# abb128/april-asr

Measured on AMD Instinct MI355X. Metric: audio_seconds_per_second (concurrent 16 kHz sessions x 1/RTF), aprilv0_en-us-sized streaming RNN-T, higher is better.
Workload: dtype f32

## Files before the change

april_asr_amd/__init__.py:

```python
import ctypes as C
import math
import struct
import weakref
from enum import IntEnum
from typing import Callable, List, Sequence

import numpy as np

from . import _ffi

__all__ = ["Result", "Token", "Model", "Session", "SessionGroup", "Bias", "resampler_taps"]


class Result(IntEnum):
    PARTIAL_RECOGNITION = 1
    FINAL_RECOGNITION = 2
    ERROR_CANT_KEEP_UP = 3
    SILENCE = 4


class Token:
    __slots__ = ("token", "logprob", "word_boundary", "sentence_end", "time", "log_softmax", "confidence", "blank_log_softmax",
                 "alternatives")

# ... 90 lines not shown
        if device_ptr:
            h = L.aprilx_model_from_blob(C.c_void_p(device_ptr), size, 1)
        else:
            blob = np.ascontiguousarray(blob, np.uint8)
            h = L.aprilx_model_from_blob(blob.ctypes.data, blob.size, 0)
        if not h:
            raise Exception("Failed to build model from blob")
        m = cls.__new__(cls)
        m._L = L; m._handle = h
        m.dims = _ffi.AprilxDims()
        L.aprilx_model_dims(h, C.byref(m.dims))
        return m

    @staticmethod
    def broadcast_id() -> bytes:
        L = _ffi.init()
        buf = C.create_string_buffer(128)
        n = L.aprilx_broadcast_get_id(buf, 128)
        if n <= 0:
            raise RuntimeError("aprilx_broadcast_get_id failed")
        return buf.raw[:n]

    @classmethod
    def broadcast(cls, root_model, rank: int, world: int, id_bytes: bytes):
        L = _ffi.init()
        idb = C.create_string_buffer(bytes(id_bytes), 128)
        h = L.aprilx_model_broadcast(root_model._handle if root_model is not None else None, rank, world, idb)
        if not h:
            raise Exception("model broadcast failed")
        if root_model is not None:
            return root_model
        m = cls.__new__(cls)
        m._L = L; m._handle = h
        m.dims = _ffi.AprilxDims()
        L.aprilx_model_dims(h, C.byref(m.dims))
        return m

    def load_info(self):
        info = _ffi.AprilxLoadInfo()
        self._L.aprilx_model_load_info(self._handle, C.byref(info))
        return info

    def save_blob(self, path: str, f16: bool = False):
        fn = self._L.aprilx_model_save_blob_f16 if f16 else self._L.aprilx_model_save_blob
        if fn(self._handle, path.encode("utf-8")) != 0:
            raise RuntimeError("blob save failed")

    @classmethod
    def load_blob(cls, path: str, init_gpu: bool = True):
        L = _ffi.init() if init_gpu else _ffi.lib()
        h = L.aprilx_model_load_blob(path.encode("utf-8"))
        if not h:
            raise Exception("Failed to load model blob")
        m = cls.__new__(cls)
        m._L = L; m._handle = h
        m.dims = _ffi.AprilxDims()
        L.aprilx_model_dims(h, C.byref(m.dims))
        return m

    def run_encoder(self, x, h, c):
        d = self.dims
        x = np.ascontiguousarray(x, np.float32); n = x.shape[0]
        h = np.ascontiguousarray(h, np.float32).reshape(n, d.n_layers, d.d_model)
        c = np.ascontiguousarray(c, np.float32).reshape(n, d.n_layers, d.hidden)
        eout = np.empty((n, d.joiner), np.float32); h2 = np.empty_like(h); c2 = np.empty_like(c)
        rc = self._L.aprilx_run_encoder(self._handle, n, x.ctypes.data, h.ctypes.data, c.ctypes.data,
                                        eout.ctypes.data, h2.ctypes.data, c2.ctypes.data)
        assert rc == 0
        return eout, h2, c2

    def run_decoder(self, ctx):
        ctx = np.ascontiguousarray(ctx, np.int64).reshape(-1, self.dims.context)
        out = np.empty((ctx.shape[0], self.dims.joiner), np.float32)
        assert self._L.aprilx_run_decoder(self._handle, ctx.shape[0], ctx.ctypes.data, out.ctypes.data) == 0
        return out

    def run_joiner(self, eout, dout):
        e = np.ascontiguousarray(eout, np.float32).reshape(-1, self.dims.joiner)
        dd = np.ascontiguousarray(dout, np.float32).reshape(-1, self.dims.joiner)
        out = np.empty((e.shape[0], self.dims.vocab), np.float32)
        assert self._L.aprilx_run_joiner(self._handle, e.shape[0], e.ctypes.data, dd.ctypes.data, out.ctypes.data) == 0
        return out

    def run_fbank(self, pcm_frames):
        p = np.ascontiguousarray(pcm_frames, np.int16).reshape(-1, self.dims.fft_size)
        out = np.empty((p.shape[0], self.dims.mel), np.float32)
        assert self._L.aprilx_run_fbank(self._handle, p.shape[0], p.ctypes.data, out.ctypes.data) == 0
        return out

    def resample(self, pcm, in_rate: int) -> np.ndarray:
        a = np.ascontiguousarray(pcm, np.int16).ravel()
        lmk = np.zeros(3, np.int32)
        if self._L.aprilx_resampler_taps(int(in_rate), int(self.dims.sample_rate), lmk.ctypes.data, None, 0) != 0:
            raise ValueError("input rate %d is not accepted" % in_rate)
        cap = (a.size * int(lmk[0]) + int(lmk[1]) - 1) // int(lmk[1])
        out = np.zeros(max(cap, 1), np.int16)
        n = int(self._L.aprilx_resample(self._handle, int(in_rate), a.ctypes.data, a.size, out.ctypes.data, out.size))
        if n < 0:
            raise ValueError("aprilx_resample refused %d samples at %d Hz" % (a.size, in_rate))
        return out[:n]

    def run_confidence(self, logits, k: int):
        a = np.ascontiguousarray(logits, np.float32).reshape(-1, self.dims.vocab)
        out = (_ffi.AprilxTokenInfo * a.shape[0])()
        if self._L.aprilx_run_confidence(self._handle, a.shape[0], a.ctypes.data, int(k), out) != 0:
            raise ValueError("aprilx_run_confidence refused n=%d k=%d" % (a.shape[0], k))
        return out

    def bias(self, phrases, boost: float = 2.0, strict: bool = False):
        return Bias(self, phrases, boost, flags=BIAS_STRICT if strict else 0)

    def run_confidence_biased(self, logits, k: int, bias, bias_state):
        a = np.ascontiguousarray(logits, np.float32).reshape(-1, self.dims.vocab)
        bs = np.ascontiguousarray(bias_state, np.int32).reshape(a.shape[0])
        out = (_ffi.AprilxTokenInfo * a.shape[0])()
        if self._L.aprilx_run_confidence_biased(self._handle, a.shape[0], a.ctypes.data, int(k), bias._handle, bs.ctypes.data, out) != 0:
            raise ValueError("aprilx_run_confidence_biased refused n=%d k=%d" % (a.shape[0], k))
        return out

    def run_decide_biased(self, logits, early_emit, now_ms, rnd, state, bias, bias_state, op: int = 0):
        st = np.ascontiguousarray(state, np.int32).reshape(-1, 4).copy()
        n = st.shape[0]
        lg = np.ascontiguousarray(logits, np.float32).reshape(n, self.dims.vocab)
        now = np.ascontiguousarray(now_ms, np.int32).reshape(n)
        bs = np.ascontiguousarray(bias_state, np.int32).reshape(n).copy()
        rec = np.zeros(n, np.dtype([("idx", np.int32), ("max", np.float32), ("blank", np.float32), ("flags", np.uint32)]))
        rc = self._L.aprilx_run_decide_biased(self._handle, n, int(op), lg.ctypes.data, float(early_emit), now.ctypes.data, int(rnd),
                                              st.ctypes.data, rec.ctypes.data, bias._handle, bs.ctypes.data)
        if rc != 0:
            raise ValueError("aprilx_run_decide_biased refused the call")
        return rec, st, bs

    def run_decide_opts(self, logits, early_emit, now_ms, rnd, state, opts, bias=None, bias_state=None, op: int = 0):
        st = np.ascontiguousarray(state, np.int32).reshape(-1, 4).copy()
        n = st.shape[0]
        lg = np.ascontiguousarray(logits, np.float32).reshape(n, self.dims.vocab)
        now = np.ascontiguousarray(now_ms, np.int32).reshape(n)
        bs = np.ascontiguousarray(bias_state, np.int32).reshape(n).copy() if bias is not None else None
        arr = (_ffi.AprilxSearchOptions * n)()
        for i, o in enumerate(opts):
            if o is not None:
                arr[i].size = C.sizeof(_ffi.AprilxSearchOptions); arr[i].endpoint_silence_ms = int(o[0]); arr[i].blank_penalty = float(o[1])
        rec = np.zeros(n, np.dtype([("idx", np.int32), ("max", np.float32), ("blank", np.float32), ("flags", np.uint32)]))
        rc = self._L.aprilx_run_decide_opts(self._handle, n, int(op), lg.ctypes.data, float(early_emit), now.ctypes.data, int(rnd), st.ctypes.data,
                                            rec.ctypes.data, bias._handle if bias is not None else None, bs.ctypes.data if bs is not None else None, arr)
        if rc != 0:
            raise ValueError("aprilx_run_decide_opts refused the call")
        return rec, st, bs

    def stats(self, device_index: int = 0):
        s = _ffi.AprilxStats()
        self._L.aprilx_model_stats(self._handle, device_index, C.byref(s))
        return s

    def feed_latencies(self, device_index: int = 0, reset: bool = False) -> np.ndarray:
        n = int(self._L.aprilx_model_feed_latency(self._handle, device_index, None, 0, 0))
        out = np.zeros(n, np.float64)
        if n:
            n = int(self._L.aprilx_model_feed_latency(self._handle, device_index, out.ctypes.data, n, 1 if reset else 0))
        elif reset:
            self._L.aprilx_model_feed_latency(self._handle, device_index, None, 0, 1)
        return out[:n]

    def profile(self, enable):
        self._L.aprilx_model_profile(self._handle, int(enable))


BIAS_STRICT = 1


class Bias:

    def __init__(self, model: Model, phrases, boost: float = 2.0, flags: int = 0):
        self._L = model._L
        items = [(p, boost) if isinstance(p, (str, bytes)) else (p[0], p[1]) for p in phrases]
        raw = [p.encode("utf-8") if isinstance(p, str) else bytes(p) for p, _ in items]
        arr = (C.c_char_p * max(len(raw), 1))(*raw)
        boosts = (C.c_float * max(len(raw), 1))(*[float(b) for _, b in items])
        err = C.create_string_buffer(256)
        self._handle = self._L.aprilx_bias_create_ex(model._handle, len(raw), arr, boosts, int(flags), err, 256)
        self.message = err.value.decode("utf-8", "replace")
        if not self._handle:
            raise ValueError("bias set refused: " + self.message)
        st, ed = C.c_int32(0), C.c_int64(0)
        self.dropped = int(self._L.aprilx_bias_info(self._handle, C.byref(st), C.byref(ed)))
        self.states, self.n_edges = int(st.value), int(ed.value)
        self.flags = int(self._L.aprilx_bias_flags(self._handle))
        self.strict = bool(self.flags & BIAS_STRICT)

    def edges(self, state: int):
        n = int(self._L.aprilx_bias_edges(self._handle, int(state), None, None, None, 0))
        if n < 0:
            raise ValueError("no state %d" % state)
        tok = np.zeros(n, np.int32); nxt = np.zeros(n, np.int32); bonus = np.zeros(n, np.float32)
        if n:
            assert self._L.aprilx_bias_edges(self._handle, int(state), tok.ctypes.data, nxt.ctypes.data, bonus.ctypes.data, n) == n
        return tok, nxt, bonus

    def csr(self):
        parts = [self.edges(s) for s in range(self.states)]
        off = np.zeros(self.states + 1, np.int32)
        off[1:] = np.cumsum([p[0].size for p in parts])
        return (off,) + tuple(np.concatenate([p[i] for p in parts]) if parts else np.zeros(0) for i in range(3))

    def close(self):
        if getattr(self, "_handle", None):
            self._L.aprilx_bias_free(self._handle)
            self._handle = None

    def __del__(self):
        try:
            self.close()
        except Exception:
            pass


def _dispatch(userdata, result_type, count, tokens):
    sess = C.cast(userdata, C.py_object).value
    sess._on_result(result_type, count, tokens)


_HANDLER = _ffi.HANDLER(_dispatch)


class Session:
    def __init__(self, model: Model, callback: Callable[[Result, List[Token]], None], asynchronous: bool = False,
                 no_rt: bool = False, speaker_name: str = "", raw_events: bool = False, counters=None, input_sample_rate=None,
                 alternatives=None, bias=None, endpoint_silence_ms=None, blank_penalty=None, max_utterance_ms=None):
        self._L = model._L
        self.info_log = None
        self.model = model
        self.callback = callback
        self._raw = raw_events
        cfg = _ffi.AprilConfig()
        cfg.flags = (2 if no_rt else 1) if asynchronous else 0
        if speaker_name:
            cfg.speaker = _ffi.AprilSpeakerID.from_buffer_copy(struct.pack("@q", hash(speaker_name)) * 2)
        if counters is not None:
            self._counters = counters
            cfg.handler = C.cast(self._L.aprilx_counting_handler, _ffi.HANDLER)
            cfg.userdata = counters.ctypes.data
        else:
            cfg.handler = _HANDLER
            cfg.userdata = id(self)
        self._handle = self._L.aas_create_session(model._handle, cfg)
        if not self._handle:
            raise Exception("Failed to create session")
        if not hasattr(model, "_sessions"):
            model._sessions = weakref.WeakSet()
        model._sessions.add(self)
        if input_sample_rate is not None:
            self.set_input_rate(input_sample_rate)
        if alternatives:
            self.set_confidence(alternatives)
        if bias is not None:
            self.set_bias(bias)
        if endpoint_silence_ms is not None or blank_penalty is not None or max_utterance_ms is not None:
            self.set_search_options(endpoint_silence_ms, blank_penalty, max_utterance_ms)

    def _on_result(self, result_type, count, tokens):
        if self.info_log is not None:
            self.info_log.append((int(result_type), [C.string_at(tokens[i].reserved, C.sizeof(_ffi.AprilxTokenInfo)) if tokens[i].reserved
                                                     else None for i in range(count)]))
        if self._raw:
            self.callback(int(result_type), [(tokens[i].token, float(tokens[i].logprob), int(tokens[i].flags),
                                              int(tokens[i].time_ms)) for i in range(count)])
        else:
            self.callback(Result(result_type), [Token(tokens[i], self.model) for i in range(count)])

    def get_rt_speedup(self) -> float:
        return float(self._L.aas_realtime_get_speedup(self._handle))

    def feed_pcm16(self, data) -> None:
        if isinstance(data, (bytes, bytearray, memoryview)):
            buf = (C.c_char * len(data)).from_buffer_copy(bytes(data))
            self._L.aas_feed_pcm16(self._handle, C.addressof(buf), len(data) // 2)
        else:
            a = np.ascontiguousarray(data, np.int16)
            self._L.aas_feed_pcm16(self._handle, a.ctypes.data, a.size)

    def flush(self) -> None:
        self._L.aas_flush(self._handle)

    def set_input_rate(self, rate_hz: int) -> None:
        if self._L.aprilx_session_set_input_rate(self._handle, int(rate_hz)) != 0:
            raise ValueError("input rate %d refused (outside 4000..384000 Hz / L > 4096, or audio fed since the last flush)" % rate_hz)

    def set_confidence(self, n_alternatives: int) -> None:
        if self._L.aprilx_session_set_confidence(self._handle, int(n_alternatives)) != 0:
            raise ValueError("confidence with %d alternatives refused (0..8, and no audio fed since the last flush)" % n_alternatives)

    def set_bias(self, bias) -> None:
        if self._L.aprilx_session_set_bias(self._handle, bias._handle if bias is not None else None) != 0:
            raise ValueError("bias set refused (built for another token list, 64 sets in use on the engine already, or audio fed since the last flush)")

    def set_search_options(self, endpoint_silence_ms=None, blank_penalty=None, max_utterance_ms=None) -> None:
        if endpoint_silence_ms is None and blank_penalty is None and max_utterance_ms is None:
            rc = self._L.aprilx_session_set_search_options(self._handle, None)
        else:
            o = _ffi.AprilxSearchOptions(C.sizeof(_ffi.AprilxSearchOptions), 2200 if endpoint_silence_ms is None else int(endpoint_silence_ms),
                                         0 if max_utterance_ms is None else int(max_utterance_ms), 0.0 if blank_penalty is None else float(blank_penalty))
            rc = self._L.aprilx_session_set_search_options(self._handle, C.byref(o))
        if rc != 0:
            raise ValueError("search options refused (a value out of range, or audio fed since the last flush)")

    @property
# ... 124 lines not shown
```

april_asr_amd/_ffi.py:

```python
import ctypes as C
import os

_HERE = os.path.dirname(os.path.abspath(__file__))
LIB_PATH = os.environ.get("APRIL_ASR_LIB") or os.path.join(_HERE, "libaprilasr.so")


class AprilSpeakerID(C.Structure):
    _fields_ = [("data", C.c_uint8 * 16)]


class AprilToken(C.Structure):
    _fields_ = [("token", C.c_char_p), ("logprob", C.c_float), ("flags", C.c_int),
                ("time_ms", C.c_size_t), ("reserved", C.c_void_p)]


HANDLER = C.CFUNCTYPE(None, C.c_void_p, C.c_int, C.c_size_t, C.POINTER(AprilToken))


class AprilConfig(C.Structure):
    _fields_ = [("speaker", AprilSpeakerID), ("handler", HANDLER), ("userdata", C.c_void_p), ("flags", C.c_int)]


class AprilxDims(C.Structure):
    _fields_ = [(n, C.c_int32) for n in ("n_layers", "d_model", "hidden", "ffn", "joiner", "vocab", "mel", "seg",
                                         "seg_step", "context", "fft_size", "frame_shift", "sample_rate", "blank_id",
                                         "n_devices", "precision", "d_model_file")] + [("param_count", C.c_int64)]


class AprilxStats(C.Structure):
    _fields_ = [(n, C.c_uint64) for n in ("ticks", "steps", "chunks", "rounds", "frames", "max_batch_seen")] + \
               [("kernel_ms", C.c_double * 6), ("kernel_launches", C.c_uint64 * 6), ("host_ms", C.c_double * 8),
                ("flights", C.c_uint64), ("replay_mismatch", C.c_uint64), ("kernels_per_step", C.c_uint64),
                ("lm_steps", C.c_uint64), ("lm_chunks", C.c_uint64),
                ("wave_steps", C.c_uint64), ("wave_chunks", C.c_uint64),
                ("gates_clock_ms", C.c_double), ("gates_clock_launches", C.c_uint64), ("gates_clock_rows", C.c_uint64),
                ("gates_clock_ms_by_n", C.c_double * 4), ("gates_clock_launches_by_n", C.c_uint64 * 4),
                ("resample_ms", C.c_double), ("resample_launches", C.c_uint64), ("confidence_records", C.c_uint64)]


class AprilxTokenInfo(C.Structure):
    _fields_ = [("size", C.c_uint32), ("n_alt", C.c_uint32), ("eval_index", C.c_uint64), ("lse", C.c_float),
                ("token_logprob", C.c_float), ("blank_logprob", C.c_float), ("reserved0", C.c_float),
                ("alt_id", C.c_int32 * 8), ("alt_logit", C.c_float * 8)]


class AprilxSearchOptions(C.Structure):
    _fields_ = [("size", C.c_uint32), ("endpoint_silence_ms", C.c_uint32), ("max_utterance_ms", C.c_uint32), ("blank_penalty", C.c_float)]


class AprilxLoadInfo(C.Structure):
    _fields_ = [("broadcast_ms", C.c_double), ("comm_init_ms", C.c_double), ("broadcast_bytes", C.c_uint64),
                ("ranks", C.c_int32), ("used_rccl", C.c_int32)]


EXPORTED_REFERENCE_SYMBOLS = [
    "aam_api_init", "aam_create_model", "aam_get_name", "aam_get_description", "aam_get_language",
    "aam_get_sample_rate", "aam_free", "aas_create_session", "aas_feed_pcm16", "aas_flush",
    "aas_realtime_get_speedup", "aas_free",
]
EXPORTED_ENGINE_SYMBOLS = [
    "aprilx_model_dims", "aprilx_model_token", "aprilx_model_blob_size", "aprilx_model_export_blob",
    "aprilx_model_from_blob", "aprilx_model_save_blob", "aprilx_model_save_blob_f16", "aprilx_model_load_blob",
    "aprilx_broadcast_get_id", "aprilx_model_broadcast", "aprilx_model_load_info", "aprilx_feed_many", "aprilx_flush_many", "aprilx_session_drain", "aprilx_feed_many_pipelined", "aprilx_drain_many",
    "aprilx_run_encoder", "aprilx_run_decoder", "aprilx_run_joiner", "aprilx_run_fbank", "aprilx_run_decide", "aprilx_plan_gemm", "aprilx_stream_form",
    "aprilx_session_trace_logits", "aprilx_session_chunks", "aprilx_session_read_frames", "aprilx_session_context", "aprilx_model_stats", "aprilx_model_profile", "aprilx_model_feed_latency",
    "aprilx_greedy_create", "aprilx_greedy_step", "aprilx_greedy_finish", "aprilx_greedy_free", "aprilx_probe_file", "aprilx_model_load_host", "aprilx_model_fbank_tables", "aprilx_counting_handler",
    "aprilx_session_set_input_rate", "aprilx_session_input_rate", "aprilx_resampler_taps", "aprilx_resample",
    "aprilx_session_set_confidence", "aprilx_session_confidence", "aprilx_run_confidence",
    "aprilx_bias_create", "aprilx_bias_free", "aprilx_bias_info", "aprilx_bias_edges", "aprilx_session_set_bias", "aprilx_session_bias_state",
    "aprilx_run_decide_biased", "aprilx_greedy_set_bias", "aprilx_greedy_bias_state",
    "aprilx_bias_create_ex", "aprilx_bias_flags", "aprilx_run_confidence_biased",
    "aprilx_session_set_search_options", "aprilx_session_search_options", "aprilx_run_decide_opts", "aprilx_greedy_set_search_options",
]

_lib = None
_inited = False


def lib():
    global _lib
    if _lib is not None:
        return _lib
    if not os.path.exists(LIB_PATH):
        raise ImportError("libaprilasr.so is not built: run `python -c 'import __graft_entry__ as g; g.build()'` "
                          "or `make -C april_asr_amd/csrc` (hipcc, gfx950). There is no CPU fallback.")
    L = C.CDLL(LIB_PATH)
    vp, sz = C.c_void_p, C.c_size_t
    L.aam_api_init.argtypes = [C.c_int]; L.aam_api_init.restype = None
    L.aam_create_model.argtypes = [C.c_char_p]; L.aam_create_model.restype = vp
    for f in ("aam_get_name", "aam_get_description", "aam_get_language"):
        getattr(L, f).argtypes = [vp]; getattr(L, f).restype = C.c_char_p
    L.aam_get_sample_rate.argtypes = [vp]; L.aam_get_sample_rate.restype = sz
    L.aam_free.argtypes = [vp]; L.aam_free.restype = None
    L.aas_create_session.argtypes = [vp, AprilConfig]; L.aas_create_session.restype = vp
    L.aas_feed_pcm16.argtypes = [vp, vp, sz]; L.aas_feed_pcm16.restype = None
    L.aas_flush.argtypes = [vp]; L.aas_flush.restype = None
    L.aas_realtime_get_speedup.argtypes = [vp]; L.aas_realtime_get_speedup.restype = C.c_float
    L.aas_free.argtypes = [vp]; L.aas_free.restype = None
    L.aprilx_model_dims.argtypes = [vp, C.POINTER(AprilxDims)]; L.aprilx_model_dims.restype = C.c_int
    L.aprilx_model_token.argtypes = [vp, C.c_int32]; L.aprilx_model_token.restype = C.c_char_p
    L.aprilx_model_blob_size.argtypes = [vp]; L.aprilx_model_blob_size.restype = sz
    L.aprilx_model_export_blob.argtypes = [vp, vp, sz]; L.aprilx_model_export_blob.restype = C.c_int
    L.aprilx_model_from_blob.argtypes = [vp, sz, C.c_int]; L.aprilx_model_from_blob.restype = vp
    L.aprilx_model_save_blob.argtypes = [vp, C.c_char_p]; L.aprilx_model_save_blob.restype = C.c_int
    L.aprilx_model_save_blob_f16.argtypes = [vp, C.c_char_p]; L.aprilx_model_save_blob_f16.restype = C.c_int
    L.aprilx_model_load_blob.argtypes = [C.c_char_p]; L.aprilx_model_load_blob.restype = vp
    L.aprilx_broadcast_get_id.argtypes = [vp, sz]; L.aprilx_broadcast_get_id.restype = C.c_int
    L.aprilx_model_broadcast.argtypes = [vp, C.c_int, C.c_int, vp]; L.aprilx_model_broadcast.restype = vp
    L.aprilx_model_load_info.argtypes = [vp, C.POINTER(AprilxLoadInfo)]; L.aprilx_model_load_info.restype = C.c_int
    L.aprilx_feed_many.argtypes = [sz, C.POINTER(vp), C.POINTER(vp), C.POINTER(sz)]; L.aprilx_feed_many.restype = None
    L.aprilx_flush_many.argtypes = [sz, C.POINTER(vp)]; L.aprilx_flush_many.restype = None
    L.aprilx_session_drain.argtypes = [vp]; L.aprilx_session_drain.restype = None
    L.aprilx_feed_many_pipelined.argtypes = [sz, C.POINTER(vp), C.POINTER(vp), C.POINTER(sz), C.c_int]; L.aprilx_feed_many_pipelined.restype = None
    L.aprilx_drain_many.argtypes = [sz, C.POINTER(vp)]; L.aprilx_drain_many.restype = None
    L.aprilx_run_encoder.argtypes = [vp, C.c_int] + [vp] * 6; L.aprilx_run_encoder.restype = C.c_int
    L.aprilx_run_decoder.argtypes = [vp, C.c_int, vp, vp]; L.aprilx_run_decoder.restype = C.c_int
    L.aprilx_run_joiner.argtypes = [vp, C.c_int, vp, vp, vp]; L.aprilx_run_joiner.restype = C.c_int
    L.aprilx_run_fbank.argtypes = [vp, C.c_int, vp, vp]; L.aprilx_run_fbank.restype = C.c_int
    L.aprilx_plan_gemm.argtypes = [C.c_int] * 6 + [vp]; L.aprilx_plan_gemm.restype = C.c_int
    L.aprilx_stream_form.argtypes = [C.c_int] * 6; L.aprilx_stream_form.restype = C.c_int
    L.aprilx_run_decide.argtypes = [vp, C.c_int, C.c_int, vp, C.c_float, vp, C.c_int, vp, vp]; L.aprilx_run_decide.restype = C.c_int
    L.aprilx_session_trace_logits.argtypes = [vp, vp, sz, C.POINTER(sz)]; L.aprilx_session_trace_logits.restype = None
    L.aprilx_session_chunks.argtypes = [vp]; L.aprilx_session_chunks.restype = C.c_uint64
    L.aprilx_session_read_frames.argtypes = [vp, C.c_uint64, C.c_int, C.c_void_p]; L.aprilx_session_read_frames.restype = C.c_uint64
    L.aprilx_session_context.argtypes = [vp, vp, vp]; L.aprilx_session_context.restype = None
    L.aprilx_model_stats.argtypes = [vp, C.c_int, C.POINTER(AprilxStats)]; L.aprilx_model_stats.restype = None
    L.aprilx_model_feed_latency.argtypes = [vp, C.c_int, vp, C.c_int, C.c_int]; L.aprilx_model_feed_latency.restype = C.c_int
    L.aprilx_model_profile.argtypes = [vp, C.c_int]; L.aprilx_model_profile.restype = None
    L.aprilx_greedy_create.argtypes = [vp, HANDLER, vp]; L.aprilx_greedy_create.restype = vp
    L.aprilx_greedy_step.argtypes = [vp, C.c_int32, C.c_float, C.c_float, C.c_float, sz, C.POINTER(C.c_int32)]
    L.aprilx_greedy_step.restype = C.c_int
    L.aprilx_greedy_finish.argtypes = [vp]; L.aprilx_greedy_finish.restype = None
    L.aprilx_greedy_free.argtypes = [vp]; L.aprilx_greedy_free.restype = None
    L.aprilx_model_load_host.argtypes = [C.c_char_p]; L.aprilx_model_load_host.restype = vp
    L.aprilx_model_fbank_tables.argtypes = [vp, vp, vp]; L.aprilx_model_fbank_tables.restype = C.c_int
    L.aprilx_probe_file.argtypes = [C.c_char_p, C.c_char_p, sz]; L.aprilx_probe_file.restype = C.c_int
    L.aprilx_session_set_input_rate.argtypes = [vp, C.c_uint32]; L.aprilx_session_set_input_rate.restype = C.c_int
    L.aprilx_session_input_rate.argtypes = [vp]; L.aprilx_session_input_rate.restype = C.c_uint32
    L.aprilx_resampler_taps.argtypes = [C.c_uint32, C.c_uint32, vp, vp, sz]; L.aprilx_resampler_taps.restype = C.c_int
    L.aprilx_resample.argtypes = [vp, C.c_uint32, vp, sz, vp, sz]; L.aprilx_resample.restype = C.c_int64
    L.aprilx_session_set_confidence.argtypes = [vp, C.c_int]; L.aprilx_session_set_confidence.restype = C.c_int
    L.aprilx_session_confidence.argtypes = [vp]; L.aprilx_session_confidence.restype = C.c_int
    L.aprilx_run_confidence.argtypes = [vp, C.c_int, vp, C.c_int, vp]; L.aprilx_run_confidence.restype = C.c_int
    L.aprilx_bias_create.argtypes = [vp, sz, C.POINTER(C.c_char_p), C.POINTER(C.c_float), C.c_char_p, sz]; L.aprilx_bias_create.restype = vp
    L.aprilx_bias_create_ex.argtypes = [vp, sz, C.POINTER(C.c_char_p), C.POINTER(C.c_float), C.c_uint32, C.c_char_p, sz]; L.aprilx_bias_create_ex.restype = vp
    L.aprilx_bias_flags.argtypes = [vp]; L.aprilx_bias_flags.restype = C.c_int
    L.aprilx_run_confidence_biased.argtypes = [vp, C.c_int, vp, C.c_int, vp, vp, vp]; L.aprilx_run_confidence_biased.restype = C.c_int
    L.aprilx_bias_free.argtypes = [vp]; L.aprilx_bias_free.restype = None
    L.aprilx_bias_info.argtypes = [vp, C.POINTER(C.c_int32), C.POINTER(C.c_int64)]; L.aprilx_bias_info.restype = C.c_int
    L.aprilx_bias_edges.argtypes = [vp, C.c_int32, vp, vp, vp, sz]; L.aprilx_bias_edges.restype = C.c_int
    L.aprilx_session_set_bias.argtypes = [vp, vp]; L.aprilx_session_set_bias.restype = C.c_int
    L.aprilx_session_bias_state.argtypes = [vp, C.POINTER(C.c_int32), C.POINTER(C.c_int32)]; L.aprilx_session_bias_state.restype = C.c_int
    L.aprilx_run_decide_biased.argtypes = [vp, C.c_int, C.c_int, vp, C.c_float, vp, C.c_int, vp, vp, vp, vp]; L.aprilx_run_decide_biased.restype = C.c_int
    L.aprilx_greedy_set_bias.argtypes = [vp, vp]; L.aprilx_greedy_set_bias.restype = C.c_int
    L.aprilx_greedy_bias_state.argtypes = [vp]; L.aprilx_greedy_bias_state.restype = C.c_int
    L.aprilx_session_set_search_options.argtypes = [vp, C.POINTER(AprilxSearchOptions)]; L.aprilx_session_set_search_options.restype = C.c_int
    L.aprilx_session_search_options.argtypes = [vp, C.POINTER(AprilxSearchOptions)]; L.aprilx_session_search_options.restype = C.c_int
    L.aprilx_run_decide_opts.argtypes = [vp, C.c_int, C.c_int, vp, C.c_float, vp, C.c_int, vp, vp, vp, vp, vp]; L.aprilx_run_decide_opts.restype = C.c_int
    L.aprilx_greedy_set_search_options.argtypes = [vp, C.POINTER(AprilxSearchOptions)]; L.aprilx_greedy_set_search_options.restype = C.c_int
    _lib = L
    return L


def init():
    global _inited
    L = lib()
    if not _inited:
        L.aam_api_init(1)
        _inited = True
    return L
```

april_asr_amd/csrc/engine.cc:

```cpp
#include "engine.h"
#include <array>
#include <algorithm>
#include <cmath>
#include <chrono>
#include <cstdlib>
#include <cstring>
#include "common.h"
#include "env.h"

namespace aprilx {

static size_t align64(size_t x) { return (x + 63) & ~(size_t)63; }

void plan_layout(const NetDims &d, bool has_dec_conv_b, PackedLayout &L)
{
    L.dims = d;
    L.has_dec_conv_b = has_dec_conv_b;
    L.vocab_pad = (d.vocab + 31) & ~31;
    size_t off = 0;
    auto take = [&](size_t n) { size_t o = off; off = align64(off + n); return o; };
    L.k3 = (d.conv_ch[1] * 9 + 63) & ~63;
    L.conv_w[0] = take((size_t)d.conv_ch[0] * 9); L.conv_b[0] = take((size_t)d.conv_ch[0]);
    L.conv_w[1] = take((size_t)d.conv_ch[1] * d.conv_ch[0] * 9); L.conv_b[1] = take((size_t)d.conv_ch[1]);
    L.conv_w[2] = take((size_t)L.k3 * d.conv_ch[2]); L.conv_b[2] = take((size_t)d.conv_ch[2]);
// ... 27 lines not shown
    v.emplace_back(L.w_out, (size_t)d.joiner * L.vocab_pad);
    return v;
}

static void pack_mfma(const float *W, int K, int N, int Npad, const std::vector<int> *colmap, float *dst)
{
    const int KB = K / 16, NTt = Npad / 16;
    for (int t = 0; t < NTt; ++t)
        for (int kb = 0; kb < KB; ++kb)
            for (int lane = 0; lane < 64; ++lane) {
                const int np = t * 16 + (lane & 15);
                const int src = np < N ? (colmap ? (*colmap)[(size_t)np] : np) : -1;
                float *o = dst + (((size_t)t * KB + kb) * 64 + lane) * 4;
                for (int j = 0; j < 4; ++j) {
                    const int k = kb * 16 + (lane >> 4) * 4 + j;
                    o[j] = src >= 0 ? W[(size_t)k * N + src] : 0.0f;
                }
            }
}

void pack_weights(const HostModel &m, PackedLayout &L, std::vector<float> &blob)
{
    const NetDims &d = L.dims;
    blob.assign(L.total, 0.0f);
    float *B = blob.data();
    for (int i = 0; i < 3; ++i) {
        if (i < 2) memcpy(B + L.conv_w[i], m.conv_w[i].data(), m.conv_w[i].size() * 4);
        memcpy(B + L.conv_b[i], m.conv_b[i].data(), m.conv_b[i].size() * 4);
    }
    {
        const int kreal = d.conv_ch[1] * 9, c2 = d.conv_ch[2];
        std::vector<float> w3((size_t)L.k3 * c2, 0.0f);
        for (int o = 0; o < c2; ++o) for (int k = 0; k < kreal; ++k) w3[(size_t)k * c2 + o] = m.conv_w[2][(size_t)o * kreal + k];
        pack_mfma(w3.data(), L.k3, c2, c2, nullptr, B + L.conv_w[2]);
    }
    {
        const int c2 = d.conv_ch[2], F = d.f_out;
        std::vector<float> we((size_t)d.embed_in * d.d_model);
        for (int c = 0; c < c2; ++c) for (int f = 0; f < F; ++f)
            memcpy(&we[((size_t)f * c2 + c) * d.d_model], &m.w_embed[((size_t)c * F + f) * d.d_model], (size_t)d.d_model * 4);
        pack_mfma(we.data(), d.embed_in, d.d_model, d.d_model, nullptr, B + L.w_embed);
    }
    memcpy(B + L.b_embed, m.b_embed.data(), (size_t)d.d_model * 4);
    L.embed_eps = m.embed_norm_eps;
    L.norm_eps.resize((size_t)d.n_layers);
    std::vector<int> gmap((size_t)4 * d.hidden);
    for (int u = 0; u < d.hidden; ++u) for (int g = 0; g < 4; ++g) gmap[(size_t)u * 4 + g] = g * d.hidden + u;
    for (int l = 0; l < d.n_layers; ++l) {
        const LayerWeights &lw = m.layers[(size_t)l];
        const PackedLayout::Layer &o = L.layers[(size_t)l];
        pack_mfma(lw.w_gates.data(), 2 * d.d_model, 4 * d.hidden, 4 * d.hidden, &gmap, B + o.wg);
        for (int n = 0; n < 4 * d.hidden; ++n) B[o.bg + n] = lw.b_gates[(size_t)gmap[(size_t)n]];
        pack_mfma(lw.w_hr.data(), d.hidden, d.d_model, d.d_model, nullptr, B + o.whr);
        pack_mfma(lw.w_ff1.data(), d.d_model, d.ffn, d.ffn, nullptr, B + o.wff1);
        memcpy(B + o.bff1, lw.b_ff1.data(), (size_t)d.ffn * 4);
        pack_mfma(lw.w_ff2.data(), d.ffn, d.d_model, d.d_model, nullptr, B + o.wff2);
        memcpy(B + o.bff2, lw.b_ff2.data(), (size_t)d.d_model * 4);
        L.norm_eps[(size_t)l] = lw.norm_eps;
    }
    pack_mfma(m.w_encproj.data(), d.d_model, d.joiner, d.joiner, nullptr, B + L.w_encproj);
    memcpy(B + L.b_encproj, m.b_encproj.data(), (size_t)d.joiner * 4);
    memcpy(B + L.emb, m.emb.data(), m.emb.size() * 4);
    memcpy(B + L.dec_conv, m.dec_conv.data(), m.dec_conv.size() * 4);
    if (!m.dec_conv_b.empty()) memcpy(B + L.dec_conv_b, m.dec_conv_b.data(), m.dec_conv_b.size() * 4);
    pack_mfma(m.w_decproj.data(), d.d_model, d.joiner, d.joiner, nullptr, B + L.w_decproj);
    memcpy(B + L.b_decproj, m.b_decproj.data(), (size_t)d.joiner * 4);
    pack_mfma(m.w_out.data(), d.joiner, d.vocab, L.vocab_pad, nullptr, B + L.w_out);
    memcpy(B + L.b_out, m.b_out.data(), (size_t)d.vocab * 4);
}

template <typename T> static T *dmalloc(size_t n) { HipLegacyLock legacy; T *p = nullptr; HIP_CHECK(hipMalloc((void **)&p, std::max<size_t>(n, 1) * sizeof(T))); return p; }
template <typename T> static T *hmalloc(size_t n) { HipLegacyLock legacy; T *p = nullptr; HIP_CHECK(hipHostMalloc((void **)&p, std::max<size_t>(n, 1) * sizeof(T), hipHostMallocDefault)); return p; }

std::recursive_mutex &hip_legacy_mutex() { static std::recursive_mutex m; return m; }

static int pick_kz(int K, int N, int kblk = 16)
{
    int kz = 256 / std::max(1, N / 16);
    kz = std::max(1, std::min(kz, 8));
    while (kz > 1 && ((K / kblk) / kz < 4 || (K / kblk) % (4 * kz) != 0)) kz >>= 1;
    return kz;
}

Engine::Engine(const EngineConfig &cfg, const PackedLayout &layout, const float *blob_host, const float *blob_device,
               const ModelParams &params, const FbankHostTables &ft, const std::vector<uint8_t> &tok_class)
    : cfg_(cfg), L_(layout), P_(params)
{
    HipLegacyLock legacy;
    HIP_CHECK(hipSetDevice(cfg_.device));
    HIP_CHECK(hipStreamCreateWithFlags(&stream_, hipStreamNonBlocking));
    HIP_CHECK(hipStreamCreateWithFlags(&f_stream_, hipStreamNonBlocking));
    HIP_CHECK(hipStreamCreateWithFlags(&s_stream_, hipStreamNonBlocking));
    search_stream_ = stream_;
    for (int i = 0; i < 32; ++i) { hipEvent_t e; HIP_CHECK(hipEventCreateWithFlags(&e, hipEventDisableTiming)); join_ev_.push_back(e); }
    split_streams_ = std::max(0, std::min(2, env_int("APRIL_SPLIT_STREAMS", 2)));
    const NetDims &d = L_.dims;
    w_ = dmalloc<float>(L_.total);
    if (blob_device) HIP_CHECK(hipMemcpy(w_, blob_device, L_.total * 4, hipMemcpyDeviceToDevice));
    else if (blob_host) HIP_CHECK(hipMemcpy(w_, blob_host, L_.total * 4, hipMemcpyHostToDevice));

    const size_t S = (size_t)cfg_.max_slots, MB = (size_t)cfg_.max_batch;
    ring_frames_ = std::max(P_.segment_size * 32, env_int("APRIL_RING_FRAMES", 8192));
    h_ = dmalloc<float>((size_t)d.n_layers * S * d.d_model);
    c_ = dmalloc<float>((size_t)d.n_layers * S * d.hidden);
    if (!env_str("APRIL_RING_FRAMES")) {
        size_t free_b = 0, total_b = 0;
        if (hipMemGetInfo(&free_b, &total_b) == hipSuccess && free_b > 0) {
            const size_t per_frame = S * (size_t)d.mel * sizeof(float);
            const size_t fit = (free_b / 4) / per_frame;
            if (fit < (size_t)ring_frames_) {
                const int shrunk = std::max(P_.segment_size * 32, (int)std::min<size_t>(fit, 8192) / 64 * 64);
                LOGW("engine: %zu MB of feature rings (%d frames x %zu slots) exceed a quarter of the %zu MB free on device %d: %d frames per session",
                     per_frame * (size_t)ring_frames_ >> 20, ring_frames_, S, free_b >> 20, cfg_.device, shrunk);
                ring_frames_ = shrunk;
            }
        } else (void)hipGetLastError();
        float *p = nullptr;
        if (hipMalloc((void **)&p, S * ring_frames_ * d.mel * sizeof(float)) == hipSuccess) ring_ = p;
        else {
            (void)hipGetLastError();
            const size_t asked = S * (size_t)ring_frames_ * d.mel * sizeof(float);
            ring_frames_ = std::max(P_.segment_size * 32, 2048);
            LOGW("engine: no room for %zu MB of feature rings, falling back to %d frames per session", asked >> 20, ring_frames_);
        }
    }
    if (!ring_) ring_ = dmalloc<float>(S * ring_frames_ * d.mel);
    eout_ = dmalloc<float>(S * d.joiner);
    dout_ = dmalloc<float>(S * d.joiner);
    gstate_ = dmalloc<GreedyState>(S);
    HIP_CHECK(hipMemset(h_, 0, (size_t)d.n_layers * S * d.d_model * 4));
    HIP_CHECK(hipMemset(c_, 0, (size_t)d.n_layers * S * d.hidden * 4));
    HIP_CHECK(hipMemset(ring_, 0, S * ring_frames_ * d.mel * 4));
    HIP_CHECK(hipMemset(eout_, 0, S * d.joiner * 4));
    HIP_CHECK(hipMemset(dout_, 0, S * d.joiner * 4));
    {
        std::vector<GreedyState> init(S);
        for (auto &g : init) { g.ctx0 = P_.blank_id; g.ctx1 = P_.blank_id; g.last_tok = -1; g.last_emit_ms = 0; }
        HIP_CHECK(hipMemcpy(gstate_, init.data(), S * sizeof(GreedyState), hipMemcpyHostToDevice));
    }
    cls_ = dmalloc<uint8_t>((size_t)d.vocab);
    HIP_CHECK(hipMemcpy(cls_, tok_class.data(), (size_t)d.vocab, hipMemcpyHostToDevice));

    kz_embed_ = pick_kz(d.embed_in, d.d_model);
    kz_hr_ = pick_kz(d.hidden, d.d_model);
    kz_ff2_ = pick_kz(d.ffn, d.d_model);
    kz_proj_ = pick_kz(d.d_model, d.joiner);
    kz_out_ = pick_kz(d.joiner, L_.vocab_pad);
    {
        const bool want = cfg_.precision == 1 && env_int("APRIL_F16_TILE", 1) != 0;
        f16_tile_ = want && d.d_model % 128 == 0 && d.hidden % 128 == 0 && d.ffn % 128 == 0 && d.hidden % 16 == 0;
        if (f16_tile_) {
            kzx_hr_ = pick_kz(d.hidden, d.d_model, 32); kzx_ff2_ = pick_kz(d.ffn, d.d_model, 32);
            for (int p = 0; p < 2; ++p) y16_buf_[p] = dmalloc<uint16_t>(MB * d.d_model);
            y16_ = y16_buf_[0]; xb16_ = dmalloc<uint16_t>(MB * d.d_model);
            u16_ = dmalloc<uint16_t>(MB * d.hidden); ff16_ = dmalloc<uint16_t>(MB * d.ffn);
            h16_ = dmalloc<uint16_t>((size_t)d.n_layers * S * d.d_model);
            HIP_CHECK(hipMemset(h16_, 0, (size_t)d.n_layers * S * d.d_model * 2));
        }
    }
    ws_mstride_ = cfg_.max_batch;
    const size_t ws_n = (size_t)std::max({kz_embed_ * d.d_model, kz_hr_ * d.d_model, kz_ff2_ * d.d_model, kz_proj_ * d.joiner, kz_out_ * L_.vocab_pad});
    ws_ = dmalloc<float>(ws_n * MB);
    ws_g_ = dmalloc<float>((size_t)std::max(kz_proj_ * d.joiner, kz_out_ * L_.vocab_pad) * MB);
    xin_ = dmalloc<float>(MB * d.embed_in);
    a3_ = dmalloc<float>(MB * d.f_out * L_.k3);
    HIP_CHECK(hipMemset(a3_, 0, MB * d.f_out * L_.k3 * 4));
    for (int p = 0; p < 2; ++p) { y_buf_[p] = dmalloc<float>(MB * d.d_model); ssq_buf_[p] = dmalloc<float>(MB * (d.d_model / SSQ_COLS)); }
    y_ = y_buf_[0]; ssq_ = ssq_buf_[0];
    ws_fe_ = dmalloc<float>((size_t)kz_embed_ * d.d_model * MB);
    ws_sr_ = dmalloc<float>((size_t)std::max(kz_proj_ * d.joiner, d.d_model) * MB);
    xb_ = dmalloc<float>(MB * d.d_model);
    u_ = dmalloc<float>(MB * d.hidden);
    ff_ = dmalloc<float>(MB * d.ffn);
    de_ = dmalloc<float>(MB * d.d_model);
    HIP_CHECK(hipMemset(de_, 0, MB * d.d_model * 4));
    logits_ = dmalloc<float>(3 * MB * d.vocab);
    logits_h_ = hmalloc<float>(3 * MB * d.vocab);
    ring_cap_ = std::max<size_t>((size_t)1 << 20, 3 * MB * 8 + 2 * S); ring_h_ = hmalloc<int>(2 * ring_cap_);
    step_cap_ = 1 << 14; step_off_h_ = hmalloc<int>((size_t)2 * step_cap_); rec_off_h_ = hmalloc<int>((size_t)2 * step_cap_);
    rec_cap_ = std::max<size_t>((size_t)1 << 20, 3 * MB * 8); rec_d_ = dmalloc<StepRecord>(2 * rec_cap_); rec_h_ = hmalloc<StepRecord>(2 * rec_cap_);
    for (int i = 0; i < 2; ++i) HIP_CHECK(hipEventCreateWithFlags(&flight_done_[i], hipEventDisableTiming));
    counter_d_ = dmalloc<int>(1);
    for (int p = 0; p < 2; ++p) {
        rec_off_buf_[p] = dmalloc<int>(1); flags_buf_[p] = dmalloc<int>(8); step_buf_[p] = dmalloc<int>(4 * MB);
        HIP_CHECK(hipMemset(rec_off_buf_[p], 0, 4)); HIP_CHECK(hipMemset(flags_buf_[p], 0, 32));
    }
    rec_off_d_ = rec_off_buf_[0]; flags_d_ = flags_buf_[0]; step_d_ = step_buf_[0];
    active_d_ = dmalloc<int>(MB); dirty_d_ = dmalloc<int>(MB);
    dec_slots_d_ = dmalloc<int>(std::max(S, MB));
    HIP_CHECK(hipMemset(counter_d_, 0, 4));

    upload_tables(ft);
    use_graphs_ = env_int("APRIL_NO_GRAPHS", 0) == 0;
    if (const int n = env_int("APRIL_GRAPH_CACHE_CAP", 0))
        step_graphs_.cap = lm_graphs_.cap = lm_search_graphs_.cap = sw_plan_cap_ = (size_t)std::max(n, 2), sw_graphs_.cap = 4 * sw_plan_cap_;
    free_.reserve(S);
    for (int i = cfg_.max_slots - 1; i >= 0; --i) free_.push_back(i);
    LOGI("engine: device %d, %d slots, max batch %d, weights %.1f MB, kz(embed,hr,ff2,proj,out)=%d,%d,%d,%d,%d",
         cfg_.device, cfg_.max_slots, cfg_.max_batch, L_.total * 4.0 / 1e6, kz_embed_, kz_hr_, kz_ff2_, kz_proj_, kz_out_);
}

void Engine::finish_weights()
{
    HipLegacyLock legacy;
    HIP_CHECK(hipSetDevice(cfg_.device));
    if (cfg_.precision == 1 && !wh_) {
        wh_ = dmalloc<uint16_t>(L_.total);
        for (const auto &sec : gemm_sections(L_)) launch_cvt_f16(w_ + sec.first, wh_ + sec.first, sec.second, nullptr);
        if (f16_tile_) {
            const NetDims &d = L_.dims;
            wx_ = dmalloc<uint16_t>(L_.total);
            for (const PackedLayout::Layer &o : L_.layers) {
                launch_repack_x32(w_ + o.wg, wx_ + o.wg, 2 * d.d_model, 4 * d.hidden, nullptr);
                launch_repack_x32(w_ + o.whr, wx_ + o.whr, d.hidden, d.d_model, nullptr);
                launch_repack_x32(w_ + o.wff1, wx_ + o.wff1, d.d_model, d.ffn, nullptr);
                launch_repack_x32(w_ + o.wff2, wx_ + o.wff2, d.ffn, d.d_model, nullptr);
            }
        }
        HIP_CHECK(hipDeviceSynchronize());
    }
    if (!conv_wt_) {
        const NetDims &d = L_.dims;
        conv_wt_ = dmalloc<float>((size_t)9 * d.conv_ch[0] + (size_t)9 * d.conv_ch[0] * d.conv_ch[1]);
        launch_conv_weight_transpose(w_ + L_.conv_w[0], w_ + L_.conv_w[1], d.conv_ch[0], d.conv_ch[1], conv_wt_, conv_wt_ + (size_t)9 * d.conv_ch[0], nullptr);
        HIP_CHECK(hipDeviceSynchronize());
    }
    build_dec_table();
}

void Engine::build_dec_table()
{
    if (dec_table_) return;
    const NetDims &d = L_.dims;
    const size_t limit_mb = (size_t)std::max(0, env_int("APRIL_DEC_TABLE_MB", 2048));
    const size_t rows = (size_t)d.vocab * (size_t)d.vocab;
    if (d.context != 2 || rows * (size_t)d.joiner * 4 > limit_mb * 1024 * 1024 || rows * (size_t)d.joiner * 4 >= ((size_t)1 << 32)) return;
    const int MB = cfg_.max_batch;
    float *table = dmalloc<float>(rows * (size_t)d.joiner);
    std::vector<int> iota((size_t)MB), ctx((size_t)MB * 2);
    for (int i = 0; i < MB; ++i) iota[(size_t)i] = i;
    int *ctx_d = dmalloc<int>((size_t)MB * 2);
    HIP_CHECK(hipMemcpy(dec_slots_d_, iota.data(), (size_t)MB * 4, hipMemcpyHostToDevice));
    for (size_t base = 0; base < rows; base += (size_t)MB) {
        const int n = (int)std::min<size_t>((size_t)MB, rows - base);
        for (int i = 0; i < n; ++i) { const size_t r = base + (size_t)i; ctx[(size_t)2 * i] = (int)(r / (size_t)d.vocab); ctx[(size_t)2 * i + 1] = (int)(r % (size_t)d.vocab); }
        HIP_CHECK(hipMemcpy(ctx_d, ctx.data(), (size_t)n * 8, hipMemcpyHostToDevice));
        DecEmbedArgs a; a.dec = dec_params(); a.ctx = ctx_d; a.M = n; a.out = de_; a.ldo = d.d_model;
        launch_dec_embed(a, stream_);
        run_decproj(n, dec_slots_d_, nullptr, nullptr, 1, table + base * (size_t)d.joiner);
        HIP_CHECK(hipStreamSynchronize(stream_));
    }
    (void)hipFree(ctx_d);
    dec_table_ = table;
    LOGI("engine: decoder table %zu rows x %d (%.0f MB)", rows, d.joiner, rows * (double)d.joiner * 4 / 1e6);
}

Engine::~Engine()
{
    HipLegacyLock legacy;
    (void)hipSetDevice(cfg_.device);
    (void)hipStreamSynchronize(f_stream_); (void)hipStreamSynchronize(stream_); (void)hipStreamSynchronize(s_stream_);
    dump_stream_trace();
    for (StreamTrace &t : trace_) for (hipEvent_t e : t.ev) if (e) (void)hipEventDestroy(e);
    if (trace_base_) (void)hipEventDestroy(trace_base_);
    for (hipEvent_t e : join_ev_) (void)hipEventDestroy(e);
    for (auto &e : ev_pool_) { (void)hipEventDestroy(e.a); (void)hipEventDestroy(e.b); }
    drop_graphs(); free_sw_plans(); if (gclk_slots_) (void)hipFree(gclk_slots_);
    if (lm_stream_) { (void)hipStreamSynchronize(lm_stream_); (void)hipStreamDestroy(lm_stream_); }
    for (hipEvent_t e : lm_events_) (void)hipEventDestroy(e);
    if (zargs_h_) { (void)hipHostFree(zargs_h_); (void)hipFree(zargs_d_); }
    for (int i = 0; i < 3; ++i) if (zargs_done_[i]) (void)hipEventDestroy(zargs_done_[i]);
    for (void *p : {(void *)lm_now_d_, (void *)lm_rows_d_, (void *)lm_rec_off_d_}) if (p) (void)hipFree(p);
    if (conf_k_d_) (void)hipFree(conf_k_d_);
    if (conf_d_) (void)hipFree(conf_d_);
    if (conf_k_h_) (void)hipHostFree(conf_k_h_);
    if (conf_h_) (void)hipHostFree(conf_h_);
    for (auto &b : bias_sets_) if (b.dev) (void)hipFree(b.dev);
    for (void *p : {(void *)bias_set_d_, (void *)bias_state_d_, (void *)bias_desc_d_}) if (p) (void)hipFree(p);
    for (void *p : {(void *)bias_set_h_, (void *)bias_desc_h_}) if (p) (void)hipHostFree(p);
    if (opt_d_) (void)hipFree(opt_d_);
    if (opt_h_) (void)hipHostFree(opt_h_);
    if (ws_g_) (void)hipFree(ws_g_);
    if (conv_wt_) (void)hipFree(conv_wt_);
    if (dec_table_) (void)hipFree(dec_table_);
    if (p_lm_) (void)hipFree(p_lm_);
    for (int p = 0; p < 2; ++p)
        for (void *q : {(void *)eout_lm_buf_[p], (void *)y16_buf_[p], (void *)y_buf_[p], (void *)ssq_buf_[p], (void *)rec_off_buf_[p], (void *)flags_buf_[p], (void *)step_buf_[p]}) if (q) (void)hipFree(q);
    if (ws_fe_) (void)hipFree(ws_fe_);
    if (ws_sr_) (void)hipFree(ws_sr_);
    for (void *p : {(void *)wx_, (void *)xb16_, (void *)u16_, (void *)ff16_, (void *)h16_}) if (p) (void)hipFree(p);
    for (void *p : {(void *)w_, (void *)wh_, (void *)h_, (void *)c_, (void *)ring_, (void *)eout_, (void *)dout_, (void *)gstate_, (void *)cls_, (void *)ws_, (void *)xin_,
                    (void *)a3_, (void *)xb_, (void *)u_, (void *)ff_, (void *)de_, (void *)logits_, (void *)rec_d_, (void *)counter_d_,
                    (void *)active_d_, (void *)dirty_d_, (void *)dec_slots_d_,
                    (void *)ds_desc_[0], (void *)ds_desc_[1], (void *)ds_pcm_[0], (void *)ds_pcm_[1]})
        if (p) (void)hipFree(p);
    for (void *p : {(void *)ring_h_, (void *)step_off_h_, (void *)rec_off_h_, (void *)rec_h_, (void *)logits_h_, (void *)hs_desc_[0], (void *)hs_desc_[1], (void *)hs_pcm_[0], (void *)hs_pcm_[1]})
        if (p) (void)hipHostFree(p);
    for (int b = 0; b < 2; ++b) if (fb_done_[b]) (void)hipEventDestroy(fb_done_[b]);
    for (int b = 0; b < 2; ++b) if (flight_done_[b]) (void)hipEventDestroy(flight_done_[b]);
    for (void *p : table_allocs_) (void)hipFree(p);
    (void)hipStreamDestroy(stream_); (void)hipStreamDestroy(f_stream_); (void)hipStreamDestroy(s_stream_);
}

void Engine::upload_tables(const FbankHostTables &ft)
{
    auto up = [&](const void *src, size_t bytes) {
        void *p = nullptr;
        HIP_CHECK(hipMalloc(&p, std::max<size_t>(bytes, 16)));
        if (bytes) HIP_CHECK(hipMemcpy(p, src, bytes, hipMemcpyHostToDevice));
        table_allocs_.push_back(p);
        return p;
    };
    ft_.window = (const float *)up(ft.window.data(), ft.window.size() * 4);
    ft_.mel = (const float *)up(ft.mel.data(), ft.mel.size() * 4);
    ft_.mel_lo = (const int *)up(ft.mel_lo.data(), ft.mel_lo.size() * 4);
    ft_.mel_hi = (const int *)up(ft.mel_hi.data(), ft.mel_hi.size() * 4);
    ft_.nfct = (int)ft.factors.size();
    for (int k = 0; k < ft_.nfct; ++k) {
        ft_.fct[k] = ft.factors[(size_t)k];
        ft_.tw[k] = (const double *)up(ft.tw[(size_t)k].data(), ft.tw[(size_t)k].size() * 8);
        ft_.tws[k] = ft.tws[(size_t)k].empty() ? nullptr : (const double *)up(ft.tws[(size_t)k].data(), ft.tws[(size_t)k].size() * 8);
    }
    ft_.padded = ft.padded; ft_.nbins = ft.nbins;
    pad_value_ = ft.pad_value;
}

int Engine::alloc_slot()
{
    std::lock_guard<std::mutex> g(slot_mu_);
    if (free_.empty() && !zero_pending_.empty()) zero_pending_slots();
    if (free_.empty()) return -1;
    const int s = free_.back();
    free_.pop_back();
    ++live_;
    return s;
}

void Engine::zero_pending_slots()
{
    if (zero_pending_.empty()) return;
    if (hipSetDevice(cfg_.device) == hipSuccess) {
        std::lock_guard<std::mutex> cg(capture_mu_);
        const NetDims &d = L_.dims;
        for (size_t o = 0; o < zero_pending_.size(); o += 64) {
            ZeroSlotArgs z;
            z.h = h_; z.c = c_; z.n_layers = d.n_layers; z.slots = (size_t)cfg_.max_slots; z.d_model = d.d_model; z.hidden = d.hidden;
            z.eout = eout_; z.dout = dout_; z.joiner = d.joiner; z.state = gstate_; z.blank = P_.blank_id; z.h16 = h16_;
            z.n_list = (int)std::min<size_t>(64, zero_pending_.size() - o);
            for (int i = 0; i < z.n_list; ++i) z.list[i] = zero_pending_[o + (size_t)i];
            launch_zero_slot(z, stream_);
        }
    }
    for (int s : zero_pending_) free_.push_back(s);
    zero_pending_.clear();
}

void Engine::free_slot(int slot)
{
    if (conf_ever_.load(std::memory_order_relaxed)) set_slot_confidence(slot, 0);
    if (bias_ever_.load(std::memory_order_relaxed)) set_slot_bias(slot, nullptr);
    if (opt_ever_.load(std::memory_order_relaxed)) set_slot_search_options(slot, SearchOpt{0u, 0.0f});
    std::lock_guard<std::mutex> g(slot_mu_);
    zero_pending_.push_back(slot);
    --live_;
    if (zero_pending_.size() >= 256) zero_pending_slots();
}

void Engine::sync_streams()
{
    HIP_CHECK(hipStreamSynchronize(f_stream_)); HIP_CHECK(hipStreamSynchronize(stream_)); HIP_CHECK(hipStreamSynchronize(s_stream_));
}

void Engine::sync()
{
    sync_streams();
    f_unseen_by_m_ = s_unseen_by_m_ = m_unseen_by_f_ = m_unseen_by_s_ = false;
    if (profiling_) collect_timing();
}

template <typename Chain> static hipGraphExec_t capture_graph(hipStream_t st, Chain &&chain)
{
    hipGraph_t graph = nullptr;
    hipGraphExec_t exec = nullptr;
    HipLegacyLock capture_guard;
    HIP_CHECK(hipStreamBeginCapture(st, hipStreamCaptureModeRelaxed));
    chain();
    HIP_CHECK(hipStreamEndCapture(st, &graph));
    HIP_CHECK(hipGraphInstantiate(&exec, graph, nullptr, nullptr, 0));
    HIP_CHECK(hipGraphDestroy(graph));
    return exec;
}

void GraphCache::clear()
{
    if (!map_.empty()) LOGI("engine: %s graphs emptied (%zu entries)", name, map_.size());
    for (auto &g : map_) (void)hipGraphExecDestroy(g.second);
    map_.clear(); uses_.clear();
}

template <typename Chain> hipGraphExec_t Engine::cached_graph(GraphCache &cache, const GraphCache::Key &key, hipStream_t st, Chain &&chain)
{
    if (!cache.find(key)) cache.insert(key, capture_graph(st, chain));
    return cache.find(key);
}

template <typename Capture> void Engine::capture_both_parities(Capture &&capture)
{
    const int par = flight_parity_;
    for (int q : {1 - par, par}) { select_parity(q); capture(); }
}

Engine::StreamTrace *Engine::trace_slot()
{
    static const char *path = env_str("APRIL_STREAM_TRACE");
    if (!path) return nullptr;
    if (!trace_base_) { HIP_CHECK(hipEventCreate(&trace_base_)); HIP_CHECK(hipEventRecord(trace_base_, stream_)); }
    if (trace_.size() >= 4096) return nullptr;
    trace_.emplace_back();
    StreamTrace &t = trace_.back();
    for (hipEvent_t &e : t.ev) HIP_CHECK(hipEventCreate(&e));
    return &t;
}

void Engine::dump_stream_trace()
{
    const char *path = env_str("APRIL_STREAM_TRACE");
    if (!path || trace_.empty()) return;
    FILE *f = fopen(path, "w");
    if (!f) return;
    fprintf(f, "# one line per split feed; times in us since the first split feed; FE = index fetch + conv + embed on stream F, LY = layer wavefront on M, SR = encoder_proj + search on S\n");
    fprintf(f, "# feed sessions chunks  FE_start FE_end  LY_start LY_end  SR_start SR_end   overlap: FE inside the previous feed's LY window? SR inside the next feed's LY window?\n");
    std::vector<std::array<float, 6>> ts;
    for (StreamTrace &t : trace_) {
        std::array<float, 6> a{};
        bool ok = t.used;
        for (int i = 0; i < 6 && ok; ++i) ok = hipEventElapsedTime(&a[(size_t)i], trace_base_, t.ev[i]) == hipSuccess;
        if (ok) ts.push_back(a); else (void)hipGetLastError();
    }
    for (size_t i = 0; i < ts.size(); ++i) {
        const auto &a = ts[i];
        const bool fe_in_prev = i > 0 && a[0] * 1e3f < ts[i - 1][3] * 1e3f && a[1] * 1e3f > ts[i - 1][2] * 1e3f;
        const bool sr_in_next = i + 1 < ts.size() && a[5] > ts[i + 1][2] && a[4] < ts[i + 1][3];
        fprintf(f, "%4zu %5d %2d  %10.1f %10.1f  %10.1f %10.1f  %10.1f %10.1f   %s %s\n", i, trace_[i].m, trace_[i].T, a[0] * 1e3, a[1] * 1e3, a[2] * 1e3, a[3] * 1e3, a[4] * 1e3, a[5] * 1e3,
                fe_in_prev ? "FE<prevLY" : "-", sr_in_next ? "SR<nextLY" : "-");
    }
    fclose(f);
}

void Engine::join(hipStream_t waiter, hipStream_t src)
{
    hipEvent_t e = join_ev_[join_pos_++ % join_ev_.size()];
    HIP_CHECK(hipEventRecord(e, src));
    HIP_CHECK(hipStreamWaitEvent(waiter, e, 0));
}

void Engine::general_prologue()
{
    if (f_unseen_by_m_) { join(stream_, f_stream_); f_unseen_by_m_ = false; }
    if (s_unseen_by_m_) { join(stream_, s_stream_); s_unseen_by_m_ = false; }
    m_unseen_by_f_ = m_unseen_by_s_ = true;
    flight_tail_s_ = false;
}

void Engine::set_profiling(bool on) { std::lock_guard<std::mutex> cg(capture_mu_); sync(); profiling_ = on; }
void Engine::reset_timing() { for (auto &t : timing_) t = KernelTiming(); }
void Engine::set_gates_clock(bool on)
{
    std::lock_guard<std::mutex> cg(capture_mu_);
    HIP_CHECK(hipSetDevice(cfg_.device));
    sync();
    if (on) {
        if (!gclk_slots_) gclk_slots_ = dmalloc<unsigned long long>((size_t)GCLK_SLOTS * STAMP_WORDS);
        HIP_CHECK(hipMemsetAsync(gclk_slots_, 0, (size_t)GCLK_SLOTS * STAMP_WORDS * 8, stream_));
        HIP_CHECK(hipStreamSynchronize(stream_));
        gclk_ms_ = 0; gclk_launches_ = 0; gclk_rows_ = 0;
        for (int i = 0; i < 4; ++i) { gclk_ms_n_[i] = 0; gclk_launches_n_[i] = 0; }
        gclk_ = true;
        return;
    }
    collect_gates_clock(); gclk_ = false;
}
void Engine::collect_gates_clock()
{
    if (!gclk_ || !gclk_slots_) return;
    std::vector<unsigned long long> h((size_t)GCLK_SLOTS * STAMP_WORDS);
    HIP_CHECK(hipMemcpyAsync(h.data(), gclk_slots_, h.size() * 8, hipMemcpyDeviceToHost, stream_)); HIP_CHECK(hipStreamSynchronize(stream_));
    for (auto &kv : sw_plans_)
        for (size_t i = 0; i < kv.second.stamp_slots.size(); ++i) {
            const auto &sl = kv.second.stamp_slots[i];
            const unsigned long long ticks = h[(size_t)sl.first * STAMP_WORDS + 2], n = h[(size_t)sl.first * STAMP_WORDS + 3];
            gclk_ms_ += (double)ticks * 1e-5; gclk_launches_ += (long)n; gclk_rows_ += (long)n * sl.second;
            const int bn = std::min(std::max(kv.second.stamp_n[i], 1), 4) - 1;
            gclk_ms_n_[bn] += (double)ticks * 1e-5; gclk_launches_n_[bn] += (long)n;
        }
}
void Engine::timed_begin(int cls)
{
    ++launch_count_;
    if (!profiling_) return;
    if (ev_used_ == ev_pool_.size()) { Ev e; HIP_CHECK(hipEventCreate(&e.a)); HIP_CHECK(hipEventCreate(&e.b)); e.cls = cls; ev_pool_.push_back(e); }
    ev_pool_[ev_used_].cls = cls;
    if (cls == T_GATES) gemm_profile_next_launch(ev_pool_[ev_used_].a, ev_pool_[ev_used_].b);
    else HIP_CHECK(hipEventRecord(ev_pool_[ev_used_].a, stream_));
}
void Engine::timed_end(int cls)
{
    if (!profiling_) return;
    if (cls == T_GATES) {
        if (gemm_profile_pending()) { gemm_profile_next_launch(nullptr, nullptr); return; }
    } else HIP_CHECK(hipEventRecord(ev_pool_[ev_used_].b, stream_));
    ++ev_used_;
}
void Engine::collect_timing()
{
    for (size_t i = 0; i < ev_used_; ++i) {
        float ms = 0;
        if (hipEventElapsedTime(&ms, ev_pool_[i].a, ev_pool_[i].b) == hipSuccess) { timing_[ev_pool_[i].cls].ms += ms; timing_[ev_pool_[i].cls].launches++; }
    }
    ev_used_ = 0;
}

void Engine::fbank(int n_frames, const FbankFrameDesc *desc, const std::pair<const int16_t *, size_t> *parts, size_t n_parts, size_t n_pcm, HostPool *pool)
{
    const int n_rs = n_frames > 0 ? std::max(rs_n_, 0) : 0;
    ResampleDesc *rs = rs_desc_;
    const std::pair<const int16_t *, size_t> *in_parts = rs_in_parts_;
    const size_t n_in_parts = n_rs ? rs_n_in_parts_ : 0, n_in = n_rs ? rs_n_in_ : 0;
    rs_n_ = 0;
    if (n_frames <= 0) return;
    HIP_CHECK(hipSetDevice(cfg_.device));
    for (int i = 0; i < n_rs; ++i) rs[i].taps = resample_table(rs_specs_[i]);
    if (n_frames > desc_cap_ || n_pcm + n_in > pcm_cap_ || (size_t)n_rs > rs_cap_) {
        sync();
        HipLegacyLock regrow_guard;
        for (int b = 0; b < 2; ++b) {
            if (hs_desc_[b]) { (void)hipHostFree(hs_desc_[b]); (void)hipFree(ds_desc_[b]); }
            if (hs_pcm_[b]) { (void)hipHostFree(hs_pcm_[b]); (void)hipFree(ds_pcm_[b]); }
        }
        desc_cap_ = std::max({n_frames * 2, desc_cap_, 1024});
        pcm_cap_ = std::max({(n_pcm + n_in) * 2, pcm_cap_, (size_t)1 << 16});
        rs_cap_ = std::max({(size_t)n_rs * 2, rs_cap_, n_rs ? (size_t)256 : (size_t)0});
        const size_t units = pcm_cap_ + 8 + ((size_t)desc_cap_ * sizeof(FbankFrameDesc) + 1) / 2 + 8 + rs_cap_ * sizeof(ResampleDesc) / 2;
        for (int b = 0; b < 2; ++b) {
            hs_pcm_[b] = hmalloc<int16_t>(units); ds_pcm_[b] = dmalloc<int16_t>(units);
            hs_desc_[b] = nullptr; ds_desc_[b] = nullptr;
            if (!fb_done_[b]) HIP_CHECK(hipEventCreateWithFlags(&fb_done_[b], hipEventDisableTiming));
        }
    }
    const int b = fb_flip_;
    fb_flip_ ^= 1;
    HIP_CHECK(hipEventSynchronize(fb_done_[b]));
    const size_t doff = ((n_pcm + n_in) * sizeof(int16_t) + 15) / 16 * 16;
    const size_t roff = (doff + (size_t)n_frames * sizeof(FbankFrameDesc) + 15) / 16 * 16;
    const size_t bytes = n_rs ? roff + (size_t)n_rs * sizeof(ResampleDesc) : doff + (size_t)n_frames * sizeof(FbankFrameDesc);
    char *hs = reinterpret_cast<char *>(hs_pcm_[b]);
    memcpy(hs + doff, desc, (size_t)n_frames * sizeof(FbankFrameDesc));
    ResampleArgs ra;
    if (n_rs) {
        ResampleDesc *hr = reinterpret_cast<ResampleDesc *>(hs + roff);
        int64_t blocks = 0, lds = 0;
        for (int i = 0; i < n_rs; ++i) {
            hr[i] = rs[i];
            hr[i].in_off += (int32_t)n_pcm;
            blocks = std::max<int64_t>(blocks, (rs[i].out_cnt + kResampleBlock - 1) / kResampleBlock);
            lds = std::max<int64_t>(lds, resample_lds_floats(rs[i].L, rs[i].M, rs[i].K));
        }
        ra.n_desc = n_rs; ra.max_blocks = (int)blocks; ra.lds_floats = (int)lds;
    }
    auto stage = [&](const std::pair<const int16_t *, size_t> *pp, size_t np, size_t base) {
        if (pool && np >= 256) {
            part_off_.resize(np);
            size_t off = base;
            for (size_t i = 0; i < np; ++i) { part_off_[i] = off; off += pp[i].second; }
            int16_t *dst = hs_pcm_[b];
            pool->run(np, 64, [&](size_t i) { if (pp[i].first) memcpy(dst + part_off_[i], pp[i].first, pp[i].second * sizeof(int16_t)); });
        } else {
            size_t off = base;
            for (size_t i = 0; i < np; ++i) { if (pp[i].first) memcpy(hs_pcm_[b] + off, pp[i].first, pp[i].second * sizeof(int16_t)); off += pp[i].second; }
        }
    };
    stage(parts, n_parts, 0);
    if (n_in_parts) stage(in_parts, n_in_parts, n_pcm);
    std::lock_guard<std::mutex> cg(capture_mu_);
    if (m_unseen_by_f_) { join(f_stream_, stream_); m_unseen_by_f_ = false; }
    HIP_CHECK(hipMemcpyAsync(ds_pcm_[b], hs_pcm_[b], bytes, hipMemcpyHostToDevice, f_stream_));
    FbankArgs a;
    a.t = ft_; a.pcm = ds_pcm_[b]; a.desc = reinterpret_cast<const FbankFrameDesc *>(reinterpret_cast<const char *>(ds_pcm_[b]) + doff); a.n_frames = n_frames; a.ring = ring_; a.ring_frames = ring_frames_; a.pad_value = pad_value_;
    if (n_rs) { ra.in = ds_pcm_[b]; ra.out = ds_pcm_[b]; ra.desc = reinterpret_cast<const ResampleDesc *>(reinterpret_cast<const char *>(ds_pcm_[b]) + roff); }
    if (profiling_) {
        join(stream_, f_stream_);
        if (n_rs) { timed_begin(T_RESAMPLE); launch_resample(ra, stream_); timed_end(T_RESAMPLE); }
        timed_begin(T_FBANK); launch_fbank(a, stream_); timed_end(T_FBANK);
        join(f_stream_, stream_);
    } else {
        if (n_rs) launch_resample(ra, f_stream_);
        launch_fbank(a, f_stream_);
    }
    HIP_CHECK(hipEventRecord(fb_done_[b], f_stream_));
    f_unseen_by_m_ = true;
}

const float *Engine::resample_table(const ResampleSpec *spec)
{
    std::lock_guard<std::mutex> g(rs_mu_);
    auto it = rs_tables_.find(spec);
    if (it != rs_tables_.end()) return it->second;
    HIP_CHECK(hipSetDevice(cfg_.device));
    float *d = dmalloc<float>(spec->taps.size());
    {
        HipLegacyLock legacy;
        if (!spec->taps.empty()) HIP_CHECK(hipMemcpy(d, spec->taps.data(), spec->taps.size() * sizeof(float), hipMemcpyHostToDevice));
        table_allocs_.push_back(d);
    }
    rs_tables_[spec] = d;
    return d;
}


RowScale Engine::in_scale(int l, size_t r0) const
{
    const NetDims &d = L_.dims;
    const int G = d.d_model / SSQ_COLS;
    RowScale r; r.ssq = ssq_ + r0 * G; r.groups = G; r.inv_n = 1.0f / (float)(d.d_norm ? d.d_norm : d.d_model); r.eps = l == 0 ? L_.embed_eps : L_.norm_eps[(size_t)l - 1];
    return r;
}

GemmArgs Engine::args_gates(int l, size_t r0, int rows, int waves) const
{
    const NetDims &d = L_.dims;
    const size_t S = (size_t)cfg_.max_slots;
    const PackedLayout::Layer &o = L_.layers[(size_t)l];
    GemmArgs g; g.a0 = y_ + r0 * d.d_model; g.lda0 = d.d_model; g.K0 = d.d_model; g.lda1 = d.d_model; g.K1 = d.d_model;
    lin(g, o.wg); g.M = rows; g.N = 4 * d.hidden; g.K = 2 * d.d_model; g.kz = 1; g.wave_mask = waves;
    if (f16_tile_) { g.a0 = reinterpret_cast<const float *>(y16_ + r0 * d.d_model); lin16(g, o.wg); }
    if (waves != GATES_H) g.x_scale = in_scale(l, r0);
    if (waves == GATES_X) {
        g.a1 = g.a0; g.epi = EPI_XPART; g.out = p_lm_ + r0 * 4 * d.hidden; g.ldo = 4 * d.hidden;
        return g;
    }
    g.a1 = h_ + (size_t)l * S * d.d_model; g.aidx1 = step_d_; g.epi = EPI_LSTM;
    g.out = u_ + r0 * d.hidden; g.ldo = d.hidden; g.bias = w_ + o.bg; g.c_state = c_ + (size_t)l * S * d.hidden; g.slot_idx = step_d_; g.hidden = d.hidden;
    if (waves == GATES_H) { g.p_add = p_lm_ + r0 * 4 * d.hidden; g.ldp = 4 * d.hidden; }
    else if (cfg_.precision == 0 && gates_tile_rows(rows)) g.tile_ok = 2;
    if (f16_tile_) {
        g.a1 = reinterpret_cast<const float *>(h16_ + (size_t)l * S * d.d_model); g.out = nullptr; g.out16 = u16_ + r0 * d.hidden;
    }
    return g;
}

constexpr long GATES_TILE_MIN_ROWS = 2048;
bool Engine::gates_tile_rows(long rows) const
{
    static const int mode = env_int("APRIL_GATES_TILE", 2);
    return mode == 1 || (mode == 2 && rows >= GATES_TILE_MIN_ROWS);
}

GemmArgs Engine::args_whr(int l, size_t r0, int rows) const
{
    const NetDims &d = L_.dims;
    const size_t S = (size_t)cfg_.max_slots;
    const PackedLayout::Layer &o = L_.layers[(size_t)l];
    GemmArgs g; g.a0 = u_ + r0 * d.hidden; g.lda0 = d.hidden; g.K0 = d.hidden; lin(g, o.whr);
    g.M = rows; g.N = d.d_model; g.K = d.hidden; g.kz = kz_hr_; g.tile_ok = tile_ok(); g.force_fullk = 1;
    g.epi = EPI_HR; g.state = h_ + (size_t)l * S * d.d_model; g.ld_state = d.d_model; g.slot_idx = step_d_; g.resid = y_ + r0 * d.d_model; g.ldr = d.d_model;
    g.r_scale = in_scale(l, r0);
    g.out = xb_ + r0 * d.d_model; g.ldo = d.d_model;
    if (f16_tile_) {
        g.a0 = reinterpret_cast<const float *>(u16_ + r0 * d.hidden); lin16(g, o.whr); g.kz = kzx_hr_;
        g.state16 = h16_ + (size_t)l * S * d.d_model; g.out16 = xb16_ + r0 * d.d_model;
    }
    return g;
}

GemmArgs Engine::args_ff1(int l, size_t r0, int rows) const
{
    const NetDims &d = L_.dims;
    const PackedLayout::Layer &o = L_.layers[(size_t)l];
    GemmArgs g; g.a0 = xb_ + r0 * d.d_model; g.lda0 = d.d_model; g.K0 = d.d_model; lin(g, o.wff1);
    g.M = rows; g.N = d.ffn; g.K = d.d_model; g.kz = 1; g.epi = EPI_BIAS_DSWISH; g.out = ff_ + r0 * d.ffn; g.ldo = d.ffn; g.bias = w_ + o.bff1;
    if (f16_tile_) { g.a0 = reinterpret_cast<const float *>(xb16_ + r0 * d.d_model); lin16(g, o.wff1); g.out = nullptr; g.out16 = ff16_ + r0 * d.ffn; }
    return g;
}

GemmArgs Engine::args_ff2(int l, size_t r0, int rows) const
{
    const NetDims &d = L_.dims;
    const PackedLayout::Layer &o = L_.layers[(size_t)l];
    GemmArgs g; g.a0 = ff_ + r0 * d.ffn; g.lda0 = d.ffn; g.K0 = d.ffn; lin(g, o.wff2);
    g.M = rows; g.N = d.d_model; g.K = d.ffn; g.kz = kz_ff2_; g.tile_ok = tile_ok(); g.force_fullk = 1;
    g.epi = EPI_RESID_SSQ; g.bias = w_ + o.bff2; g.resid = xb_ + r0 * d.d_model; g.ldr = d.d_model; g.out = y_ + r0 * d.d_model; g.ldo = d.d_model; g.ssq_out = ssq_ + r0 * (d.d_model / SSQ_COLS);
    if (f16_tile_) { g.a0 = reinterpret_cast<const float *>(ff16_ + r0 * d.ffn); lin16(g, o.wff2); g.kz = kzx_ff2_; g.out16 = y16_ + r0 * d.d_model; }
    return g;
}

GemmArgs Engine::args_encproj(size_t r0, int rows, const int *slot_idx, float *out) const
{
    const NetDims &d = L_.dims;
    GemmArgs g; g.a0 = y_ + r0 * d.d_model; g.lda0 = d.d_model; g.K0 = d.d_model; lin(g, L_.w_encproj);
    g.M = rows; g.N = d.joiner; g.K = d.d_model; g.kz = kz_proj_; g.tile_ok = tile_ok();
    g.epi = EPI_SLOT_STORE; g.bias = w_ + L_.b_encproj; g.out = out; g.ldo = d.joiner; g.slot_idx = slot_idx; g.x_scale = in_scale(d.n_layers, r0);
    return g;
}

static GemmArgs partial_form(const GemmArgs &f, float *ws, int m_stride)
{
    GemmArgs g = f;
    g.epi = EPI_PARTIAL; g.force_fullk = 0; g.out = ws; g.m_stride = m_stride;
    g.bias = nullptr; g.resid = nullptr; g.state = nullptr; g.slot_idx = nullptr; g.ssq_out = nullptr; g.r_scale = RowScale(); g.out16 = nullptr; g.state16 = nullptr;
    g.x_scale = RowScale(); g.row_mask = nullptr;
    return g;
}
static RowArgs row_form(const GemmArgs &f, const float *ws, int m_stride, int parts)
{
    RowArgs r; r.ws = ws; r.parts = parts; r.m_stride = m_stride; r.N = f.N; r.M = f.M;
    r.resid = f.resid; r.ldr = f.ldr; r.out = f.out; r.ldo = f.ldo; r.out16 = f.out16; r.run_flag = f.run_flag; r.run_gen = f.run_gen;
    if (f.epi == EPI_HR) { r.mode = ROW_HR; r.r_scale = f.r_scale; r.slot_idx = f.slot_idx; r.state = f.state; r.ld_state = f.ld_state; r.state16 = f.state16; }
    else if (f.epi == EPI_RESID_SSQ) { r.mode = ROW_RESID_SSQ; r.bias = f.bias; r.ssq_out = f.ssq_out; }
    else { r.mode = ROW_SLOT_STORE; r.bias = f.bias; r.slot_idx = f.slot_idx; r.r_scale = f.x_scale; r.row_mask = f.row_mask; }
    return r;
}

void Engine::launch_rowepi(GemmArgs f, float *ws, hipStream_t st, bool force, int cls)
{
    const int row_cls = cls == T_DEC ? T_DEC : T_ROW;
    f.force_fullk = force ? 1 : 0;
    if (gemm_fullk(f.M, f.N, f.kz, force, 1, f.tile_ok)) { timed_begin(cls); launch_gemm(f, st); timed_end(cls); return; }
    timed_begin(cls); launch_gemm(partial_form(f, ws, ws_mstride_), st); timed_end(cls);
    timed_begin(row_cls); launch_row(row_form(f, ws, ws_mstride_, gemm_partials(f.M, f.N, f.kz, 1, f.tile_ok)), st); timed_end(row_cls);
}

void Engine::encoder_front(size_t r0, int rows, const int *row_slots, const float *x_direct, hipStream_t st, float *ws)
{
    const NetDims &d = L_.dims;
    ConvEmbedArgs ca;
    ca.ring = ring_; ca.ring_frames = ring_frames_; ca.mel = d.mel; ca.seg = d.seg;
    ca.slot_idx = row_slots + r0; ca.ring_tail = step_d_ + cfg_.max_batch + r0; ca.x_direct = x_direct;
    for (int i = 0; i < 3; ++i) { ca.w[i] = w_ + L_.conv_w[i]; ca.b[i] = w_ + L_.conv_b[i]; ca.ch[i] = d.conv_ch[i]; ca.stride[i] = d.conv_stride[i]; }
    ca.ch1_per_group = 1;
    for (int k = 8; k > 1; --k) if (d.conv_ch[1] % k == 0) { ca.ch1_per_group = k; break; }
    ca.out = a3_ + r0 * d.f_out * L_.k3; ca.ldo = L_.k3; ca.M = rows;
    if (conv_wt_) { ca.w0t = conv_wt_; ca.w1t = conv_wt_ + (size_t)9 * d.conv_ch[0]; }
    timed_begin(T_CONV); launch_conv_embed(ca, st); timed_end(T_CONV);
// ... 121 lines not shown
}

static int lm_block_steps(int T)
{
    const int b = (int)(0.75 * std::sqrt((double)std::max(1, T)) + 0.5);
    return std::max(6, std::min(32, b));
}
constexpr int LM_WAVEFRONT_MIN_CHUNKS = 10;

static bool lm_wavefront_on()
{
    static const bool on = env_int("APRIL_LM_WAVEFRONT", 1) != 0;
    return on;
}

void Engine::run_lm_chain(int m, int T, bool dump_logits)
{
    const NetDims &d = L_.dims;
    const int MB = cfg_.max_batch;
    const int L = d.n_layers;
    launch_advance(advance_args(m, T), stream_);
    encoder_front(0, m * T, step_d_ + 3 * MB, nullptr, stream_, ws_);
    for (int l = 0; l < L; ++l) lm_stage_layer(l, m, 0, T, stream_);
    lm_stage_proj(m, 0, T, stream_, ws_);
    for (int t = 0; t < T; ++t) run_greedy_rounds(m, dump_logits, t, eout_lm_ + (size_t)t * m * d.joiner);
}

void Engine::run_lm_wavefront(int m, int T, bool dump_logits)
{
    const NetDims &d = L_.dims;
    const int MB = cfg_.max_batch;
    const int L = d.n_layers;
    const int blk = lm_block_steps(T);
    const int NB = (T + blk - 1) / blk;
    launch_advance(advance_args(m, T), stream_);
    hipStream_t cs = lm_stream_;
    HIP_CHECK(hipEventRecord(lm_events_[0], stream_));
    HIP_CHECK(hipStreamWaitEvent(cs, lm_events_[0], 0));

    const size_t need = (size_t)(NB + L + 1) * (size_t)(2 * blk + 6) * (size_t)L;
    if (need > zargs_region_) {
        HIP_CHECK(hipStreamSynchronize(cs));
        HipLegacyLock regrow_guard;
        if (zargs_h_) { (void)hipHostFree(zargs_h_); (void)hipFree(zargs_d_); }
        zargs_region_ = need + need / 4;
        zargs_h_ = hmalloc<GemmArgs>(3 * zargs_region_); zargs_d_ = dmalloc<GemmArgs>(3 * zargs_region_);
        for (int i = 0; i < 3; ++i) zargs_busy_[i] = false;
    }
    const int zslot = zargs_next_;
    zargs_next_ = (zargs_next_ + 1) % 3;
    if (zargs_busy_[zslot]) HIP_CHECK(hipEventSynchronize(zargs_done_[zslot]));
    zargs_pos_ = (size_t)zslot * zargs_region_;

    static const bool timing = env_str("APRIL_LM_TIMING") != nullptr;
    double tacc[6] = {0, 0, 0, 0, 0, 0};
    auto now = [&]() { return timing ? std::chrono::duration<double, std::micro>(std::chrono::steady_clock::now().time_since_epoch()).count() : 0.0; };
    struct Batch { size_t off; int n; };
    std::vector<Batch> plan;
    std::vector<size_t> plan_end((size_t)(NB + L + 1), 0);
    std::vector<GemmArgs> items;
    struct Act { int l, t0, t1; };
    std::vector<Act> act;
    double tq = now();
    auto lap = [&](int i) { if (timing) { const double t = now(); tacc[i] += t - tq; tq = t; } };
    const size_t first = zargs_pos_;
    for (int W = 0; W <= NB + L; ++W) {
        act.clear();
        for (int l = 0; l < L; ++l) { const int b = W - 1 - l; if (b >= 0 && b < NB) act.push_back({l, b * blk, std::min(T, (b + 1) * blk)}); }
        auto flush = [&]() {
            if (items.empty()) return;
            stage_gemm_z(items.data(), (int)items.size(), zargs_h_ + zargs_pos_);
            plan.push_back({zargs_pos_, (int)items.size()});
            zargs_pos_ += items.size(); items.clear();
        };
        auto by_len = [&](auto make) {
            for (int pass = 0; pass < 2; ++pass) {
                for (const Act &x : act) if (((x.t1 - x.t0) == blk) == (pass == 0)) items.push_back(make(x));
                flush();
            }
        };
        by_len([&](const Act &x) { return args_gates(x.l, (size_t)x.t0 * m, (x.t1 - x.t0) * m, GATES_X); });
        for (int i = 0; i < blk; ++i) {
            for (const Act &x : act) if (x.t0 + i < x.t1) items.push_back(args_gates(x.l, (size_t)(x.t0 + i) * m, m, GATES_H));
            flush();
            for (const Act &x : act) if (x.t0 + i < x.t1) items.push_back(args_whr(x.l, (size_t)(x.t0 + i) * m, m));
            flush();
        }
        by_len([&](const Act &x) { return args_ff1(x.l, (size_t)x.t0 * m, (x.t1 - x.t0) * m); });
        by_len([&](const Act &x) { return args_ff2(x.l, (size_t)x.t0 * m, (x.t1 - x.t0) * m); });
        plan_end[(size_t)W] = plan.size();
    }
    lap(0);
    if (zargs_pos_ > first)
        HIP_CHECK(hipMemcpyAsync(zargs_d_ + first, zargs_h_ + first, (zargs_pos_ - first) * sizeof(GemmArgs), hipMemcpyHostToDevice, cs));
    lap(1);
    for (int W = 0; W <= NB + L; ++W) {
        if (W < NB) encoder_front((size_t)W * blk * m, (std::min(T, (W + 1) * blk) - W * blk) * m, step_d_ + 3 * MB, nullptr, cs, ws_);
        lap(2);
        for (size_t k = W ? plan_end[(size_t)W - 1] : 0; k < plan_end[(size_t)W]; ++k) launch_gemm_z(zargs_h_ + plan[k].off, plan[k].n, zargs_d_ + plan[k].off, cs);
        lap(3);
        const int bp = W - L - 1;
        if (bp >= 0) {
            const int t0 = bp * blk, t1 = std::min(T, t0 + blk), len = t1 - t0;
            lm_stage_proj(m, t0, t1, cs, ws_);
            hipEvent_t e = lm_events_[1 + (size_t)(bp % (int)(lm_events_.size() - 1))];
            HIP_CHECK(hipEventRecord(e, cs));
            HIP_CHECK(hipStreamWaitEvent(stream_, e, 0));
            BlockSetupArgs bs;
            bs.now_src = step_d_ + 2 * MB + (size_t)t0 * m; bs.now_dst = lm_now_d_; bs.rows_dst = lm_rows_d_; bs.row0 = t0 * m; bs.count = len * m;
            bs.rec_off_step = rec_off_d_; bs.rec_off_block = lm_rec_off_d_; bs.rec_add = t0 * 3 * m; bs.flags = flags_d_; bs.n_flags = 8;
            launch_block_setup(bs, stream_);
            lap(4);
            auto search = [&]() {
                for (int i = 0; i < len; ++i) {
                    GreedyIo io;
                    io.gen = i + 1; io.now = lm_now_d_ + (size_t)i * m; io.eout = eout_lm_; io.eout_rows = lm_rows_d_ + (size_t)i * m;
                    io.rec_off = lm_rec_off_d_; io.rec_slot0 = i * 3;
                    io.dump = dump_logits ? logits_ + (size_t)(t0 + i) * 3 * m * d.vocab : nullptr;
                    run_greedy_rounds(m, io);
                }
            };
            if (!use_graphs_ || dump_logits) { search(); continue; }
            const GraphCache::Key key = graph_key(m, len);
            if (!lm_search_graphs_.find(key) && lm_search_graphs_.full()) { HIP_CHECK(hipStreamSynchronize(stream_));  lm_search_graphs_.clear(); }
            HIP_CHECK(hipGraphLaunch(cached_graph(lm_search_graphs_, key, stream_, search), stream_));
            lap(5);
        }
    }
    HIP_CHECK(hipEventRecord(zargs_done_[zslot], cs));
    zargs_busy_[zslot] = true;
    if (timing) fprintf(stderr, "lm wavefront %d x %d: host us: args %.0f, arg copy %.0f, front end %.0f, layer launches %.0f, proj + events + setup %.0f, search graph %.0f\n",
                        m, T, tacc[0], tacc[1], tacc[2], tacc[3], tacc[4], tacc[5]);
}

static bool lm_gates_split_on()
{
    static const bool on = env_int("APRIL_GATES_SPLIT", 1) != 0;
    return on;
}

Engine::SwPlan &Engine::sw_plan(int m, int T)
{
    const GraphCache::Key key = sw_key(m, T);
    auto it = sw_plans_.find(key);
    if (it != sw_plans_.end()) return it->second;
    if (sw_plans_.size() >= sw_plan_cap_) {
        sync();
        HipLegacyLock evict_guard;
        collect_gates_clock(); free_sw_plans();
        if (gclk_slots_) { HIP_CHECK(hipMemsetAsync(gclk_slots_, 0, (size_t)GCLK_SLOTS * STAMP_WORDS * 8, stream_)); HIP_CHECK(hipStreamSynchronize(stream_)); }
        gclk_used_ = 0;
    }
    SwPlan &p = sw_plans_[key];
    const NetDims &d = L_.dims;
    const int L = d.n_layers;
    std::vector<GemmArgs> items;
    std::vector<RowArgs> rows;
    for (int W = 0; W <= T + L; ++W) {
        for (int kind = 0; kind < 4; ++kind) {
            items.clear(); rows.clear();
            int n_act = 0;
            for (int l = 0; l < L; ++l) { const int t = W - 1 - l; if (t >= 0 && t < T) ++n_act; }
            if (n_act == 0) continue;
            const int kz = kind == 1 ? kz_hr() : kz_ff2();
            const int tk = f16_tile_ ? 2 : tile_ok();
            const bool split = (kind == 1 || kind == 3) && tk && (tk == 2 || gemm_tile_planned(m, d.d_model, kz, n_act)) && !gemm_fullk(m, d.d_model, kz, false, n_act, tk);
            for (int l = 0; l < L; ++l) {
                const int t = W - 1 - l;
                if (t < 0 || t >= T) continue;
                const size_t r0 = (size_t)t * m;
                GemmArgs g = kind == 0 ? args_gates(l, r0, m, GATES_ALL) : kind == 1 ? args_whr(l, r0, m) : kind == 2 ? args_ff1(l, r0, m) : args_ff2(l, r0, m);
                if (kind == 0 && cfg_.precision == 0) g.tile_ok = gates_tile_rows((long)m * n_act) ? 2 : 0;
                if (split) {
                    float *ws = ws_ + r0 * d.d_model;
                    rows.push_back(row_form(g, ws, ws_mstride_, gemm_partials(m, d.d_model, kz, n_act, tk)));
                    g = partial_form(g, ws, ws_mstride_);
                } else if (tk == 2) g.force_fullk = 0;
                items.push_back(g);
            }
            std::vector<int> groups;
            {
                int left = (int)items.size();
                const bool cut = kind == 0 && cfg_.precision == 0 && left >= 4 && !gates_tile_rows((long)m * n_act) && lm_gates_split_on();
                while (cut && left > 0) { const int take = (left == 4 || left == 2) ? 2 : (left >= 3 ? 3 : left); groups.push_back(take); left -= take; }
                if (groups.empty()) groups.push_back((int)items.size());
            }
            size_t first = 0;
            for (size_t gi = 0; gi < groups.size(); ++gi) {
                const int gn = groups[gi];
                if (kind == 0 && gclk_ && gclk_slots_ && gclk_used_ < GCLK_SLOTS) {
                    p.stamp_slots.push_back(std::make_pair(gclk_used_, (long)m * gn)); p.stamp_n.push_back(gn);
                    for (int i = 0; i < gn; ++i) items[first + (size_t)i].stamp = gclk_slots_ + (size_t)gclk_used_ * STAMP_WORDS;
                    ++gclk_used_;
                } else if (kind == 0 && gclk_ && gclk_slots_ && !gclk_warned_) {
                    gclk_warned_ = true; LOGW("engine: the gates clock is out of stamp slots (%d): the gates launches of further plans are not timed", GCLK_SLOTS);
                }
                SwPlan::Batch b; b.off = p.host.size(); b.n = gn; b.macro = W; b.kind = kind; b.roff = p.rhost.size(); b.rn = gi == 0 ? (int)rows.size() : 0;
                p.host.resize(p.host.size() + (size_t)gn);
                stage_gemm_z(items.data() + first, gn, p.host.data() + b.off);
                if (gi == 0) p.rhost.insert(p.rhost.end(), rows.begin(), rows.end());
                p.batches.push_back(b);
                first += (size_t)gn;
            }
        }
    }
    p.dev = dmalloc<GemmArgs>(p.host.size());
    HIP_CHECK(hipMemcpyAsync(p.dev, p.host.data(), p.host.size() * sizeof(GemmArgs), hipMemcpyHostToDevice, stream_));
    if (!p.rhost.empty()) {
        p.rdev = dmalloc<RowArgs>(p.rhost.size());
        HIP_CHECK(hipMemcpyAsync(p.rdev, p.rhost.data(), p.rhost.size() * sizeof(RowArgs), hipMemcpyHostToDevice, stream_));
    }
    return p;
}

void Engine::free_sw_plans()
{
    if (!sw_plans_.empty()) LOGI("engine: feed wavefront plans emptied (%zu plans)", sw_plans_.size());
    for (auto &p : sw_plans_) { if (p.second.dev) (void)hipFree(p.second.dev); if (p.second.rdev) (void)hipFree(p.second.rdev); }
    sw_graphs_.clear(); sw_plans_.clear();
}

void Engine::run_sw_chain(int m, int T, bool dump_logits, const SwPlan &p, int part, hipStream_t st)
{
    const NetDims &d = L_.dims;
    const int MB = cfg_.max_batch;
    if (part < 0 || part == 0) {
        launch_advance(advance_args(m, T), st);
        encoder_front(0, m * T, step_d_ + 3 * MB, nullptr, st, part == 0 ? ws_fe_ : ws_);
    }
    if (part < 0 || part == 1) {
        static const int cls_of[4] = {T_GATES, T_GEMM_OTHER, T_GEMM_OTHER, T_GEMM_OTHER};
        for (size_t bi = 0; bi < p.batches.size(); ++bi) {
            const SwPlan::Batch &b = p.batches[bi];
            timed_begin(cls_of[b.kind]); launch_gemm_z(p.host.data() + b.off, b.n, p.dev + b.off, st); timed_end(cls_of[b.kind]);
            if (b.rn > 0) { timed_begin(T_ROW); launch_row_z(p.rhost.data() + b.roff, b.rn, p.rdev + b.roff, st); timed_end(T_ROW); }
        }
        if (part < 0) lm_stage_proj(m, 0, T, st, ws_);
    }
    if (part < 0 || part == 2) {
        if (part == 2) lm_stage_proj(m, 0, T, st, ws_sr_);
        hipStream_t keep = search_stream_;
        search_stream_ = st;
        for (int t = 0; t < T; ++t) run_greedy_rounds(m, dump_logits, t, eout_lm_ + (size_t)t * m * d.joiner);
        search_stream_ = keep;
    }
}

int Engine::lm_step(int m, int T, const int *slots, const int *ring_tails, const int *now_ms, float *logits_out, int mode)
{
    const int rows = m * T;
    if (m <= 0 || T <= 0 || rows > cfg_.max_batch || !flight_has_room(rows + m, 1)) { LOGE("engine: layer-major step %d x %d does not fit (max batch %d)", m, T, cfg_.max_batch); abort(); }
    HIP_CHECK(hipSetDevice(cfg_.device));
    const NetDims &d = L_.dims;
    if (!p_lm_) {
        p_lm_ = dmalloc<float>((size_t)cfg_.max_batch * 4 * d.hidden);
        for (int p = 0; p < 2; ++p) eout_lm_buf_[p] = dmalloc<float>((size_t)cfg_.max_batch * d.joiner);
        eout_lm_ = eout_lm_buf_[flight_parity_];
    }
    if (!lm_stream_) {
        HIP_CHECK(hipStreamCreateWithFlags(&lm_stream_, hipStreamNonBlocking));
        for (int i = 0; i < 9; ++i) { hipEvent_t e; HIP_CHECK(hipEventCreateWithFlags(&e, hipEventDisableTiming)); lm_events_.push_back(e); }
        for (int i = 0; i < 3; ++i) HIP_CHECK(hipEventCreateWithFlags(&zargs_done_[i], hipEventDisableTiming));
        lm_now_d_ = dmalloc<int>((size_t)cfg_.max_batch); lm_rows_d_ = dmalloc<int>((size_t)cfg_.max_batch); lm_rec_off_d_ = dmalloc<int>(1);
    }
    const int k = stage_step(m, T, slots, ring_tails, now_ms);
    std::lock_guard<std::mutex> cg(capture_mu_);
    mode == 1 ? run_feed_wavefront(m, T, logits_out != nullptr) : run_layer_major(m, T, logits_out != nullptr);
    if (logits_out) read_back_logits(k, rows, logits_out);
    return k;
}

void Engine::run_feed_wavefront(int m, int T, bool dump_logits)
{
    sw_plan(m, T);
    const bool graphs = use_graphs_ && !profiling_ && !dump_logits && (sw_graphs_.find(sw_key(m, T)) || sw_graphs_.find(sw_key(m, T, 1)) || sw_graphs_.use(m, T) >= 2);
    const bool split = graphs && split_streams_ > 0 && overlap_hint_ && flight_steps_ == 1 && !gclk_;
    const hipStream_t on[3] = {split_streams_ >= 2 ? f_stream_ : stream_, stream_, s_stream_};
    if (graphs && !sw_graphs_.find(sw_key(m, T, split ? 1 : 0)))
        capture_both_parities([&]() {
            const SwPlan &pl = sw_plan(m, T);
            if (split) for (int part = 0; part < 3; ++part) cached_graph(sw_graphs_, sw_key(m, T, 1 + part), on[part], [&]() { run_sw_chain(m, T, false, pl, part, on[part]); });
            else cached_graph(sw_graphs_, sw_key(m, T), stream_, [&]() { run_sw_chain(m, T, false, pl, -1, stream_); });
        });
    if (split) { launch_split_feed(m, T, on[0]); return; }
    general_prologue();
    if (graphs) { HIP_CHECK(hipGraphLaunch(sw_graphs_.find(sw_key(m, T)), stream_)); return; }
    launch_count_ = 0; run_sw_chain(m, T, dump_logits, sw_plan(m, T), -1, stream_); kernels_per_step_ = (launch_count_ + 1 + T - 1) / T;
}

void Engine::launch_split_feed(int m, int T, hipStream_t fe)
{
    if (fe == f_stream_) {
        if (m_unseen_by_f_) { join(f_stream_, stream_); m_unseen_by_f_ = false; }
    } else if (f_unseen_by_m_) { join(stream_, f_stream_); f_unseen_by_m_ = false; }
    if (m_unseen_by_s_) { join(s_stream_, stream_); m_unseen_by_s_ = false; }
    StreamTrace *tr = trace_slot();
    auto part = [&](int i, hipStream_t st) {
        if (tr) HIP_CHECK(hipEventRecord(tr->ev[2 * i], st));
        HIP_CHECK(hipGraphLaunch(sw_graphs_.find(sw_key(m, T, 1 + i)), st));
        if (tr) HIP_CHECK(hipEventRecord(tr->ev[2 * i + 1], st));
    };
    part(0, fe);
    if (fe == f_stream_) { join(stream_, f_stream_); f_unseen_by_m_ = false; }
    part(1, stream_); join(s_stream_, stream_); part(2, s_stream_);
    if (tr) { tr->m = m; tr->T = T; tr->used = true; }
    s_unseen_by_m_ = true; flight_tail_s_ = true;
    if (fe != f_stream_) m_unseen_by_f_ = true;
}

void Engine::run_layer_major(int m, int T, bool dump_logits)
{
    general_prologue();
    const NetDims &d = L_.dims; const int tk = f16_tile_ ? 2 : tile_ok();
    const bool wavefront = lm_wavefront_on() && !profiling_ && T > LM_WAVEFRONT_MIN_CHUNKS &&
                           gemm_fullk(m, d.d_model, kz_hr(), true, 1, tk) && gemm_fullk(m, d.d_model, kz_ff2(), true, 1, tk);
    if (wavefront) { run_lm_wavefront(m, T, dump_logits); return; }
    if (!use_graphs_ || profiling_ || dump_logits) { launch_count_ = 0; run_lm_chain(m, T, dump_logits); kernels_per_step_ = launch_count_ + 1; return; }
    const GraphCache::Key key = graph_key(m, T);
    if (!lm_graphs_.find(key) && lm_graphs_.full()) { sync(); lm_graphs_.clear(); }
    HIP_CHECK(hipGraphLaunch(cached_graph(lm_graphs_, key, stream_, [&]() { run_lm_chain(m, T, false); }), stream_));
}

int Engine::stage_step(int m, int T, const int *slots, const int *ring_tails, const int *now_ms)
{
    const size_t rows = (size_t)m * (size_t)std::max(T, 1);
    const int k = next_step_index(); int *blk = ring_h_ + ring_pos_;
    memcpy(blk, slots, (size_t)m * 4); memcpy(blk + m, ring_tails, rows * 4); memcpy(blk + m + rows, now_ms, rows * 4);
    for (int t = 0; t < T; ++t) memcpy(blk + m + 2 * rows + (size_t)t * m, slots, (size_t)m * 4);
    step_off_h_[k] = (int)ring_pos_; rec_off_h_[k] = (int)rec_pos_;
    ring_pos_ += (size_t)m + (T ? 3 : 2) * rows; rec_pos_ += 3 * rows;
    if (conf_k_h_) note_conf_step(k, slots, m, 3 * rows);
    return k;
}

void Engine::read_back_logits(int k, int rows, float *out)
{
    const size_t n = (size_t)3 * rows * L_.dims.vocab;
    HIP_CHECK(hipMemcpyAsync(logits_h_, logits_, n * 4, hipMemcpyDeviceToHost, stream_));
    HIP_CHECK(hipMemcpyAsync(rec_h_ + rec_off_h_[k], rec_d_ + rec_off_h_[k], (size_t)3 * rows * sizeof(StepRecord), hipMemcpyDeviceToHost, stream_));
    sync();
    memcpy(out, logits_h_, n * 4);
}

void Engine::apply_confidence_pending()
{
    std::vector<std::pair<int, int>> todo;
    { std::lock_guard<std::mutex> g(conf_mu_); todo.swap(conf_pending_); conf_has_pending_.store(false, std::memory_order_release); }
    if (!conf_k_h_) {
        bool any = false;
        for (const auto &t : todo) any = any || t.second > 0;
        if (!any) return;
        std::lock_guard<std::mutex> cg(capture_mu_);
        HipLegacyLock legacy;
        sync();
        drop_graphs();
        const size_t S = (size_t)cfg_.max_slots;
        conf_k_d_ = dmalloc<uint8_t>(S); conf_k_h_ = hmalloc<uint8_t>(S);
        memset(conf_k_h_, 0, S);
        conf_d_ = dmalloc<ConfRecord>(2 * rec_cap_); conf_h_ = hmalloc<ConfRecord>(2 * rec_cap_);
        LOGI("engine: confidences on (side ring %.0f MB on the device and pinned)", 2.0 * rec_cap_ * sizeof(ConfRecord) / 1e6);
    }
    for (const auto &t : todo) if (t.first >= 0 && t.first < cfg_.max_slots) conf_k_h_[t.first] = (uint8_t)t.second;
    std::lock_guard<std::mutex> cg(capture_mu_);
    HIP_CHECK(hipMemcpyAsync(conf_k_d_, conf_k_h_, (size_t)cfg_.max_slots, hipMemcpyHostToDevice, stream_));
}

void Engine::drop_graphs()
{
    for (GraphCache *c : {&step_graphs_, &lm_graphs_, &lm_search_graphs_, &sw_graphs_}) c->clear();
}

BiasDesc Engine::upload_bias(const BiasSet &set, void **dev, hipStream_t st)
{
    auto pad = [](size_t b) { return (b + 15) & ~(size_t)15; };
    const size_t ns = set.state_off.size() * 4, ne = std::max<size_t>(set.edge_tok.size(), 1) * 4;
    char *p = nullptr;
    HIP_CHECK(hipMalloc((void **)&p, pad(ns) + 3 * pad(ne)));
    BiasDesc d;
    d.state_off = (const int32_t *)p; d.edge_tok = (const int32_t *)(p + pad(ns)); d.edge_next = (const int32_t *)(p + pad(ns) + pad(ne));
    d.edge_bonus = (const float *)(p + pad(ns) + 2 * pad(ne)); d.n_states = set.states(); d.flags = (int32_t)set.flags;
    HIP_CHECK(hipMemcpyAsync((void *)d.state_off, set.state_off.data(), ns, hipMemcpyHostToDevice, st));
    if (!set.edge_tok.empty()) {
        const size_t b = set.edge_tok.size() * 4;
        HIP_CHECK(hipMemcpyAsync((void *)d.edge_tok, set.edge_tok.data(), b, hipMemcpyHostToDevice, st));
        HIP_CHECK(hipMemcpyAsync((void *)d.edge_next, set.edge_next.data(), b, hipMemcpyHostToDevice, st));
        HIP_CHECK(hipMemcpyAsync((void *)d.edge_bonus, set.edge_bonus.data(), b, hipMemcpyHostToDevice, st));
    }
    *dev = p;
    return d;
}

void Engine::apply_bias_pending()
{
    std::lock_guard<std::mutex> bg(bias_mu_);
    std::vector<std::pair<int, int>> todo;
    todo.swap(bias_pending_);
    bias_has_pending_.store(false, std::memory_order_release);
    std::lock_guard<std::mutex> cg(capture_mu_);
    if (!bias_set_h_) {
        bool any = false;
        for (const auto &t : todo) any = any || t.second >= 0;
        if (!any) return;
        HipLegacyLock legacy;
        sync();
        drop_graphs();
        const size_t S = (size_t)cfg_.max_slots;
        bias_set_d_ = dmalloc<int32_t>(S); bias_set_h_ = hmalloc<int32_t>(S); bias_state_d_ = dmalloc<int32_t>(S);
        bias_desc_d_ = dmalloc<BiasDesc>(kBiasSets); bias_desc_h_ = hmalloc<BiasDesc>(kBiasSets);
        for (size_t i = 0; i < S; ++i) bias_set_h_[i] = -1;
        for (int i = 0; i < kBiasSets; ++i) bias_desc_h_[i] = BiasDesc();
        HIP_CHECK(hipMemsetAsync(bias_state_d_, 0, S * 4, stream_));
        LOGI("engine: phrase boosting on");
    }
    bool tables = false;
    for (int i = 0; i < kBiasSets; ++i) {
        BiasEntry &b = bias_sets_[(size_t)i];
        if (b.set && b.users > 0 && !b.dev) {
            HipLegacyLock legacy;
            bias_desc_h_[i] = upload_bias(*b.set, &b.dev, stream_);
            HIP_CHECK(hipStreamSynchronize(stream_));
            tables = true;
        } else if (b.set && b.users == 0) {
            if (b.dev) { HipLegacyLock legacy; sync_streams(); (void)hipFree(b.dev); b.dev = nullptr; }
            bias_desc_h_[i] = BiasDesc();
            b.set.reset();
            tables = true;
        }
    }
    for (const auto &t : todo) {
        bias_set_h_[t.first] = t.second;
        HIP_CHECK(hipMemsetAsync(bias_state_d_ + t.first, 0, 4, stream_));
    }
    if (tables) HIP_CHECK(hipMemcpyAsync(bias_desc_d_, bias_desc_h_, sizeof(BiasDesc) * kBiasSets, hipMemcpyHostToDevice, stream_));
    HIP_CHECK(hipMemcpyAsync(bias_set_d_, bias_set_h_, (size_t)cfg_.max_slots * 4, hipMemcpyHostToDevice, stream_));
}

void Engine::apply_search_options_pending()
{
    std::vector<std::pair<int, SearchOpt>> todo;
    { std::lock_guard<std::mutex> g(opt_mu_); todo.swap(opt_pending_); opt_has_pending_.store(false, std::memory_order_release); }
    if (!opt_h_) {
        bool any = false;
        for (const auto &t : todo) any = any || t.second.endpoint_ms != 0;
        if (!any) return;
        std::lock_guard<std::mutex> cg(capture_mu_);
        HipLegacyLock legacy;
        sync();
        drop_graphs();
        const size_t S = (size_t)cfg_.max_slots;
        opt_d_ = dmalloc<SearchOpt>(S); opt_h_ = hmalloc<SearchOpt>(S);
        memset(opt_h_, 0, S * sizeof(SearchOpt));
        LOGI("engine: search options on");
    }
    for (const auto &t : todo) if (t.first >= 0 && t.first < cfg_.max_slots) opt_h_[t.first] = t.second;
    std::lock_guard<std::mutex> cg(capture_mu_);
    HIP_CHECK(hipMemcpyAsync(opt_d_, opt_h_, (size_t)cfg_.max_slots * sizeof(SearchOpt), hipMemcpyHostToDevice, stream_));
}

int Engine::read_bias_state(int slot)
{
    if (!bias_ever_.load(std::memory_order_relaxed)) return 0;
    std::lock_guard<std::mutex> bg(bias_mu_);
    for (const auto &t : bias_pending_) if (t.first == slot) return 0;
    HipLegacyLock legacy;
    HIP_CHECK(hipSetDevice(cfg_.device));
    sync_streams();
    int v = 0;
    if (bias_state_d_) HIP_CHECK(hipMemcpy(&v, bias_state_d_ + slot, 4, hipMemcpyDeviceToHost));
    return v;
}

void Engine::note_conf_step(int k, const int *slots, int m, size_t records)
{
    bool any = false;
    for (int i = 0; i < m && !any; ++i) any = conf_k_h_[slots[i]] != 0;
    if (!any) return;
    const size_t first = (size_t)rec_off_h_[k];
    if (!conf_spans_.empty() && conf_spans_.back().first + conf_spans_.back().second == first) conf_spans_.back().second += records;
    else conf_spans_.push_back(std::make_pair(first, records));
}

void Engine::select_parity(int p)
{
    flight_parity_ = p;
    y_ = y_buf_[p]; ssq_ = ssq_buf_[p]; y16_ = y16_buf_[p]; step_d_ = step_buf_[p]; flags_d_ = flags_buf_[p]; rec_off_d_ = rec_off_buf_[p]; eout_lm_ = eout_lm_buf_[p];
}

void Engine::begin_flight()
{
    HIP_CHECK(hipSetDevice(cfg_.device));
    const int p = flight_parity_ = next_parity_; next_parity_ ^= 1;
    if (flight_open_[p]) { HIP_CHECK(hipEventSynchronize(flight_done_[p])); flight_open_[p] = false; }
    if (conf_has_pending_.load(std::memory_order_acquire)) apply_confidence_pending();
    if (bias_has_pending_.load(std::memory_order_acquire)) apply_bias_pending();
    if (opt_has_pending_.load(std::memory_order_acquire)) apply_search_options_pending();
    conf_spans_.clear();
    ring_base_ = (size_t)p * ring_cap_; rec_base_ = (size_t)p * rec_cap_;
    ring_pos_ = ring_base_; rec_pos_ = rec_base_; flight_steps_ = 0;
    select_parity(p);
    flight_tail_s_ = false;
    { std::lock_guard<std::mutex> g(slot_mu_); zero_pending_slots(); }
}

bool Engine::flight_has_room(int rows, int nsteps) const
{
    return flight_steps_ + nsteps <= step_cap_ && ring_pos_ + (size_t)3 * rows + (size_t)cfg_.max_slots <= ring_base_ + ring_cap_ && rec_pos_ + (size_t)3 * rows <= rec_base_ + rec_cap_;
}

int Engine::step(int m, const int *slots, const int *ring_tails, const int *now_ms, float *logits_out)
{
    if (m <= 0 || m > cfg_.max_batch || !flight_has_room(m, 1)) { LOGE("engine: step of %d rows does not fit (max batch %d)", m, cfg_.max_batch); abort(); }
    const int k = stage_step(m, 0, slots, ring_tails, now_ms);
    std::lock_guard<std::mutex> cg(capture_mu_);
    general_prologue();
    const GraphCache::Key key = graph_key(m);
    if (use_graphs_ && !profiling_ && !logits_out && (step_graphs_.find(key) || step_graphs_.use(m) >= 2)) {
        if (!step_graphs_.find(key)) {
            if (step_graphs_.full()) { sync(); step_graphs_.clear(); }
            capture_both_parities([&]() { cached_graph(step_graphs_, graph_key(m), stream_, [&]() { run_chain(m, false); }); });
        }
        HIP_CHECK(hipGraphLaunch(step_graphs_.find(key), stream_));
        return k;
    }
    launch_count_ = 0; run_chain(m, logits_out != nullptr); kernels_per_step_ = launch_count_ + 1;
    if (logits_out) read_back_logits(k, m, logits_out);
    return k;
}

void Engine::decode_rows(int n, const int *slots, int op)
{
    if (n <= 0) return;
    if (dec_table_ && op == 0) return;
    HIP_CHECK(hipSetDevice(cfg_.device));
    const NetDims &d = L_.dims;
    const int MB = cfg_.max_batch;
    std::lock_guard<std::mutex> cg(capture_mu_);
    general_prologue();
    for (int o = 0; o < n; o += MB) {
        const int m = std::min(MB, n - o);
        if (ring_pos_ + (size_t)m > ring_base_ + ring_cap_) { LOGE("engine: index ring exhausted"); abort(); }
        int *blk = ring_h_ + ring_pos_;
        memcpy(blk, slots + o, (size_t)m * 4);
        ring_pos_ += (size_t)m;
        HIP_CHECK(hipMemcpyAsync(dec_slots_d_, blk, (size_t)m * 4, hipMemcpyHostToDevice, stream_));
        DecRowsArgs a; a.slot_idx = dec_slots_d_; a.M = m; a.op = op; a.blank = P_.blank_id; a.state = gstate_; a.dec = dec_params(); a.de_out = dec_table_ ? nullptr : de_; a.ld_de = d.d_model;
        a.bias_state = bias_state_d_;
        timed_begin(T_DEC); launch_dec_rows(a, stream_); timed_end(T_DEC);
        if (!dec_table_) run_decproj(m, dec_slots_d_, nullptr, nullptr, 1);
    }
}

int Engine::close_flight()
{
    HIP_CHECK(hipSetDevice(cfg_.device));
    std::lock_guard<std::mutex> cg(capture_mu_);
    hipStream_t tail = s_stream_;
    if (!(flight_tail_s_ && s_unseen_by_m_)) {
        tail = stream_;
        if (f_unseen_by_m_) { join(stream_, f_stream_); f_unseen_by_m_ = false; }
        if (s_unseen_by_m_) { join(stream_, s_stream_); s_unseen_by_m_ = false; }
    }
    if (rec_pos_ > rec_base_) HIP_CHECK(hipMemcpyAsync(rec_h_ + rec_base_, rec_d_ + rec_base_, (rec_pos_ - rec_base_) * sizeof(StepRecord), hipMemcpyDeviceToHost, tail));
    for (const auto &sp : conf_spans_) {
        HIP_CHECK(hipMemcpyAsync(conf_h_ + sp.first, conf_d_ + sp.first, sp.second * sizeof(ConfRecord), hipMemcpyDeviceToHost, tail));
        conf_copied_.fetch_add(sp.second, std::memory_order_relaxed);
    }
    conf_spans_.clear();
    HIP_CHECK(hipEventRecord(flight_done_[flight_parity_], tail));
    flight_open_[flight_parity_] = true;
    return flight_parity_;
}

bool Engine::flight_done(int parity)
{
    const hipError_t e = hipEventQuery(flight_done_[parity]);
    if (e == hipSuccess) return true;
    if (e != hipErrorNotReady) HIP_CHECK(e);
    (void)hipGetLastError();
    return false;
}

void Engine::wait_flight(int parity)
{
    HIP_CHECK(hipSetDevice(cfg_.device));
    HIP_CHECK(hipEventSynchronize(flight_done_[parity]));
    if (profiling_) sync();
}

void Engine::end_flight() { wait_flight(close_flight()); }

void Engine::zero_slots(int n)
{
    const NetDims &d = L_.dims;
    for (int i = 0; i < n; ++i) {
        ZeroSlotArgs z;
        z.h = h_; z.c = c_; z.n_layers = d.n_layers; z.slots = (size_t)cfg_.max_slots; z.d_model = d.d_model; z.hidden = d.hidden;
        z.eout = eout_; z.dout = dout_; z.joiner = d.joiner; z.state = gstate_; z.blank = P_.blank_id; z.slot = i; z.h16 = h16_;
        launch_zero_slot(z, stream_);
    }
    HIP_CHECK(hipStreamSynchronize(stream_));
}

void Engine::debug_encoder(int n, const float *x, const float *h, const float *c, float *eout, float *h2, float *c2)
{
    std::lock_guard<std::mutex> cg(capture_mu_);
    HipLegacyLock legacy;
    HIP_CHECK(hipSetDevice(cfg_.device));
    const NetDims &d = L_.dims;
    const size_t S = (size_t)cfg_.max_slots;
    if (n > cfg_.max_batch || n > cfg_.max_slots) { LOGE("debug_encoder: n too large"); abort(); }
    std::vector<int> slots((size_t)n);
    for (int i = 0; i < n; ++i) slots[(size_t)i] = i;
    float *xd = dmalloc<float>((size_t)n * d.seg * d.mel);
    HIP_CHECK(hipMemcpy(xd, x, (size_t)n * d.seg * d.mel * 4, hipMemcpyHostToDevice));
    for (int i = 0; i < n; ++i)
        for (int l = 0; l < d.n_layers; ++l) {
            HIP_CHECK(hipMemcpy(h_ + ((size_t)l * S + i) * d.d_model, h + ((size_t)i * d.n_layers + l) * d.d_model, (size_t)d.d_model * 4, hipMemcpyHostToDevice));
            HIP_CHECK(hipMemcpy(c_ + ((size_t)l * S + i) * d.hidden, c + ((size_t)i * d.n_layers + l) * d.hidden, (size_t)d.hidden * 4, hipMemcpyHostToDevice));
        }
    HIP_CHECK(hipMemcpy(step_d_, slots.data(), (size_t)n * 4, hipMemcpyHostToDevice));
    if (f16_tile_)
        for (int l = 0; l < d.n_layers; ++l) launch_cvt_f16(h_ + (size_t)l * S * d.d_model, h16_ + (size_t)l * S * d.d_model, (size_t)n * d.d_model, stream_);
    run_encoder_rows(n, xd);
    sync();
    for (int i = 0; i < n; ++i) {
        HIP_CHECK(hipMemcpy(eout + (size_t)i * d.joiner, eout_ + (size_t)i * d.joiner, (size_t)d.joiner * 4, hipMemcpyDeviceToHost));
        for (int l = 0; l < d.n_layers; ++l) {
            HIP_CHECK(hipMemcpy(h2 + ((size_t)i * d.n_layers + l) * d.d_model, h_ + ((size_t)l * S + i) * d.d_model, (size_t)d.d_model * 4, hipMemcpyDeviceToHost));
            HIP_CHECK(hipMemcpy(c2 + ((size_t)i * d.n_layers + l) * d.hidden, c_ + ((size_t)l * S + i) * d.hidden, (size_t)d.hidden * 4, hipMemcpyDeviceToHost));
        }
    }
    (void)hipFree(xd);
    zero_slots(n);
}

void Engine::debug_decoder(int n, const int64_t *ctx, float *dout)
{
// ... 249 lines not shown
```

april_asr_amd/csrc/engine.h:

```cpp
#pragma once
#include <hip/hip_runtime.h>
#include <atomic>
#include <cstdint>
#include <deque>
#include <array>
#include <functional>
#include <map>
#include <memory>
#include <mutex>
#include <string>
#include <utility>
#include <vector>
#include "bias.h"
#include "fbank_tables.h"
#include "resample.h"
#include "kernels.h"
#include "host_pool.h"
#include "model_loader.h"

namespace aprilx {

struct PackedLayout {
    NetDims dims;
    size_t conv_w[3], conv_b[3];
    int k3 = 0;
    size_t w_embed, b_embed;
    struct Layer { size_t wg, bg, whr, wff1, bff1, wff2, bff2; };
    std::vector<Layer> layers;
    size_t w_encproj, b_encproj, emb, dec_conv, dec_conv_b, w_decproj, b_decproj, w_out, b_out;
    size_t total = 0;
    int vocab_pad = 0;
    bool has_dec_conv_b = false;
    std::vector<float> norm_eps;
    float embed_eps = 0;
};
void plan_layout(const NetDims &d, bool has_dec_conv_b, PackedLayout &L);
std::vector<std::pair<size_t, size_t>> gemm_sections(const PackedLayout &L);
void pack_weights(const HostModel &m, PackedLayout &L, std::vector<float> &blob);

std::recursive_mutex &hip_legacy_mutex();
struct HipLegacyLock { std::lock_guard<std::recursive_mutex> g; HipLegacyLock() : g(hip_legacy_mutex()) {} };

struct EngineConfig {
    int device = 0;
    int max_slots = 4096;
    int max_batch = 2048;
    int precision = 0;
};

struct KernelTiming { double ms = 0; long launches = 0; };

struct GraphCache {
    using Key = std::array<int, 3>;
    const char *name; size_t cap;
    bool full() const { return map_.size() >= cap; }
    hipGraphExec_t find(const Key &k) const { auto it = map_.find(k); return it == map_.end() ? nullptr : it->second; }
    void insert(const Key &k, hipGraphExec_t g) { map_[k] = g; }
    int use(int m, int T = 0) { return ++uses_[std::make_pair(m, T)]; }
    void clear();
    std::map<Key, hipGraphExec_t> map_; std::map<std::pair<int, int>, int> uses_;
};

class Engine {
public:
    Engine(const EngineConfig &cfg, const PackedLayout &layout, const float *blob_host, const float *blob_device,
           const ModelParams &params, const FbankHostTables &ft, const std::vector<uint8_t> &tok_class);
    ~Engine();

    int device() const { return cfg_.device; }
    int max_batch() const { return cfg_.max_batch; }
    int max_slots() const { return cfg_.max_slots; }
    int ring_frames() const { return ring_frames_; }
    const NetDims &dims() const { return L_.dims; }
    hipStream_t stream() const { return stream_; }
    const float *weights_device() const { return w_; }
    float *weights_mut() { return w_; }
    void finish_weights();
    int precision() const { return cfg_.precision; }
    int tile_ok() const { return cfg_.precision == 0 ? 1 : 0; }
    bool f16_tile() const { return f16_tile_; }
    const PackedLayout &layout() const { return L_; }

    int alloc_slot();
    void free_slot(int slot);
    int live_slots() const { return live_.load(std::memory_order_relaxed); }

    void fbank(int n_frames, const FbankFrameDesc *desc, const std::pair<const int16_t *, size_t> *parts, size_t n_parts, size_t n_pcm,
               HostPool *pool = nullptr);
    void set_resample_pass(int n, ResampleDesc *rs, const ResampleSpec *const *specs, const std::pair<const int16_t *, size_t> *in_parts,
                           size_t n_in_parts, size_t n_in)
    {
        rs_n_ = n; rs_desc_ = rs; rs_specs_ = specs; rs_in_parts_ = in_parts; rs_n_in_parts_ = n_in_parts; rs_n_in_ = n_in;
    }
    void begin_flight();
    bool flight_has_room(int rows, int nsteps = 1) const;
    int step(int m, const int *slots, const int *ring_tails, const int *now_ms, float *logits_out = nullptr);
    int lm_step(int m, int T, const int *slots, const int *ring_tails, const int *now_ms, float *logits_out = nullptr, int mode = 0);
    int lm_max_rows() const { return cfg_.max_batch; }
    void decode_rows(int n, const int *slots, int op);
    int close_flight();
    bool flight_done(int parity);
    void wait_flight(int parity);
    void end_flight();
    bool profiling() const { return profiling_; }
    void set_overlap_hint(bool on) { overlap_hint_ = on; }
    const StepRecord *records(int step_index) const { return rec_h_ + rec_off_h_[step_index]; }
    void set_slot_confidence(int slot, int k)
    {
        std::lock_guard<std::mutex> g(conf_mu_);
        conf_pending_.push_back(std::make_pair(slot, k));
        if (k > 0) conf_ever_.store(true, std::memory_order_relaxed);
        conf_has_pending_.store(true, std::memory_order_release);
    }
    const ConfRecord *conf_records(int step_index) const { return conf_h_ ? conf_h_ + rec_off_h_[step_index] : nullptr; }
    uint64_t confidence_records() const { return conf_copied_.load(std::memory_order_relaxed); }
    static constexpr int kBiasSets = 64;
    bool set_slot_bias(int slot, const std::shared_ptr<const BiasSet> &set)
    {
        std::lock_guard<std::mutex> g(bias_mu_);
        if (slot < 0 || slot >= cfg_.max_slots) return false;
        if (bias_slot_set_.empty()) {
            if (!set) return true;
            bias_slot_set_.assign((size_t)cfg_.max_slots, -1); bias_sets_.resize(kBiasSets);
        }
        int idx = -1;
        if (set) {
            if (set->vocab != L_.dims.vocab || set->vocab > kBiasMaxVocab) return false;
            for (int i = 0; i < kBiasSets && idx < 0; ++i) if (bias_sets_[(size_t)i].set == set) idx = i;
            for (int i = 0; i < kBiasSets && idx < 0; ++i) if (!bias_sets_[(size_t)i].set) idx = i;
            if (idx < 0) return false;
            bias_sets_[(size_t)idx].set = set;
            ++bias_sets_[(size_t)idx].users;
        }
        const int old = bias_slot_set_[(size_t)slot];
        if (old < 0 && idx < 0) return true;
        if (old >= 0) --bias_sets_[(size_t)old].users;
        bias_slot_set_[(size_t)slot] = idx;
        bias_pending_.push_back(std::make_pair(slot, idx));
        if (set) bias_ever_.store(true, std::memory_order_relaxed);
        bias_has_pending_.store(true, std::memory_order_release);
        return true;
    }
    int read_bias_state(int slot);
    void debug_decide_biased(int n, int op, const float *logits, float early_emit, const int *now_ms, int round, int32_t *state_io, StepRecord *rec_out,
                             const BiasSet &set, int32_t *bias_state_io);
    void set_slot_search_options(int slot, SearchOpt o)
    {
        std::lock_guard<std::mutex> g(opt_mu_);
        if (o.endpoint_ms == 0 && !opt_ever_.load(std::memory_order_relaxed)) return;
        opt_pending_.push_back(std::make_pair(slot, o));
        if (o.endpoint_ms) opt_ever_.store(true, std::memory_order_relaxed);
        opt_has_pending_.store(true, std::memory_order_release);
    }
    void debug_decide_opts(int n, int op, const float *logits, float early_emit, const int *now_ms, int round, int32_t *state_io, StepRecord *rec_out,
                           const BiasSet *set, int32_t *bias_state_io, const SearchOpt *opts);
    void sync();
    void sync_streams();

    void debug_encoder(int n, const float *x, const float *h, const float *c, float *eout, float *h2, float *c2);
    void debug_decoder(int n, const int64_t *ctx, float *dout);
    void debug_joiner(int n, const float *eout, const float *dout, float *logits);
    void debug_decide(int n, int op, const float *logits, float early_emit, const int *now_ms, int round, int32_t *state_io, StepRecord *rec_out);
    void debug_confidence(int n, const float *logits, int k, ConfRecord *out, const BiasSet *set = nullptr, const int32_t *bias_state = nullptr);
    void debug_fbank(int n_frames, const int16_t *pcm_frames , float *out );
    void debug_resample(const ResampleSpec *spec, const int16_t *pcm, size_t n, int16_t *out);
    void read_ring(int slot, int row, int n_rows, float *out);
    void read_greedy_state(int slot, GreedyState *out);

    void set_profiling(bool on);
    void set_gates_clock(bool on);
    void gates_clock(double *ms, long *launches, long *rows) const { *ms = gclk_ms_; *launches = gclk_launches_; *rows = gclk_rows_; }
    void gates_clock_by_n(double *ms4, long *launches4) const { for (int i = 0; i < 4; ++i) { ms4[i] = gclk_ms_n_[i]; launches4[i] = gclk_launches_n_[i]; } }
    KernelTiming timing(int cls) const { return timing_[cls]; }
    void reset_timing();
    enum { T_GATES = 0, T_GEMM_OTHER = 1, T_ROW = 2, T_CONV = 3, T_FBANK = 4, T_DEC = 5, T_RESAMPLE = 6, T_COUNT = 7 };
    long kernels_per_step() const { return kernels_per_step_.load(std::memory_order_relaxed); }

private:
    void upload_tables(const FbankHostTables &ft);
    void zero_slots(int n);
    void run_encoder_rows(int n, const float *x_direct);
    void encoder_front(size_t r0, int rows, const int *row_slots, const float *x_direct, hipStream_t st, float *ws);
    void lm_stage_layer(int l, int m, int t0, int t1, hipStream_t st);
    void lm_stage_proj(int m, int t0, int t1, hipStream_t st, float *ws);
    enum { GATES_ALL = 0xF, GATES_X = 0x3, GATES_H = 0xC };
    RowScale in_scale(int l, size_t r0) const;
    GemmArgs args_gates(int l, size_t r0, int rows, int waves) const;
    GemmArgs args_whr(int l, size_t r0, int rows) const;
    GemmArgs args_ff1(int l, size_t r0, int rows) const;
    GemmArgs args_ff2(int l, size_t r0, int rows) const;
    GemmArgs args_encproj(size_t r0, int rows, const int *slot_idx, float *out) const;
    AdvanceArgs advance_args(int m, int T) const;
    struct GreedyIo {
        int gen = 1;
        const int *now = nullptr;
        const float *eout = nullptr;
        const int *eout_rows = nullptr;
        const int *rec_off = nullptr; int rec_slot0 = 0;
        float *dump = nullptr;
    };
    void run_greedy_rounds(int n, bool dump_logits, int chunk = 0, const float *eout_rows = nullptr);
    void run_greedy_rounds(int n, const GreedyIo &io);
    void run_lm_chain(int m, int T, bool dump_logits);
    void run_lm_wavefront(int m, int T, bool dump_logits);
    struct SwPlan {
        struct Batch { size_t off; int n, macro, kind; size_t roff; int rn; };
        std::vector<GemmArgs> host; GemmArgs *dev = nullptr; std::vector<Batch> batches;
        std::vector<RowArgs> rhost; RowArgs *rdev = nullptr;
        std::vector<std::pair<int, long>> stamp_slots; std::vector<int> stamp_n;
    };
    GraphCache::Key graph_key(int m, int T = 0, int part = 0) const { return {m, T, flight_parity_ * 4 + part}; }
    GraphCache::Key sw_key(int m, int T, int part = 0) const { return graph_key(gclk_ ? -m : m, T, part); }
    SwPlan &sw_plan(int m, int T);
    void free_sw_plans();
    void run_sw_chain(int m, int T, bool dump_logits, const SwPlan &p, int part, hipStream_t st);
    int stage_step(int m, int T, const int *slots, const int *ring_tails, const int *now_ms); void read_back_logits(int k, int rows, float *out);
    template <typename Chain> hipGraphExec_t cached_graph(GraphCache &cache, const GraphCache::Key &key, hipStream_t st, Chain &&chain);
    template <typename Capture> void capture_both_parities(Capture &&capture);
    void run_feed_wavefront(int m, int T, bool dump_logits); void run_layer_major(int m, int T, bool dump_logits); void launch_split_feed(int m, int T, hipStream_t fe);
    struct StreamTrace { hipEvent_t ev[6] = {nullptr, nullptr, nullptr, nullptr, nullptr, nullptr}; int m = 0, T = 0; bool used = false; };
    std::deque<StreamTrace> trace_; hipEvent_t trace_base_ = nullptr;
    StreamTrace *trace_slot();
    void dump_stream_trace();
    void select_parity(int p);
    void join(hipStream_t waiter, hipStream_t src);
    void general_prologue();
    int next_step_index() { ++flight_steps_; return (int)(step_seq_++ & (uint64_t)(2 * step_cap_ - 1)); }
    void launch_rowepi(GemmArgs fused_form, float *ws, hipStream_t st, bool force = false, int cls = T_GEMM_OTHER);
    bool gates_tile_rows(long rows) const;
    void run_decproj(int n, const int *d_slots, const int *row_mask, const int *run_flag, int run_gen, float *out = nullptr);
    void build_dec_table();
    void run_chain(int m, bool dump_logits);
    void collect_gates_clock();
    void timed_begin(int cls);
    void timed_end(int cls);
    void collect_timing();
    DecEmbedParams dec_params() const;

    EngineConfig cfg_;
    PackedLayout L_;
    ModelParams P_;
    hipStream_t stream_ = nullptr;
    float *w_ = nullptr;
    uint16_t *wh_ = nullptr;
    void lin(GemmArgs &g, size_t off) const { if (wh_) { g.wp = wh_ + off; g.wt = 1; } else { g.wp = w_ + off; g.wt = 0; } }
    bool f16_tile_ = false;
    uint16_t *wx_ = nullptr;
    uint16_t *y16_ = nullptr, *xb16_ = nullptr, *u16_ = nullptr, *ff16_ = nullptr;
    uint16_t *h16_ = nullptr;
    int kzx_hr_ = 1, kzx_ff2_ = 1;
    void lin16(GemmArgs &g, size_t off) const { g.wp = wx_ + off; g.wt = 1; g.tile_ok = 2; }
    int kz_hr() const { return f16_tile_ ? kzx_hr_ : kz_hr_; }
    int kz_ff2() const { return f16_tile_ ? kzx_ff2_ : kz_ff2_; }
    float *h_ = nullptr, *c_ = nullptr, *ring_ = nullptr, *eout_ = nullptr, *dout_ = nullptr;
    GreedyState *gstate_ = nullptr;
    float *dec_table_ = nullptr;
    uint8_t *cls_ = nullptr;
    int ring_frames_ = 0;
    float *xin_ = nullptr, *a3_ = nullptr, *y_ = nullptr, *ssq_ = nullptr, *xb_ = nullptr, *u_ = nullptr, *ff_ = nullptr, *ws_ = nullptr, *ws_g_ = nullptr, *de_ = nullptr;
    float *logits_ = nullptr;
    float *p_lm_ = nullptr, *eout_lm_ = nullptr;
    int *ring_h_ = nullptr; size_t ring_cap_ = 0, ring_pos_ = 0;
    int *step_off_h_ = nullptr, *rec_off_h_ = nullptr; int step_cap_ = 0;
    StepRecord *rec_d_ = nullptr, *rec_h_ = nullptr; size_t rec_cap_ = 0, rec_pos_ = 0;
    int flight_parity_ = 0, next_parity_ = 0; size_t ring_base_ = 0, rec_base_ = 0; int flight_steps_ = 0;
    uint64_t step_seq_ = 0;
    hipEvent_t flight_done_[2] = {nullptr, nullptr};
    std::mutex conf_mu_;
    std::vector<std::pair<int, int>> conf_pending_;
    std::atomic<bool> conf_has_pending_{false}, conf_ever_{false};
    uint8_t *conf_k_d_ = nullptr, *conf_k_h_ = nullptr;
    ConfRecord *conf_d_ = nullptr, *conf_h_ = nullptr;
    std::vector<std::pair<size_t, size_t>> conf_spans_;
    std::atomic<uint64_t> conf_copied_{0};
    void apply_confidence_pending();
    void drop_graphs();
    struct BiasEntry { std::shared_ptr<const BiasSet> set; int users = 0; void *dev = nullptr; };
    std::mutex bias_mu_;
    std::vector<BiasEntry> bias_sets_;
    std::vector<int> bias_slot_set_;
    std::vector<std::pair<int, int>> bias_pending_;
    std::atomic<bool> bias_has_pending_{false}, bias_ever_{false};
    int32_t *bias_set_d_ = nullptr, *bias_set_h_ = nullptr, *bias_state_d_ = nullptr;
    BiasDesc *bias_desc_d_ = nullptr, *bias_desc_h_ = nullptr;
    void apply_bias_pending();
    std::mutex opt_mu_;
    std::vector<std::pair<int, SearchOpt>> opt_pending_;
    std::atomic<bool> opt_has_pending_{false}, opt_ever_{false};
    SearchOpt *opt_d_ = nullptr, *opt_h_ = nullptr;
    void apply_search_options_pending();
    BiasDesc upload_bias(const BiasSet &set, void **dev, hipStream_t st);
    void debug_decide_impl(int n, int op, const float *logits, float early_emit, const int *now_ms, int round, int32_t *state_io, StepRecord *rec_out,
                           const BiasSet *set, int32_t *bias_state_io, const SearchOpt *opts = nullptr);
    void note_conf_step(int k, const int *slots, int m, size_t records);
    bool flight_open_[2] = {false, false};
    hipStream_t f_stream_ = nullptr, s_stream_ = nullptr, search_stream_ = nullptr;
    std::vector<hipEvent_t> join_ev_; size_t join_pos_ = 0;
    bool f_unseen_by_m_ = false, s_unseen_by_m_ = false, m_unseen_by_f_ = false, m_unseen_by_s_ = false, flight_tail_s_ = false;
    bool overlap_hint_ = false;
    int split_streams_ = 2;
    float *y_buf_[2] = {nullptr, nullptr}, *ssq_buf_[2] = {nullptr, nullptr}, *eout_lm_buf_[2] = {nullptr, nullptr}, *ws_fe_ = nullptr, *ws_sr_ = nullptr;
    uint16_t *y16_buf_[2] = {nullptr, nullptr};
    int *step_buf_[2] = {nullptr, nullptr}, *flags_buf_[2] = {nullptr, nullptr}, *rec_off_buf_[2] = {nullptr, nullptr};
    int *counter_d_ = nullptr, *step_d_ = nullptr, *active_d_ = nullptr, *dirty_d_ = nullptr, *rec_off_d_ = nullptr, *flags_d_ = nullptr;
    int *dec_slots_d_ = nullptr;
    float *logits_h_ = nullptr;
    FbankFrameDesc *hs_desc_[2] = {nullptr, nullptr}, *ds_desc_[2] = {nullptr, nullptr}; int desc_cap_ = 0;
    int16_t *hs_pcm_[2] = {nullptr, nullptr}, *ds_pcm_[2] = {nullptr, nullptr}; size_t pcm_cap_ = 0;
    int fb_flip_ = 0;
    hipEvent_t fb_done_[2] = {nullptr, nullptr};
    std::vector<size_t> part_off_;
    size_t rs_cap_ = 0;
    int rs_n_ = 0;
    ResampleDesc *rs_desc_ = nullptr;
    const ResampleSpec *const *rs_specs_ = nullptr;
    const std::pair<const int16_t *, size_t> *rs_in_parts_ = nullptr;
    size_t rs_n_in_parts_ = 0, rs_n_in_ = 0;
    std::mutex rs_mu_;
    std::map<const ResampleSpec *, const float *> rs_tables_;
    const float *resample_table(const ResampleSpec *spec);
    FbankTables ft_;
    std::vector<void *> table_allocs_;
    float pad_value_ = 0;
    std::vector<int> free_, zero_pending_;
    void zero_pending_slots();
    std::atomic<int> live_{0};
    std::mutex slot_mu_;
    std::mutex capture_mu_;
    int kz_embed_ = 1, kz_hr_ = 1, kz_ff2_ = 1, kz_proj_ = 1, kz_out_ = 1;
    int ws_mstride_ = 0;
    float *conv_wt_ = nullptr;
    bool use_graphs_ = true;
    GraphCache step_graphs_{"chunk step", 256};
    GraphCache lm_graphs_{"layer-major chain", 32};
    GraphCache lm_search_graphs_{"long-feed search", 64};
    GraphCache sw_graphs_{"feed wavefront", 4 * 64};
    size_t sw_plan_cap_ = 64;
    std::map<GraphCache::Key, SwPlan> sw_plans_;
    hipStream_t lm_stream_ = nullptr;
    std::vector<hipEvent_t> lm_events_;
    GemmArgs *zargs_h_ = nullptr, *zargs_d_ = nullptr; size_t zargs_region_ = 0, zargs_pos_ = 0;
    hipEvent_t zargs_done_[3] = {nullptr, nullptr, nullptr}; bool zargs_busy_[3] = {false, false, false}; int zargs_next_ = 0;
    int *lm_now_d_ = nullptr, *lm_rows_d_ = nullptr, *lm_rec_off_d_ = nullptr;
    std::atomic<long> kernels_per_step_{0};
    long launch_count_ = 0;
    bool profiling_ = false;
    bool gclk_ = false, gclk_warned_ = false; unsigned long long *gclk_slots_ = nullptr; int gclk_used_ = 0;
    static constexpr int GCLK_SLOTS = 2048;
    double gclk_ms_ = 0; long gclk_launches_ = 0, gclk_rows_ = 0; double gclk_ms_n_[4] = {0, 0, 0, 0}; long gclk_launches_n_[4] = {0, 0, 0, 0};
    struct Ev { hipEvent_t a, b; int cls; };
    std::vector<Ev> ev_pool_; size_t ev_used_ = 0;
    KernelTiming timing_[T_COUNT];
};

}
```

april_asr_amd/csrc/kernels.h:

```cpp
#pragma once
#include <hip/hip_runtime.h>
#include <cstdint>

namespace aprilx {

enum GemmEpilogue {
    EPI_PARTIAL = 0,
    EPI_LSTM = 1,
    EPI_BIAS_DSWISH = 2,
    EPI_HR = 3,
    EPI_RESID_SSQ = 4,
    EPI_SLOT_STORE = 5,
    EPI_XPART = 6
};
enum GemmAOp { AOP_NONE = 0, AOP_TANH_ADD = 1 };
enum GemmMode { GM_SLAB = 0, GM_FULLK = 1, GM_TILE = 2, GM_KW = 3, GM_PP = 4 };


constexpr int SSQ_COLS = 32;

struct RowScale {
    const float *ssq = nullptr;
    int groups = 0;
    float inv_n = 0.0f;
    float eps = 0.0f;
};

struct GreedyState { int32_t ctx0, ctx1; int32_t last_tok; uint32_t last_emit_ms; };

constexpr int STAMP_WORDS = 144, STAMP_ENDS = 8, STAMP_NENDS = 64, STAMP_SUBS = 72;

struct GemmArgs {
    const float *a0 = nullptr; int lda0 = 0; const int *aidx0 = nullptr; int K0 = 0;
    const float *a1 = nullptr; int lda1 = 0; const int *aidx1 = nullptr; int K1 = 0;
    const float *a0b = nullptr;
    const int *aidx0b = nullptr; int same_idx_b = 1;
    const GreedyState *ctx_state = nullptr; int ctx_vocab = 0;
    int a_op = AOP_NONE;
    RowScale x_scale;
    const void *wp = nullptr;
    int wt = 0;
    int M = 0, N = 0, K = 0;
    int kz = 1;
    int zs = 1;
    int mode = GM_SLAB;
    int epi = EPI_PARTIAL;
    float *out = nullptr; int ldo = 0;
    void *out16 = nullptr;
    void *state16 = nullptr;
    int m_stride = 0;
    const float *bias = nullptr;
    float *c_state = nullptr;
    const int *slot_idx = nullptr;
    int hidden = 0;
    float *state = nullptr; int ld_state = 0;
    const float *resid = nullptr; int ldr = 0;
    RowScale r_scale;
    float *ssq_out = nullptr;
    const int *row_mask = nullptr;
    const int *run_flag = nullptr;
    int run_gen = 1;
    int wave_mask = 0xF;
    const float *p_add = nullptr; int ldp = 0;
    int force_fullk = 0;
    int zcount = 1;
    int tile_ok = 0;
    int asm_loop = 0;
    unsigned long long *trace = nullptr;
    unsigned long long *stamp = nullptr;
    int debug = 0;
};
void launch_gemm(const GemmArgs &g, hipStream_t s);
void gemm_profile_next_launch(hipEvent_t start, hipEvent_t stop);
bool gemm_profile_pending();
void launch_gemm_tile(const GemmArgs &g, int mt, int nt, const GemmArgs *dev_args, int n, hipStream_t s);
int gemm_kw_waves(const GemmArgs &g);
bool gemm_pp_ok(const GemmArgs &g, int mt);
void launch_gemm_pp(const GemmArgs &g, int mt, const GemmArgs *dev_args, int n, hipStream_t s);
bool gemm_pw_ok(const GemmArgs &g);
void launch_gemm_pw(const GemmArgs &g, const GemmArgs *dev_args, int n, hipStream_t s);
void gemm_pp_pin(int enable, int mt);
bool gemm_kw_has_kernel(const GemmArgs &g, int mt, int nt);
void launch_gemm_kw(const GemmArgs &g, int mt, int nt, const GemmArgs *dev_args, int n, hipStream_t s);
void gemm_kw_pin(int enable, int mt);
int recur_form(const GemmArgs &g);
void launch_recur(const GemmArgs &g, int form, const GemmArgs *dev_args, int n, hipStream_t s);
void stage_gemm_z(const GemmArgs *items, int n, GemmArgs *staged);
void launch_gemm_z(const GemmArgs *staged, int n, const GemmArgs *dev_args, hipStream_t s);
int gemm_partials(int M, int N, int kz, int zcount = 1, int tile_ok = 0);
bool gemm_fullk(int M, int N, int kz, bool force = false, int zcount = 1, int tile_ok = 0);
bool gemm_tile_planned(int M, int N, int kz, int zcount = 1);
void gemm_tile_pin(int enable, int mt, int zs);

enum RowMode {
    ROW_HR = 0,
    ROW_RESID_SSQ = 1,
    ROW_SLOT_STORE = 2
};
struct RowArgs {
    int mode = ROW_HR;
    const float *ws = nullptr; int parts = 1; int m_stride = 0; int N = 0; int M = 0;
    const float *bias = nullptr;
    const float *resid = nullptr; int ldr = 0;
    RowScale r_scale;
    float *out = nullptr; int ldo = 0;
    const int *slot_idx = nullptr;
    float *state = nullptr; int ld_state = 0;
    float *ssq_out = nullptr;
    void *out16 = nullptr, *state16 = nullptr;
    const int *row_mask = nullptr;
    const int *run_flag = nullptr;
    int run_gen = 1;
};
void launch_row(const RowArgs &r, hipStream_t s);
void launch_row_z(const RowArgs *host_args, int n, const RowArgs *dev_args, hipStream_t s);

struct StepRecord { int32_t idx; float max_val; float blank_val; uint32_t flags; };
constexpr int kConfMaxAlt = 8;
struct ConfRecord { float lse; float blank_val; int32_t n_alt; uint32_t reserved; int32_t alt_id[kConfMaxAlt]; float alt_logit[kConfMaxAlt]; };
static_assert(sizeof(ConfRecord) == 80, "ConfRecord is 20 x 32 bit");
enum { REC_VALID = 1, REC_BLANK = 2, REC_CTX = 4 };
enum TokClassBits { TKC_WORD_START = 1, TKC_SENT_END = 2, TKC_COMMA = 4, TKC_DOT = 8, TKC_DIGIT_START = 16 };

struct BiasDesc { const int32_t *state_off = nullptr, *edge_tok = nullptr, *edge_next = nullptr; const float *edge_bonus = nullptr; int32_t n_states = 0, flags = 0; };

struct SearchOpt { uint32_t endpoint_ms; float blank_penalty; };
static_assert(sizeof(SearchOpt) == 8, "SearchOpt is 2 x 32 bit");

struct DecEmbedParams {
    const float *emb = nullptr;
    const float *conv_w = nullptr;
    const float *conv_b = nullptr;
    int d = 0, groups = 0, context = 0, vocab = 0;
};

struct DecideArgs {
    const float *ws = nullptr; int parts = 1; int m_stride = 0; int N = 0; int M = 0;
    int n_valid = 0;
    const float *bias = nullptr;
    int blank = 0;
    float early_emit = 0.0f;
    const int *slot_idx = nullptr;
    const int *now_ms = nullptr;
    int *active = nullptr;
    int gen = 1;
    int rec_slot = 0;
    int *dirty = nullptr;
    const uint8_t *tok_class = nullptr;
    GreedyState *state = nullptr;
    StepRecord *rec = nullptr;
    StepRecord *rec_ring = nullptr;
    const int *rec_off = nullptr; int round = 0;
    float *logits_dump = nullptr;
    DecEmbedParams dec;
    float *de_out = nullptr; int ld_de = 0;
    int *run_flags = nullptr;
    int *rerun_flags = nullptr;
    const uint8_t *conf_k = nullptr;
    ConfRecord *conf_ring = nullptr;
    ConfRecord *conf = nullptr; int conf_k_all = 0;
    const int32_t *bias_set = nullptr;
    int32_t *bias_state = nullptr;
    const BiasDesc *bias_desc = nullptr;
    const SearchOpt *opt = nullptr;
};
void launch_decide(const DecideArgs &a, hipStream_t s);

struct DecRowsArgs {
    const int *slot_idx = nullptr; int M = 0;
    int op = 0; int blank = 0;
    GreedyState *state = nullptr;
    DecEmbedParams dec;
    float *de_out = nullptr; int ld_de = 0;
    int32_t *bias_state = nullptr;
};
void launch_dec_rows(const DecRowsArgs &a, hipStream_t s);

struct DecEmbedArgs {
    DecEmbedParams dec;
    const int *ctx = nullptr;
    int M = 0;
    float *out = nullptr; int ldo = 0;
};
void launch_dec_embed(const DecEmbedArgs &a, hipStream_t s);

struct AdvanceArgs {
    const int *host_ring = nullptr;
    const int *host_step_off = nullptr;
    const int *host_rec_off = nullptr;
    int *counter = nullptr;
    int index_mask = 0x7fffffff;
    int *dst = nullptr; int dst_stride = 0;
    int n_arrays = 3; int len[4] = {0, 0, 0, 0};
    int *rec_off = nullptr;
    int *flags = nullptr; int n_flags = 0;
};
void launch_advance(const AdvanceArgs &a, hipStream_t s);

struct ZeroSlotArgs {
    float *h = nullptr, *c = nullptr; int n_layers = 0; size_t slots = 0; int d_model = 0, hidden = 0;
    float *eout = nullptr, *dout = nullptr; int joiner = 0;
    GreedyState *state = nullptr; int blank = 0;
    int slot = 0;
    void *h16 = nullptr;
    int n_list = 0; int list[64] = {0};
};
void launch_zero_slot(const ZeroSlotArgs &a, hipStream_t s);

struct BlockSetupArgs {
    const int *now_src = nullptr; int *now_dst = nullptr;
    int *rows_dst = nullptr; int row0 = 0; int count = 0;
    const int *rec_off_step = nullptr; int *rec_off_block = nullptr; int rec_add = 0;
    int *flags = nullptr; int n_flags = 0;
};
void launch_block_setup(const BlockSetupArgs &a, hipStream_t s);

struct ConvEmbedArgs {
    const float *ring = nullptr;
    int ring_frames = 0, mel = 0, seg = 0;
    const int *slot_idx = nullptr;
    const int *ring_tail = nullptr;
    const float *w[3] = {nullptr, nullptr, nullptr};
    const float *b[3] = {nullptr, nullptr, nullptr};
    int ch[3] = {0, 0, 0};
    int ch1_per_group = 0;
    int stride[3] = {1, 2, 2};
    float *out = nullptr; int ldo = 0;
    int M = 0;
    const float *x_direct = nullptr;
    const float *w0t = nullptr, *w1t = nullptr;
};
void launch_conv_embed(const ConvEmbedArgs &a, hipStream_t s);
void launch_conv_weight_transpose(const float *w0, const float *w1, int c0, int c1, float *w0t, float *w1t, hipStream_t s);

void launch_cvt_f16(const float *src, void *dst, size_t n, hipStream_t s);

void launch_repack_x32(const float *src_packed, void *dst, int K, int N, hipStream_t s);

struct FbankTables {
    const float *window = nullptr;
    const double *tw[16] = {nullptr};
    const double *tws[16] = {nullptr};
    int fct[16] = {0}; int nfct = 0;
    const float *mel = nullptr;
    const int *mel_lo = nullptr;
    const int *mel_hi = nullptr;
    int padded = 0, nbins = 0;
};
struct FbankFrameDesc { int32_t slot; int32_t ring_row; int32_t pcm_off; };
struct FbankArgs {
    FbankTables t;
    const int16_t *pcm = nullptr;
    const FbankFrameDesc *desc = nullptr;
    int n_frames = 0;
    float *ring = nullptr; int ring_frames = 0;
    float pad_value = 0.0f;
};
void launch_fbank(const FbankArgs &a, hipStream_t s);

struct ResampleDesc {
    const float *taps = nullptr;
    int64_t in_base = 0;
    int64_t out_first = 0;
    int64_t out_end = 0;
    int32_t in_off = 0, in_n = 0;
    int32_t out_dst = 0, out_cnt = 0;
    int32_t L = 1, M = 1, K = 0, ldt = 0;
};
// ... 12 lines not shown
```

april_asr_amd/csrc/kernels_misc.hip:

```cpp
#include "kernels.h"
#include "device_utils.h"
#include "env.h"
#include <algorithm>
#include <cstdio>
#include <cstdlib>

namespace aprilx {

template <int MODE>
__device__ __forceinline__ void row_body(const RowArgs &r)
{
    if (r.run_flag && *r.run_flag != r.run_gen) return;
    const int m = blockIdx.x;
    const int tid = threadIdx.x;
    const int slot = r.slot_idx ? r.slot_idx[m] : m;
    if (MODE == ROW_SLOT_STORE) { if (r.row_mask && !r.row_mask[m]) return; }
    float rs = 1.0f;
    const bool scaled = MODE == ROW_HR || (MODE == ROW_SLOT_STORE && r.r_scale.ssq != nullptr);
    if (scaled) rs = row_scale(r.r_scale, m);
    const int nq = r.N >> 2;
    for (int q0 = 0; q0 < nq; q0 += 256) {
        const int q = q0 + tid;
        const bool ok = q < nq;
        const int n = q * 4;
        f32x4 s = f32x4{0.f, 0.f, 0.f, 0.f};
        if (ok) s = tree_sum4(r.ws, r.parts, r.m_stride, r.N, m, n);
        if (MODE == ROW_HR) {
            if (ok) {
                const HrTail t = hr_tail(s, *reinterpret_cast<const f32x4 *>(r.resid + (size_t)m * r.ldr + n), rs);
                *reinterpret_cast<f32x4 *>(r.state + (size_t)slot * r.ld_state + n) = t.state;
                *reinterpret_cast<f32x4 *>(r.out + (size_t)m * r.ldo + n) = t.out;
                if (r.state16) *reinterpret_cast<h4 *>(reinterpret_cast<_Float16 *>(r.state16) + (size_t)slot * r.ld_state + n) = to_h4(t.state);
                if (r.out16) *reinterpret_cast<h4 *>(reinterpret_cast<_Float16 *>(r.out16) + (size_t)m * r.ldo + n) = to_h4(t.out);
            }
        } else if (MODE == ROW_RESID_SSQ) {
            f32x4 y = f32x4{0.f, 0.f, 0.f, 0.f};
            if (ok) {
                const f32x4 res = r.resid ? *reinterpret_cast<const f32x4 *>(r.resid + (size_t)m * r.ldr + n) : f32x4{0.f, 0.f, 0.f, 0.f};
                y = resid_tail(s, *reinterpret_cast<const f32x4 *>(r.bias + n), res, r.resid != nullptr);
                *reinterpret_cast<f32x4 *>(r.out + (size_t)m * r.ldo + n) = y;
                if (r.out16) *reinterpret_cast<h4 *>(reinterpret_cast<_Float16 *>(r.out16) + (size_t)m * r.ldo + n) = to_h4(y);
            }
            float ss;
            if (granule_ssq_store(y, ok, q, ss)) r.ssq_out[(size_t)m * (r.N / SSQ_COLS) + n / SSQ_COLS] = ss;
        } else {
            if (ok) {
                const f32x4 b = *reinterpret_cast<const f32x4 *>(r.bias + n);
                *reinterpret_cast<f32x4 *>(r.out + (size_t)slot * r.ldo + n) = scaled ? slot_value(s, rs, b) : slot_value(s, b);
            }
        }
    }
}

template <int MODE>
__global__ __launch_bounds__(256) void row_kernel(RowArgs r) { row_body<MODE>(r); }

template <int MODE>
__global__ __launch_bounds__(256) void row_zkernel(const RowArgs *__restrict__ zargs)
{
    const RowArgs r = zargs[blockIdx.y];
    row_body<MODE>(r);
}

void launch_row(const RowArgs &r, hipStream_t s)
{
    dim3 grid((unsigned)r.M), block(256);
    switch (r.mode) {
    case ROW_HR: hipLaunchKernelGGL(row_kernel<ROW_HR>, grid, block, 0, s, r); break;
    case ROW_RESID_SSQ: hipLaunchKernelGGL(row_kernel<ROW_RESID_SSQ>, grid, block, 0, s, r); break;
    default: hipLaunchKernelGGL(row_kernel<ROW_SLOT_STORE>, grid, block, 0, s, r); break;
    }
}

void launch_row_z(const RowArgs *host_args, int n, const RowArgs *dev_args, hipStream_t s)
{
    if (n <= 0) return;
    const RowArgs &r = host_args[0];
    for (int i = 1; i < n; ++i)
        if (host_args[i].mode != r.mode || host_args[i].M != r.M || host_args[i].N != r.N || host_args[i].parts != r.parts) {
            fprintf(stderr, "libapril(mi355x): launch_row_z: the problems of one launch must have one shape\n"); abort();
        }
    dim3 grid((unsigned)r.M, (unsigned)n), block(256);
    switch (r.mode) {
    case ROW_HR: hipLaunchKernelGGL(row_zkernel<ROW_HR>, grid, block, 0, s, dev_args); break;
    case ROW_RESID_SSQ: hipLaunchKernelGGL(row_zkernel<ROW_RESID_SSQ>, grid, block, 0, s, dev_args); break;
    default: hipLaunchKernelGGL(row_zkernel<ROW_SLOT_STORE>, grid, block, 0, s, dev_args); break;
    }
}

__device__ __forceinline__ void dec_embed_row(const DecEmbedParams &p, int tok0, int tok1, float *out)
{
    const int cg = p.d / p.groups;
    for (int o = threadIdx.x; o < p.d; o += 256) {
        const int g0 = (o / cg) * cg;
        const float *w = p.conv_w + (size_t)o * cg * p.context;
        float acc = 0.0f;
        for (int ci = 0; ci < cg; ++ci) {
            acc += p.emb[(size_t)tok0 * p.d + g0 + ci] * w[ci * p.context + 0];
            acc += p.emb[(size_t)tok1 * p.d + g0 + ci] * w[ci * p.context + 1];
        }
        if (p.conv_b) acc += p.conv_b[o];
        out[o] = acc > 0.0f ? acc : 0.0f;
    }
}

#include "kernels_bias.inc"
#include "kernels_confidence.inc"

template <bool CONF, bool BIAS, bool OPT>
__device__ __forceinline__ void decide_body(const DecideArgs &a)
{
    extern __shared__ __attribute__((aligned(16))) unsigned char bias_lds[];
    __shared__ float s_best[4], s_blank[4];
    __shared__ int s_idx[4];
    __shared__ int s_ctx[3];
    if (a.round > 0 && a.run_flags && a.run_flags[a.round] != a.gen) return;
    const int m = blockIdx.x;
    const int tid = threadIdx.x;
    StepRecord *rec = a.rec ? a.rec + m : a.rec_ring + (size_t)a.rec_off[0] + (size_t)a.rec_slot * a.M + m;
    if (a.round > 0 && a.active[m] != a.gen) {
        if (tid == 0) { rec->idx = -1; rec->max_val = 0.0f; rec->blank_val = 0.0f; rec->flags = 0; a.dirty[m] = 0; }
        return;
    }
    float best = -9999999999.0f;
    int best_i = -1;
    float blank_v = 0.0f;
    BiasRow br;
    if (BIAS) bias_row_begin(a, m, bias_lds, br);
    if (BIAS && br.bonus) bias_scan(a, m, br, best, best_i, blank_v);
    else
    for (int n = tid; n < a.n_valid; n += 256) {
        const float v = tree_sum(a.ws, a.parts, a.m_stride, a.N, m, n) + a.bias[n];
        if (a.logits_dump) a.logits_dump[(size_t)m * a.n_valid + n] = v;
        if (n == a.blank) blank_v = v;
        else if (v > best) { best = v; best_i = n; }
    }
#pragma unroll
    for (int off = 32; off > 0; off >>= 1) {
        const float ov = __shfl_xor(best, off);
        const int oi = __shfl_xor(best_i, off);
        const bool take = (oi >= 0) && (best_i < 0 || ov > best || (ov == best && oi < best_i));
        if (take) { best = ov; best_i = oi; }
        blank_v += __shfl_xor(blank_v, off);
    }
    const int wave = tid >> 6;
    if ((tid & 63) == 0) { s_best[wave] = best; s_idx[wave] = best_i; s_blank[wave] = blank_v; }
    __syncthreads();
    if (tid == 0) {
        float b = s_best[0]; int bi = s_idx[0];
        for (int w = 1; w < 4; ++w) {
            const float ov = s_best[w]; const int oi = s_idx[w];
            if (oi >= 0 && (bi < 0 || ov > b || (ov == b && oi < bi))) { b = ov; bi = oi; }
        }
        float bl = s_blank[(a.blank & 255) >> 6];
        rec->idx = bi; rec->max_val = b; rec->blank_val = bl;

        const int slot = a.slot_idx[m];
        GreedyState st = a.state[slot];
        SearchOpt so; so.endpoint_ms = 0u; so.blank_penalty = 0.0f;
        if (OPT) { so = a.opt[slot]; if (so.endpoint_ms) bl = bl - so.blank_penalty; }
        int tok = bi; float tv = b;
        if (tok < 0) { tok = a.blank == 0 ? 1 : 0; tv = -9999999999.0f; }
        const bool cleared = st.ctx1 == a.blank;
        const bool same = st.ctx1 == tok;
        const float ee = same ? 0.0f : a.early_emit;
        bool is_blank = (bl - ee) > tv;
        const unsigned tc = a.tok_class[tok];
        bool punct = (tc & (TKC_SENT_END | TKC_COMMA)) != 0;
        if (punct && st.last_tok >= 0 && (a.tok_class[st.last_tok] & TKC_DIGIT_START) && (tc & TKC_DOT)) punct = false;
        if (!cleared && punct && !same && tv > (bl - 3.5f)) is_blank = false;
        const unsigned now = (unsigned)a.now_ms[m];
        unsigned flags = REC_VALID;
        bool rerun = false, silence = false;
        if (!is_blank) {
            st.last_emit_ms = now;
            st.ctx0 = st.ctx1; st.ctx1 = tok;
            st.last_tok = tok;
            rerun = true;
        } else {
            flags |= REC_BLANK;
            if (OPT && so.endpoint_ms) silence = now - st.last_emit_ms >= so.endpoint_ms;
            else if (now - st.last_emit_ms >= 2200u) { silence = true; }
            if (silence) {
                st.last_tok = -1;
                if (st.ctx0 != a.blank) { st.ctx0 = a.blank; st.ctx1 = a.blank; rerun = true; }
            }
        }
        a.active[m] = is_blank ? 0 : a.gen;
        if (rerun) flags |= REC_CTX;
        rec->flags = flags;
        a.state[slot] = st;
        if (BIAS && br.bonus) bias_row_end(a, br, slot, is_blank, tok, OPT ? silence : is_blank && now - st.last_emit_ms >= 2200u);
        a.dirty[m] = rerun ? 1 : 0;
        if (a.run_flags) {
            if (!is_blank && a.round < 2) a.run_flags[a.round + 1] = a.gen;
            if (rerun) a.rerun_flags[a.round] = a.gen;
        }
        s_ctx[0] = st.ctx0; s_ctx[1] = st.ctx1; s_ctx[2] = rerun ? 1 : 0;
    }
    __syncthreads();
    if (s_ctx[2] && a.de_out) dec_embed_row(a.dec, s_ctx[0], s_ctx[1], a.de_out + (size_t)m * a.ld_de);
    if (CONF) {
        if (a.conf) confidence_row(a, m, a.conf_k_all, a.conf + m, BIAS ? br.bonus : nullptr);
        else {
            const int k = a.conf_k[a.slot_idx[m]];
            if (k) confidence_row(a, m, k, a.conf_ring + (rec - a.rec_ring), BIAS ? br.bonus : nullptr);
        }
    }
}

__global__ __launch_bounds__(256) void decide_kernel(DecideArgs a) { decide_body<false, false, false>(a); }
__global__ __launch_bounds__(256) void decide_conf_kernel(DecideArgs a) { decide_body<true, false, false>(a); }
__global__ __launch_bounds__(256) void decide_bias_kernel(DecideArgs a) { decide_body<false, true, false>(a); }
__global__ __launch_bounds__(256) void decide_conf_bias_kernel(DecideArgs a) { decide_body<true, true, false>(a); }
__global__ __launch_bounds__(256) void decide_opt_kernel(DecideArgs a) { decide_body<false, false, true>(a); }
__global__ __launch_bounds__(256) void decide_conf_opt_kernel(DecideArgs a) { decide_body<true, false, true>(a); }
__global__ __launch_bounds__(256) void decide_bias_opt_kernel(DecideArgs a) { decide_body<false, true, true>(a); }
__global__ __launch_bounds__(256) void decide_conf_bias_opt_kernel(DecideArgs a) { decide_body<true, true, true>(a); }

void launch_decide(const DecideArgs &a, hipStream_t s)
{
    const bool conf = a.conf || a.conf_k;
    if (a.bias_set) {
        if (a.n_valid > 8192 || !a.bias_state || !a.bias_desc) { fprintf(stderr, "libapril(mi355x): launch_decide: phrase boosting needs a vocabulary of at most 8192 tokens and all three tables\n"); abort(); }
        const size_t lds = bias_lds_bytes(a.n_valid);
        if (a.opt) {
            if (conf) hipLaunchKernelGGL(decide_conf_bias_opt_kernel, dim3((unsigned)a.M), dim3(256), lds, s, a);
            else hipLaunchKernelGGL(decide_bias_opt_kernel, dim3((unsigned)a.M), dim3(256), lds, s, a);
        }
        else if (conf) hipLaunchKernelGGL(decide_conf_bias_kernel, dim3((unsigned)a.M), dim3(256), lds, s, a);
        else hipLaunchKernelGGL(decide_bias_kernel, dim3((unsigned)a.M), dim3(256), lds, s, a);
    }
    else if (a.opt) {
        if (conf) hipLaunchKernelGGL(decide_conf_opt_kernel, dim3((unsigned)a.M), dim3(256), 0, s, a);
        else hipLaunchKernelGGL(decide_opt_kernel, dim3((unsigned)a.M), dim3(256), 0, s, a);
    }
    else if (conf) hipLaunchKernelGGL(decide_conf_kernel, dim3((unsigned)a.M), dim3(256), 0, s, a);
    else hipLaunchKernelGGL(decide_kernel, dim3((unsigned)a.M), dim3(256), 0, s, a);
}

// ... 356 lines not shown
```

include/aprilx_engine.h:

```cpp
#ifndef APRILX_ENGINE_H
#define APRILX_ENGINE_H
#include "april_api.h"

#ifdef __cplusplus
extern "C" {
#endif

typedef struct AprilxDims {
    int32_t n_layers, d_model, hidden, ffn, joiner, vocab, mel, seg, seg_step, context;
    int32_t fft_size, frame_shift, sample_rate, blank_id, n_devices;
    int32_t precision;
    int32_t d_model_file;
    int64_t param_count;
} AprilxDims;
APRIL_EXPORT int aprilx_model_dims(AprilASRModel model, AprilxDims *out);
APRIL_EXPORT const char *aprilx_model_token(AprilASRModel model, int32_t id);

typedef struct AprilxLoadInfo {
    double broadcast_ms;
    double comm_init_ms;
    uint64_t broadcast_bytes;
    int32_t ranks;
    int32_t used_rccl;
} AprilxLoadInfo;
APRIL_EXPORT int aprilx_broadcast_get_id(void *id_out, size_t cap);
APRIL_EXPORT AprilASRModel aprilx_model_broadcast(AprilASRModel root_model, int rank, int world, const void *id_bytes);
APRIL_EXPORT int aprilx_model_load_info(AprilASRModel model, AprilxLoadInfo *out);
APRIL_EXPORT size_t aprilx_model_blob_size(AprilASRModel model);
APRIL_EXPORT int aprilx_model_export_blob(AprilASRModel model, void *dst, size_t dst_size);
APRIL_EXPORT AprilASRModel aprilx_model_from_blob(const void *blob, size_t size, int blob_is_device_ptr);
APRIL_EXPORT int aprilx_model_save_blob(AprilASRModel model, const char *path);
APRIL_EXPORT int aprilx_model_save_blob_f16(AprilASRModel model, const char *path);
APRIL_EXPORT AprilASRModel aprilx_model_load_blob(const char *path);

APRIL_EXPORT void aprilx_feed_many(size_t n, AprilASRSession *sessions, const short *const *pcm16, const size_t *short_counts);
APRIL_EXPORT void aprilx_flush_many(size_t n, AprilASRSession *sessions);
APRIL_EXPORT void aprilx_session_drain(AprilASRSession session);
APRIL_EXPORT void aprilx_feed_many_pipelined(size_t n, AprilASRSession *sessions, const short *const *pcm16, const size_t *short_counts, int depth);
APRIL_EXPORT void aprilx_drain_many(size_t n, AprilASRSession *sessions);

APRIL_EXPORT int aprilx_run_encoder(AprilASRModel model, int n, const float *x, const float *h, const float *c,
                                    float *eout, float *h2, float *c2);
APRIL_EXPORT int aprilx_run_decoder(AprilASRModel model, int n, const int64_t *context, float *dout);
APRIL_EXPORT int aprilx_run_joiner(AprilASRModel model, int n, const float *eout, const float *dout, float *logits);
APRIL_EXPORT int aprilx_run_fbank(AprilASRModel model, int n_frames, const int16_t *pcm_frames, float *out);
APRIL_EXPORT int aprilx_run_decide(AprilASRModel model, int n, int op, const float *logits, float early_emit, const int32_t *now_ms,
                                   int round, int32_t *state_io, void *records_out);

APRIL_EXPORT int aprilx_plan_gemm(int M, int N, int kz, int zcount, int tile_ok, int force, int32_t *out);

APRIL_EXPORT int aprilx_stream_form(int kind, int M, int N, int K, int kz, int groups);

APRIL_EXPORT int aprilx_session_set_input_rate(AprilASRSession session, uint32_t rate_hz);
APRIL_EXPORT uint32_t aprilx_session_input_rate(AprilASRSession session);
APRIL_EXPORT int aprilx_resampler_taps(uint32_t in_rate, uint32_t out_rate, int32_t *lmk_out, float *taps, size_t cap);
APRIL_EXPORT int64_t aprilx_resample(AprilASRModel model, uint32_t in_rate, const int16_t *pcm, size_t n, int16_t *out, size_t cap);

typedef struct AprilxTokenInfo {
    uint32_t size;
    uint32_t n_alt;
    uint64_t eval_index;
    float lse;
    float token_logprob;
    float blank_logprob;
    float reserved0;
    int32_t alt_id[8];
    float alt_logit[8];
} AprilxTokenInfo;
APRIL_EXPORT int aprilx_session_set_confidence(AprilASRSession session, int n_alternatives);
APRIL_EXPORT int aprilx_session_confidence(AprilASRSession session);
APRIL_EXPORT int aprilx_run_confidence(AprilASRModel model, int n, const float *logits, int k, AprilxTokenInfo *out);

typedef struct AprilxBias_i *AprilxBias;
APRIL_EXPORT AprilxBias aprilx_bias_create(AprilASRModel model, size_t n, const char *const *phrases, const float *boosts, char *err, size_t err_cap);
#define APRILX_BIAS_STRICT 1u
APRIL_EXPORT AprilxBias aprilx_bias_create_ex(AprilASRModel model, size_t n, const char *const *phrases, const float *boosts, uint32_t flags, char *err,
                                              size_t err_cap);
APRIL_EXPORT int aprilx_bias_flags(AprilxBias bias);
APRIL_EXPORT void aprilx_bias_free(AprilxBias bias);
APRIL_EXPORT int aprilx_bias_info(AprilxBias bias, int32_t *states, int64_t *edges);
APRIL_EXPORT int aprilx_bias_edges(AprilxBias bias, int32_t state, int32_t *tok, int32_t *next, float *bonus, size_t cap);
APRIL_EXPORT int aprilx_session_set_bias(AprilASRSession session, AprilxBias bias);
APRIL_EXPORT int aprilx_session_bias_state(AprilASRSession session, int32_t *host_state, int32_t *device_state);
APRIL_EXPORT int aprilx_run_decide_biased(AprilASRModel model, int n, int op, const float *logits, float early_emit, const int32_t *now_ms, int round,
                                          int32_t *state_io, void *records_out, AprilxBias bias, int32_t *bias_state_io);
APRIL_EXPORT int aprilx_run_confidence_biased(AprilASRModel model, int n, const float *logits, int k, AprilxBias bias, const int32_t *bias_state,
                                              AprilxTokenInfo *out);

typedef struct AprilxSearchOptions {
    uint32_t size;
    uint32_t endpoint_silence_ms;
    uint32_t max_utterance_ms;
    float blank_penalty;
} AprilxSearchOptions;
APRIL_EXPORT int aprilx_session_set_search_options(AprilASRSession session, const AprilxSearchOptions *options);
APRIL_EXPORT int aprilx_session_search_options(AprilASRSession session, AprilxSearchOptions *out);
APRIL_EXPORT int aprilx_run_decide_opts(AprilASRModel model, int n, int op, const float *logits, float early_emit, const int32_t *now_ms, int round,
                                        int32_t *state_io, void *records_out, AprilxBias bias, int32_t *bias_state_io, const AprilxSearchOptions *opts);

APRIL_EXPORT void aprilx_session_trace_logits(AprilASRSession session, float *buf, size_t cap_floats, size_t *used_floats);
APRIL_EXPORT uint64_t aprilx_session_chunks(AprilASRSession session);
APRIL_EXPORT uint64_t aprilx_session_read_frames(AprilASRSession session, uint64_t first, int n, float *out);
APRIL_EXPORT void aprilx_session_context(AprilASRSession session, int32_t *host_ctx, int32_t *device_state);

typedef struct AprilxStats {
    uint64_t ticks, steps, chunks, rounds, frames, max_batch_seen;
    double kernel_ms[6];
    uint64_t kernel_launches[6];
    double host_ms[8];
    uint64_t flights;
    uint64_t replay_mismatch;
    uint64_t kernels_per_step;
    uint64_t lm_steps, lm_chunks;
    uint64_t wave_steps, wave_chunks;
    double gates_clock_ms; uint64_t gates_clock_launches, gates_clock_rows;
    double gates_clock_ms_by_n[4]; uint64_t gates_clock_launches_by_n[4];
    double resample_ms; uint64_t resample_launches;
    uint64_t confidence_records;
} AprilxStats;
APRIL_EXPORT void aprilx_model_stats(AprilASRModel model, int device_index, AprilxStats *out);
APRIL_EXPORT int aprilx_model_feed_latency(AprilASRModel model, int device_index, double *out_ms, int cap, int reset);
APRIL_EXPORT void aprilx_model_profile(AprilASRModel model, int enable);

typedef struct AprilxGreedy_i *AprilxGreedy;
APRIL_EXPORT AprilxGreedy aprilx_greedy_create(AprilASRModel model, AprilRecognitionResultHandler handler, void *userdata);
APRIL_EXPORT int aprilx_greedy_step(AprilxGreedy g, int32_t idx, float max_val, float blank_val, float early_emit,
                                    size_t now_ms, int32_t *ctx_out);
APRIL_EXPORT void aprilx_greedy_finish(AprilxGreedy g);
APRIL_EXPORT void aprilx_greedy_free(AprilxGreedy g);
APRIL_EXPORT int aprilx_greedy_set_bias(AprilxGreedy g, AprilxBias bias);
APRIL_EXPORT int aprilx_greedy_bias_state(AprilxGreedy g);
APRIL_EXPORT int aprilx_greedy_set_search_options(AprilxGreedy g, const AprilxSearchOptions *options);

APRIL_EXPORT void aprilx_counting_handler(void *userdata, AprilResultType type, size_t count, const AprilToken *tokens);

APRIL_EXPORT AprilASRModel aprilx_model_load_host(const char *model_path);
APRIL_EXPORT int aprilx_model_fbank_tables(AprilASRModel model, float *window, float *mel);

APRIL_EXPORT int aprilx_probe_file(const char *path, char *err, size_t err_cap);

#ifdef __cplusplus
}
#endif
#endif
```

Measured before the change: 19750.

## Merge the next feed's wavefront ramp-up into the previous feed's ramp-down

Adds a 'ramp merge' mode, on by default through APRIL_RAMP_MERGE=1. When two consecutive split feeds share the same batch size, the tail macro-steps of one feed's layer wavefront host the head problems of the next feed through device-side ready/latch flags. Working buffers are double-buffered per parity so the two feeds do not collide. The aim is to fill the underused ramp-up and ramp-down batches of the wavefront and cut launch count. In exchange it adds small latch kernels, run flags on GEMM problems, a second plan chain per shape and a fair amount of cross-feed synchronisation complexity.

```diff
diff --git a/april_asr_amd/__init__.py b/april_asr_amd/__init__.py
--- a/april_asr_amd/__init__.py
+++ b/april_asr_amd/__init__.py
@@ -266,6 +266,12 @@
         s = _ffi.AprilxStats()
         self._L.aprilx_model_stats(self._handle, device_index, C.byref(s))
         return s
+
+    def ramp_stats(self, device_index: int = 0):
+        h, e = C.c_uint64(0), C.c_uint64(0)
+        if self._L.aprilx_model_ramp_stats(self._handle, device_index, C.byref(h), C.byref(e)) != 0:
+            raise ValueError("aprilx_model_ramp_stats refused the call")
+        return int(h.value), int(e.value)
 
     def feed_latencies(self, device_index: int = 0, reset: bool = False) -> np.ndarray:
         n = int(self._L.aprilx_model_feed_latency(self._handle, device_index, None, 0, 0))
diff --git a/april_asr_amd/_ffi.py b/april_asr_amd/_ffi.py
--- a/april_asr_amd/_ffi.py
+++ b/april_asr_amd/_ffi.py
@@ -71,6 +71,7 @@
     "aprilx_run_decide_biased", "aprilx_greedy_set_bias", "aprilx_greedy_bias_state",
     "aprilx_bias_create_ex", "aprilx_bias_flags", "aprilx_run_confidence_biased",
     "aprilx_session_set_search_options", "aprilx_session_search_options", "aprilx_run_decide_opts", "aprilx_greedy_set_search_options",
+    "aprilx_ramp_window", "aprilx_model_ramp_stats",
 ]
 
 _lib = None
@@ -118,6 +119,8 @@
     L.aprilx_run_joiner.argtypes = [vp, C.c_int, vp, vp, vp]; L.aprilx_run_joiner.restype = C.c_int
     L.aprilx_run_fbank.argtypes = [vp, C.c_int, vp, vp]; L.aprilx_run_fbank.restype = C.c_int
     L.aprilx_plan_gemm.argtypes = [C.c_int] * 6 + [vp]; L.aprilx_plan_gemm.restype = C.c_int
+    L.aprilx_ramp_window.argtypes = [C.c_int] * 3 + [vp, C.c_int]; L.aprilx_ramp_window.restype = C.c_int
+    L.aprilx_model_ramp_stats.argtypes = [vp, C.c_int, C.POINTER(C.c_uint64), C.POINTER(C.c_uint64)]; L.aprilx_model_ramp_stats.restype = C.c_int
     L.aprilx_stream_form.argtypes = [C.c_int] * 6; L.aprilx_stream_form.restype = C.c_int
     L.aprilx_run_decide.argtypes = [vp, C.c_int, C.c_int, vp, C.c_float, vp, C.c_int, vp, vp]; L.aprilx_run_decide.restype = C.c_int
     L.aprilx_session_trace_logits.argtypes = [vp, vp, sz, C.POINTER(sz)]; L.aprilx_session_trace_logits.restype = None
diff --git a/april_asr_amd/csrc/engine.cc b/april_asr_amd/csrc/engine.cc
--- a/april_asr_amd/csrc/engine.cc
+++ b/april_asr_amd/csrc/engine.cc
@@ -203,8 +203,9 @@
         if (f16_tile_) {
             kzx_hr_ = pick_kz(d.hidden, d.d_model, 32); kzx_ff2_ = pick_kz(d.ffn, d.d_model, 32);
             for (int p = 0; p < 2; ++p) y16_buf_[p] = dmalloc<uint16_t>(MB * d.d_model);
-            y16_ = y16_buf_[0]; xb16_ = dmalloc<uint16_t>(MB * d.d_model);
-            u16_ = dmalloc<uint16_t>(MB * d.hidden); ff16_ = dmalloc<uint16_t>(MB * d.ffn);
+            y16_ = y16_buf_[0];
+            for (int p = 0; p < 2; ++p) { xb16_buf_[p] = dmalloc<uint16_t>(MB * d.d_model); u16_buf_[p] = dmalloc<uint16_t>(MB * d.hidden); ff16_buf_[p] = dmalloc<uint16_t>(MB * d.ffn); }
+            xb16_ = xb16_buf_[0]; u16_ = u16_buf_[0]; ff16_ = ff16_buf_[0];
             h16_ = dmalloc<uint16_t>((size_t)d.n_layers * S * d.d_model);
             HIP_CHECK(hipMemset(h16_, 0, (size_t)d.n_layers * S * d.d_model * 2));
         }
@@ -220,9 +221,11 @@
     y_ = y_buf_[0]; ssq_ = ssq_buf_[0];
     ws_fe_ = dmalloc<float>((size_t)kz_embed_ * d.d_model * MB);
     ws_sr_ = dmalloc<float>((size_t)std::max(kz_proj_ * d.joiner, d.d_model) * MB);
-    xb_ = dmalloc<float>(MB * d.d_model);
-    u_ = dmalloc<float>(MB * d.hidden);
-    ff_ = dmalloc<float>(MB * d.ffn);
+    for (int p = 0; p < 2; ++p) { xb_buf_[p] = dmalloc<float>(MB * d.d_model); u_buf_[p] = dmalloc<float>(MB * d.hidden); ff_buf_[p] = dmalloc<float>(MB * d.ffn); }
+    xb_ = xb_buf_[0]; u_ = u_buf_[0]; ff_ = ff_buf_[0];
+    ramp_mode_ = env_int("APRIL_RAMP_MERGE", 1);
+    if (ramp_mode_ < 0 || ramp_mode_ > 2) ramp_mode_ = 1;
+    ramp_d_ = dmalloc<RampState>(1); HIP_CHECK(hipMemset(ramp_d_, 0, sizeof(RampState)));
     de_ = dmalloc<float>(MB * d.d_model);
     HIP_CHECK(hipMemset(de_, 0, MB * d.d_model * 4));
     logits_ = dmalloc<float>(3 * MB * d.vocab);
@@ -312,6 +315,10 @@
     (void)hipSetDevice(cfg_.device);
     (void)hipStreamSynchronize(f_stream_); (void)hipStreamSynchronize(stream_); (void)hipStreamSynchronize(s_stream_);
     dump_stream_trace();
+    if (ramp_d_ && ramp_eligible_.load() > 0) {
+        unsigned h = 0;
+        if (hipMemcpy(&h, &ramp_d_->hosted, sizeof h, hipMemcpyDeviceToHost) == hipSuccess) LOGI("engine: ramp merge: %u of %llu hostable split feeds were hosted by their predecessor", h, (unsigned long long)ramp_eligible_.load());
+    }
     for (StreamTrace &t : trace_) for (hipEvent_t e : t.ev) if (e) (void)hipEventDestroy(e);
     if (trace_base_) (void)hipEventDestroy(trace_base_);
     for (hipEvent_t e : join_ev_) (void)hipEventDestroy(e);
@@ -336,12 +343,13 @@
     if (dec_table_) (void)hipFree(dec_table_);
     if (p_lm_) (void)hipFree(p_lm_);
     for (int p = 0; p < 2; ++p)
-        for (void *q : {(void *)eout_lm_buf_[p], (void *)y16_buf_[p], (void *)y_buf_[p], (void *)ssq_buf_[p], (void *)rec_off_buf_[p], (void *)flags_buf_[p], (void *)step_buf_[p]}) if (q) (void)hipFree(q);
+        for (void *q : {(void *)eout_lm_buf_[p], (void *)y16_buf_[p], (void *)y_buf_[p], (void *)ssq_buf_[p], (void *)xb_buf_[p], (void *)u_buf_[p], (void *)ff_buf_[p],
+                        (void *)xb16_buf_[p], (void *)u16_buf_[p], (void *)ff16_buf_[p], (void *)rec_off_buf_[p], (void *)flags_buf_[p], (void *)step_buf_[p]}) if (q) (void)hipFree(q);
     if (ws_fe_) (void)hipFree(ws_fe_);
     if (ws_sr_) (void)hipFree(ws_sr_);
-    for (void *p : {(void *)wx_, (void *)xb16_, (void *)u16_, (void *)ff16_, (void *)h16_}) if (p) (void)hipFree(p);
+    for (void *p : {(void *)wx_, (void *)h16_, (void *)ramp_d_}) if (p) (void)hipFree(p);
     for (void *p : {(void *)w_, (void *)wh_, (void *)h_, (void *)c_, (void *)ring_, (void *)eout_, (void *)dout_, (void *)gstate_, (void *)cls_, (void *)ws_, (void *)xin_,
-                    (void *)a3_, (void *)xb_, (void *)u_, (void *)ff_, (void *)de_, (void *)logits_, (void *)rec_d_, (void *)counter_d_,
+                    (void *)a3_, (void *)de_, (void *)logits_, (void *)rec_d_, (void *)counter_d_,
                     (void *)active_d_, (void *)dirty_d_, (void *)dec_slots_d_,
                     (void *)ds_desc_[0], (void *)ds_desc_[1], (void *)ds_pcm_[0], (void *)ds_pcm_[1]})
         if (p) (void)hipFree(p);
@@ -392,6 +400,7 @@
     if (zero_pending_.empty()) return;
     if (hipSetDevice(cfg_.device) == hipSuccess) {
         std::lock_guard<std::mutex> cg(capture_mu_);
+        m_touched();
         const NetDims &d = L_.dims;
         for (size_t o = 0; o < zero_pending_.size(); o += 64) {
             ZeroSlotArgs z;
@@ -424,6 +433,7 @@
 
 void Engine::sync()
 {
+    m_touched();
     sync_streams();
     f_unseen_by_m_ = s_unseen_by_m_ = m_unseen_by_f_ = m_unseen_by_s_ = false;
     if (profiling_) collect_timing();
@@ -458,6 +468,7 @@
 template <typename Capture> void Engine::capture_both_parities(Capture &&capture)
 {
     const int par = flight_parity_;
+    m_touched();
     for (int q : {1 - par, par}) { select_parity(q); capture(); }
 }
 
@@ -507,6 +518,7 @@
 
 void Engine::general_prologue()
 {
+    m_touched();
     if (f_unseen_by_m_) { join(stream_, f_stream_); f_unseen_by_m_ = false; }
     if (s_unseen_by_m_) { join(stream_, s_stream_); s_unseen_by_m_ = false; }
     m_unseen_by_f_ = m_unseen_by_s_ = true;
@@ -639,6 +651,7 @@
     a.t = ft_; a.pcm = ds_pcm_[b]; a.desc = reinterpret_cast<const FbankFrameDesc *>(reinterpret_cast<const char *>(ds_pcm_[b]) + doff); a.n_frames = n_frames; a.ring = ring_; a.ring_frames = ring_frames_; a.pad_value = pad_value_;
     if (n_rs) { ra.in = ds_pcm_[b]; ra.out = ds_pcm_[b]; ra.desc = reinterpret_cast<const ResampleDesc *>(reinterpret_cast<const char *>(ds_pcm_[b]) + roff); }
     if (profiling_) {
+        m_touched();
         join(stream_, f_stream_);
         if (n_rs) { timed_begin(T_RESAMPLE); launch_resample(ra, stream_); timed_end(T_RESAMPLE); }
         timed_begin(T_FBANK); launch_fbank(a, stream_); timed_end(T_FBANK);
@@ -1066,31 +1079,86 @@
         gclk_used_ = 0;
     }
     SwPlan &p = sw_plans_[key];
+    build_sw_chain(p, p.one, m, T, false);
+    if (ramp_mode_ != 0 && !gclk_) build_sw_chain(p, p.split, m, T, true);
+    return p;
+}
+
+std::vector<RampStep> ramp_window(int L, int T, int R, int max_problems)
+{
+    std::vector<RampStep> w;
+    if (L <= 2 * R || T < 1 || R < 1) return w;
+    for (int j = 1; j <= R; ++j) {
+        RampStep s; s.macro = L + T - 1 - R + j;
+        for (int l = 0; l < L; ++l) { const int t = s.macro - 1 - l; if (t >= 0 && t < T) ++s.own; }
+        for (int t = 0; t < j; ++t) s.guests.push_back(std::make_pair(j - 1 - t, t));
+        if (s.own + (int)s.guests.size() > max_problems) return std::vector<RampStep>();
+        w.push_back(s);
+    }
+    return w;
+}
+
+void Engine::ramp_counts(uint64_t *hosted, uint64_t *eligible)
+{
+    unsigned h = 0;
+    {
+        HipLegacyLock legacy;
+        if (hipSetDevice(cfg_.device) == hipSuccess) HIP_CHECK(hipMemcpy(&h, &ramp_d_->hosted, sizeof h, hipMemcpyDeviceToHost));
+    }
+    *hosted = h; *eligible = ramp_eligible_.load(std::memory_order_relaxed);
+}
+
+void Engine::build_sw_chain(SwPlan &p, SwPlan::Chain &c, int m, int T, bool ramp)
+{
     const NetDims &d = L_.dims;
     const int L = d.n_layers;
+    const int par = flight_parity_;
+    const int tk = f16_tile_ ? 2 : tile_ok();
+    auto needs_rows = [&](int kind, int n) {
+        const int kz = kind == 1 ? kz_hr() : kz_ff2();
+        return (kind == 1 || kind == 3) && tk && (tk == 2 || gemm_tile_planned(m, d.d_model, kz, n)) && !gemm_fullk(m, d.d_model, kz, false, n, tk);
+    };
+    std::vector<RampStep> window;
+    if (ramp && m <= RAMP_MAX_M && T <= RAMP_MAX_T) {
+        window = ramp_window(L, T, RAMP_R);
+        for (const RampStep &s : window) if (needs_rows(1, s.own + (int)s.guests.size()) || needs_rows(3, s.own + (int)s.guests.size())) { window.clear(); break; }
+    }
+    if (ramp) p.hosts = !window.empty();
     std::vector<GemmArgs> items;
     std::vector<RowArgs> rows;
     for (int W = 0; W <= T + L; ++W) {
+        const RampStep *host = nullptr; int wj = 0;
+        for (size_t j = 0; j < window.size(); ++j) if (window[j].macro == W) { host = &window[j]; wj = (int)j; }
+        if (host && wj == 0) { SwPlan::Batch b; b.off = c.host.size(); b.n = 0; b.macro = W; b.kind = 4; b.roff = c.rhost.size(); b.rn = 0; c.batches.push_back(b); }
         for (int kind = 0; kind < 4; ++kind) {
             items.clear(); rows.clear();
             int n_act = 0;
             for (int l = 0; l < L; ++l) { const int t = W - 1 - l; if (t >= 0 && t < T) ++n_act; }
             if (n_act == 0) continue;
+            if (host) n_act += (int)host->guests.size();
             const int kz = kind == 1 ? kz_hr() : kz_ff2();
-            const int tk = f16_tile_ ? 2 : tile_ok();
-            const bool split = (kind == 1 || kind == 3) && tk && (tk == 2 || gemm_tile_planned(m, d.d_model, kz, n_act)) && !gemm_fullk(m, d.d_model, kz, false, n_act, tk);
-            for (int l = 0; l < L; ++l) {
-                const int t = W - 1 - l;
-                if (t < 0 || t >= T) continue;
+            const bool split = needs_rows(kind, n_act);
+            auto problem = [&](int l, int t, const int *run_flag) {
                 const size_t r0 = (size_t)t * m;
                 GemmArgs g = kind == 0 ? args_gates(l, r0, m, GATES_ALL) : kind == 1 ? args_whr(l, r0, m) : kind == 2 ? args_ff1(l, r0, m) : args_ff2(l, r0, m);
                 if (kind == 0 && cfg_.precision == 0) g.tile_ok = gates_tile_rows((long)m * n_act) ? 2 : 0;
+                if (run_flag) { g.run_flag = run_flag; g.run_gen = 1; }
                 if (split) {
                     float *ws = ws_ + r0 * d.d_model;
                     rows.push_back(row_form(g, ws, ws_mstride_, gemm_partials(m, d.d_model, kz, n_act, tk)));
                     g = partial_form(g, ws, ws_mstride_);
                 } else if (tk == 2) g.force_fullk = 0;
                 items.push_back(g);
+            };
+            for (int l = 0; l < L; ++l) {
+                const int t = W - 1 - l;
+                if (t < 0 || t >= T) continue;
+                problem(l, t, ramp && W <= RAMP_R ? &ramp_d_->head_live[par] : nullptr);
+            }
+            if (host) {
+                select_parity(1 - par);
+                for (const auto &lt : host->guests) problem(lt.first, lt.second, &ramp_d_->guest_live[par][wj][lt.second]);
+                select_parity(par);
             }
             std::vector<int> groups;
             {
@@ -1102,35 +1170,35 @@
             size_t first = 0;
             for (size_t gi = 0; gi < groups.size(); ++gi) {
                 const int gn = groups[gi];
-                if (kind == 0 && gclk_ && gclk_slots_ && gclk_used_ < GCLK_SLOTS) {
+                if (kind == 0 && !ramp && gclk_ && gclk_slots_ && gclk_used_ < GCLK_SLOTS) {
                     p.stamp_slots.push_back(std::make_pair(gclk_used_, (long)m * gn)); p.stamp_n.push_back(gn);
                     for (int i = 0; i < gn; ++i) items[first + (size_t)i].stamp = gclk_slots_ + (size_t)gclk_used_ * STAMP_WORDS;
                     ++gclk_used_;
-                } else if (kind == 0 && gclk_ && gclk_slots_ && !gclk_warned_) {
+                } else if (kind == 0 && !ramp && gclk_ && gclk_slots_ && !gclk_warned_) {
                     gclk_warned_ = true; LOGW("engine: the gates clock is out of stamp slots (%d): the gates launches of further plans are not timed", GCLK_SLOTS);
                 }
-                SwPlan::Batch b; b.off = p.host.size(); b.n = gn; b.macro = W; b.kind = kind; b.roff = p.rhost.size(); b.rn = gi == 0 ? (int)rows.size() : 0;
-                p.host.resize(p.host.size() + (size_t)gn);
-                stage_gemm_z(items.data() + first, gn, p.host.data() + b.off);
-                if (gi == 0) p.rhost.insert(p.rhost.end(), rows.begin(), rows.end());
-                p.batches.push_back(b);
+                SwPlan::Batch b; b.off = c.host.size(); b.n = gn; b.macro = W; b.kind = kind; b.roff = c.rhost.size(); b.rn = gi == 0 ? (int)rows.size() : 0;
+                c.host.resize(c.host.size() + (size_t)gn);
+                stage_gemm_z(items.data() + first, gn, c.host.data() + b.off);
+                if (gi == 0) c.rhost.insert(c.rhost.end(), rows.begin(), rows.end());
+                c.batches.push_back(b);
                 first += (size_t)gn;
             }
         }
     }
-    p.dev = dmalloc<GemmArgs>(p.host.size());
-    HIP_CHECK(hipMemcpyAsync(p.dev, p.host.data(), p.host.size() * sizeof(GemmArgs), hipMemcpyHostToDevice, stream_));
-    if (!p.rhost.empty()) {
-        p.rdev = dmalloc<RowArgs>(p.rhost.size());
-        HIP_CHECK(hipMemcpyAsync(p.rdev, p.rhost.data(), p.rhost.size() * sizeof(RowArgs), hipMemcpyHostToDevice, stream_));
-    }
-    return p;
+    m_touched();
+    c.dev = dmalloc<GemmArgs>(c.host.size());
+    HIP_CHECK(hipMemcpyAsync(c.dev, c.host.data(), c.host.size() * sizeof(GemmArgs), hipMemcpyHostToDevice, stream_));
+    if (!c.rhost.empty()) {
+        c.rdev = dmalloc<RowArgs>(c.rhost.size());
+        HIP_CHECK(hipMemcpyAsync(c.rdev, c.rhost.data(), c.rhost.size() * sizeof(RowArgs), hipMemcpyHostToDevice, stream_));
+    }
 }
 
 void Engine::free_sw_plans()
 {
     if (!sw_plans_.empty()) LOGI("engine: feed wavefront plans emptied (%zu plans)", sw_plans_.size());
-    for (auto &p : sw_plans_) { if (p.second.dev) (void)hipFree(p.second.dev); if (p.second.rdev) (void)hipFree(p.second.rdev); }
+    for (auto &p : sw_plans_) for (SwPlan::Chain *c : {&p.second.one, &p.second.split}) { if (c->dev) (void)hipFree(c->dev); if (c->rdev) (void)hipFree(c->rdev); }
     sw_graphs_.clear(); sw_plans_.clear();
 }
 
@@ -1144,10 +1212,12 @@
     }
     if (part < 0 || part == 1) {
         static const int cls_of[4] = {T_GATES, T_GEMM_OTHER, T_GEMM_OTHER, T_GEMM_OTHER};
-        for (size_t bi = 0; bi < p.batches.size(); ++bi) {
-            const SwPlan::Batch &b = p.batches[bi];
-            timed_begin(cls_of[b.kind]); launch_gemm_z(p.host.data() + b.off, b.n, p.dev + b.off, st); timed_end(cls_of[b.kind]);
-            if (b.rn > 0) { timed_begin(T_ROW); launch_row_z(p.rhost.data() + b.roff, b.rn, p.rdev + b.roff, st); timed_end(T_ROW); }
+        const SwPlan::Chain &c = p.layers(part == 1);
+        for (size_t bi = 0; bi < c.batches.size(); ++bi) {
+            const SwPlan::Batch &b = c.batches[bi];
+            if (b.kind == 4) { launch_ramp_latch(ramp_d_, flight_parity_, m, st); continue; }
+            timed_begin(cls_of[b.kind]); launch_gemm_z(c.host.data() + b.off, b.n, c.dev + b.off, st); timed_end(cls_of[b.kind]);
+            if (b.rn > 0) { timed_begin(T_ROW); launch_row_z(c.rhost.data() + b.roff, b.rn, c.rdev + b.roff, st); timed_end(T_ROW); }
         }
         if (part < 0) lm_stage_proj(m, 0, T, st, ws_);
     }
@@ -1215,8 +1285,15 @@
         if (tr) HIP_CHECK(hipEventRecord(tr->ev[2 * i + 1], st));
     };
     part(0, fe);
+    if (ramp_mode_ != 0) {
+        const bool hostable = ramp_mode_ == 1 && fe == f_stream_ && m_quiet_.load(std::memory_order_acquire);
+        if (hostable) ramp_eligible_.fetch_add(1, std::memory_order_relaxed);
+        launch_ramp_ready(ramp_d_, flight_parity_, m, T, hostable ? 1 : 0, fe);
+    }
     if (fe == f_stream_) { join(stream_, f_stream_); f_unseen_by_m_ = false; }
-    part(1, stream_); join(s_stream_, stream_); part(2, s_stream_);
+    part(1, stream_);
+    if (ramp_mode_ != 0) m_quiet_.store(true, std::memory_order_release);
+    join(s_stream_, stream_); part(2, s_stream_);
     if (tr) { tr->m = m; tr->T = T; tr->used = true; }
     s_unseen_by_m_ = true; flight_tail_s_ = true;
     if (fe != f_stream_) m_unseen_by_f_ = true;
@@ -1276,6 +1353,7 @@
     }
     for (const auto &t : todo) if (t.first >= 0 && t.first < cfg_.max_slots) conf_k_h_[t.first] = (uint8_t)t.second;
     std::lock_guard<std::mutex> cg(capture_mu_);
+    m_touched();
     HIP_CHECK(hipMemcpyAsync(conf_k_d_, conf_k_h_, (size_t)cfg_.max_slots, hipMemcpyHostToDevice, stream_));
 }
 
@@ -1311,6 +1389,7 @@
     todo.swap(bias_pending_);
     bias_has_pending_.store(false, std::memory_order_release);
     std::lock_guard<std::mutex> cg(capture_mu_);
+    m_touched();
     if (!bias_set_h_) {
         bool any = false;
         for (const auto &t : todo) any = any || t.second >= 0;
@@ -1368,6 +1447,7 @@
     }
     for (const auto &t : todo) if (t.first >= 0 && t.first < cfg_.max_slots) opt_h_[t.first] = t.second;
     std::lock_guard<std::mutex> cg(capture_mu_);
+    m_touched();
     HIP_CHECK(hipMemcpyAsync(opt_d_, opt_h_, (size_t)cfg_.max_slots * sizeof(SearchOpt), hipMemcpyHostToDevice, stream_));
 }
 
@@ -1397,6 +1477,7 @@
 void Engine::select_parity(int p)
 {
     flight_parity_ = p;
+    xb_ = xb_buf_[p]; u_ = u_buf_[p]; ff_ = ff_buf_[p]; xb16_ = xb16_buf_[p]; u16_ = u16_buf_[p]; ff16_ = ff16_buf_[p];
     y_ = y_buf_[p]; ssq_ = ssq_buf_[p]; y16_ = y16_buf_[p]; step_d_ = step_buf_[p]; flags_d_ = flags_buf_[p]; rec_off_d_ = rec_off_buf_[p]; eout_lm_ = eout_lm_buf_[p];
 }
 
diff --git a/april_asr_amd/csrc/engine.h b/april_asr_amd/csrc/engine.h
--- a/april_asr_amd/csrc/engine.h
+++ b/april_asr_amd/csrc/engine.h
@@ -60,6 +60,9 @@
     void clear();
     std::map<Key, hipGraphExec_t> map_; std::map<std::pair<int, int>, int> uses_;
 };
+
+struct RampStep { int macro = 0, own = 0; std::vector<std::pair<int, int>> guests; };
+std::vector<RampStep> ramp_window(int L, int T, int R, int max_problems = 3);
 
 class Engine {
 public:
@@ -172,6 +175,7 @@
     void gates_clock(double *ms, long *launches, long *rows) const { *ms = gclk_ms_; *launches = gclk_launches_; *rows = gclk_rows_; }
     void gates_clock_by_n(double *ms4, long *launches4) const { for (int i = 0; i < 4; ++i) { ms4[i] = gclk_ms_n_[i]; launches4[i] = gclk_launches_n_[i]; } }
     KernelTiming timing(int cls) const { return timing_[cls]; }
+    void ramp_counts(uint64_t *hosted, uint64_t *eligible);
     void reset_timing();
     enum { T_GATES = 0, T_GEMM_OTHER = 1, T_ROW = 2, T_CONV = 3, T_FBANK = 4, T_DEC = 5, T_RESAMPLE = 6, T_COUNT = 7 };
     long kernels_per_step() const { return kernels_per_step_.load(std::memory_order_relaxed); }
@@ -205,13 +209,17 @@
     void run_lm_wavefront(int m, int T, bool dump_logits);
     struct SwPlan {
         struct Batch { size_t off; int n, macro, kind; size_t roff; int rn; };
-        std::vector<GemmArgs> host; GemmArgs *dev = nullptr; std::vector<Batch> batches;
-        std::vector<RowArgs> rhost; RowArgs *rdev = nullptr;
+        struct Chain { std::vector<GemmArgs> host; GemmArgs *dev = nullptr; std::vector<Batch> batches; std::vector<RowArgs> rhost; RowArgs *rdev = nullptr; };
+        Chain one;
+        Chain split;
+        bool hosts = false;
+        const Chain &layers(bool split_feed) const { return split_feed && !split.batches.empty() ? split : one; }
         std::vector<std::pair<int, long>> stamp_slots; std::vector<int> stamp_n;
     };
     GraphCache::Key graph_key(int m, int T = 0, int part = 0) const { return {m, T, flight_parity_ * 4 + part}; }
     GraphCache::Key sw_key(int m, int T, int part = 0) const { return graph_key(gclk_ ? -m : m, T, part); }
     SwPlan &sw_plan(int m, int T);
+    void build_sw_chain(SwPlan &p, SwPlan::Chain &c, int m, int T, bool ramp);
     void free_sw_plans();
     void run_sw_chain(int m, int T, bool dump_logits, const SwPlan &p, int part, hipStream_t st);
     int stage_step(int m, int T, const int *slots, const int *ring_tails, const int *now_ms); void read_back_logits(int k, int rows, float *out);
@@ -299,6 +307,13 @@
     bool f_unseen_by_m_ = false, s_unseen_by_m_ = false, m_unseen_by_f_ = false, m_unseen_by_s_ = false, flight_tail_s_ = false;
     bool overlap_hint_ = false;
     int split_streams_ = 2;
+    int ramp_mode_ = 1;
+    RampState *ramp_d_ = nullptr;
+    std::atomic<bool> m_quiet_{false};
+    void m_touched() { m_quiet_.store(false, std::memory_order_release); }
+    std::atomic<uint64_t> ramp_eligible_{0};
+    float *xb_buf_[2] = {nullptr, nullptr}, *u_buf_[2] = {nullptr, nullptr}, *ff_buf_[2] = {nullptr, nullptr};
+    uint16_t *xb16_buf_[2] = {nullptr, nullptr}, *u16_buf_[2] = {nullptr, nullptr}, *ff16_buf_[2] = {nullptr, nullptr};
     float *y_buf_[2] = {nullptr, nullptr}, *ssq_buf_[2] = {nullptr, nullptr}, *eout_lm_buf_[2] = {nullptr, nullptr}, *ws_fe_ = nullptr, *ws_sr_ = nullptr;
     uint16_t *y16_buf_[2] = {nullptr, nullptr};
     int *step_buf_[2] = {nullptr, nullptr}, *flags_buf_[2] = {nullptr, nullptr}, *rec_off_buf_[2] = {nullptr, nullptr};
diff --git a/april_asr_amd/csrc/kernels.h b/april_asr_amd/csrc/kernels.h
--- a/april_asr_amd/csrc/kernels.h
+++ b/april_asr_amd/csrc/kernels.h
@@ -114,6 +114,18 @@
 };
 void launch_row(const RowArgs &r, hipStream_t s);
 void launch_row_z(const RowArgs *host_args, int n, const RowArgs *dev_args, hipStream_t s);
+
+constexpr int RAMP_R = 2;
+struct RampState {
+    unsigned long long ready[2];
+    int head_live[2];
+    int guest_live[2][RAMP_R][RAMP_R];
+    unsigned generation;
+    unsigned hosted;
+};
+constexpr int RAMP_MAX_M = 0xFFFFF, RAMP_MAX_T = 0xFF;
+void launch_ramp_ready(RampState *rs, int q, int m, int T, int hostable, hipStream_t s);
+void launch_ramp_latch(RampState *rs, int p, int m, hipStream_t s);
 
 struct StepRecord { int32_t idx; float max_val; float blank_val; uint32_t flags; };
 constexpr int kConfMaxAlt = 8;
diff --git a/april_asr_amd/csrc/kernels_misc.hip b/april_asr_amd/csrc/kernels_misc.hip
--- a/april_asr_amd/csrc/kernels_misc.hip
+++ b/april_asr_amd/csrc/kernels_misc.hip
@@ -86,6 +86,44 @@
     case ROW_RESID_SSQ: hipLaunchKernelGGL(row_zkernel<ROW_RESID_SSQ>, grid, block, 0, s, dev_args); break;
     default: hipLaunchKernelGGL(row_zkernel<ROW_SLOT_STORE>, grid, block, 0, s, dev_args); break;
     }
+}
+
+__global__ __launch_bounds__(64) void ramp_ready_kernel(RampState *rs, int q, int m, int T, int hostable)
+{
+    if (threadIdx.x != 0) return;
+    __hip_atomic_store(&rs->head_live[q], 1, __ATOMIC_RELAXED, __HIP_MEMORY_SCOPE_AGENT);
+    const unsigned g = __hip_atomic_load(&rs->generation, __ATOMIC_RELAXED, __HIP_MEMORY_SCOPE_AGENT) + 1u;
+    __hip_atomic_store(&rs->generation, g, __ATOMIC_RELAXED, __HIP_MEMORY_SCOPE_AGENT);
+    __builtin_amdgcn_fence(__ATOMIC_RELEASE, "agent");
+    asm volatile("s_waitcnt vmcnt(0)" ::: "memory");
+    const unsigned long long rec = ((unsigned long long)g << 32) | ((unsigned long long)(unsigned)m << 12) | ((unsigned long long)(unsigned)T << 4) | (unsigned long long)(hostable & 1);
+    __hip_atomic_store(&rs->ready[q], rec, __ATOMIC_RELAXED, __HIP_MEMORY_SCOPE_AGENT);
+}
+
+__global__ __launch_bounds__(64) void ramp_latch_kernel(RampState *rs, int p, int m)
+{
+    if (threadIdx.x != 0) return;
+    const unsigned long long mine = __hip_atomic_load(&rs->ready[p], __ATOMIC_RELAXED, __HIP_MEMORY_SCOPE_AGENT);
+    const unsigned long long next = __hip_atomic_load(&rs->ready[1 - p], __ATOMIC_RELAXED, __HIP_MEMORY_SCOPE_AGENT);
+    const unsigned g = (unsigned)(mine >> 32);
+    const int next_m = (int)((next >> 12) & RAMP_MAX_M), next_T = (int)((next >> 4) & RAMP_MAX_T);
+    const bool host = (unsigned)(next >> 32) == g + 1u && next_m == m && (int)((mine >> 12) & RAMP_MAX_M) == m && (next & 1ull) != 0;
+    if (host) {
+        __builtin_amdgcn_fence(__ATOMIC_ACQUIRE, "agent");
+        __hip_atomic_store(&rs->head_live[1 - p], 0, __ATOMIC_RELAXED, __HIP_MEMORY_SCOPE_AGENT);
+        rs->hosted += 1u;
+    }
+    for (int j = 1; j <= RAMP_R; ++j)
+        for (int t = 0; t < RAMP_R; ++t) rs->guest_live[p][j - 1][t] = (host && t < j && t < next_T) ? 1 : 0;
+}
+
+void launch_ramp_ready(RampState *rs, int q, int m, int T, int hostable, hipStream_t s)
+{
+    hipLaunchKernelGGL(ramp_ready_kernel, dim3(1), dim3(64), 0, s, rs, q, m, T, hostable);
+}
+void launch_ramp_latch(RampState *rs, int p, int m, hipStream_t s)
+{
+    hipLaunchKernelGGL(ramp_latch_kernel, dim3(1), dim3(64), 0, s, rs, p, m);
 }
 
 __device__ __forceinline__ void dec_embed_row(const DecEmbedParams &p, int tok0, int tok1, float *out)
diff --git a/april_asr_amd/csrc/ramp_api.cc b/april_asr_amd/csrc/ramp_api.cc
--- /dev/null
+++ b/april_asr_amd/csrc/ramp_api.cc
@@ -0,0 +1,34 @@
+#include <vector>
+#include "../../include/april_api.h"
+#include "../../include/aprilx_engine.h"
+#include "common.h"
+#include "session.h"
+
+using namespace aprilx;
+
+struct AprilASRModel_i { Model m; };
+
+extern "C" {
+
+int aprilx_ramp_window(int L, int T, int R, int32_t *out, int cap)
+{
+    if (L <= 0 || T <= 0 || R <= 0 || !out) return -1;
+    const std::vector<RampStep> w = ramp_window(L, T, R);
+    const int stride = 3 + 2 * R;
+    if ((int)w.size() * stride > cap) return -1;
+    for (size_t i = 0; i < w.size(); ++i) {
+        int32_t *o = out + i * (size_t)stride;
+        for (int k = 0; k < stride; ++k) o[k] = -1;
+        o[0] = w[i].macro; o[1] = w[i].own; o[2] = (int32_t)w[i].guests.size();
+        for (size_t g = 0; g < w[i].guests.size() && (int)g < R; ++g) { o[3 + 2 * g] = w[i].guests[g].first; o[4 + 2 * g] = w[i].guests[g].second; }
+    }
+    return (int)w.size();
+}
+int aprilx_model_ramp_stats(AprilASRModel model, int device_index, uint64_t *ramp_hosted, uint64_t *ramp_eligible)
+{
+    if (!model || device_index < 0 || device_index >= (int)model->m.engines.size() || !ramp_hosted || !ramp_eligible) return -1;
+    model->m.engines[(size_t)device_index]->ramp_counts(ramp_hosted, ramp_eligible);
+    return 0;
+}
+
+}
diff --git a/include/aprilx_engine.h b/include/aprilx_engine.h
--- a/include/aprilx_engine.h
+++ b/include/aprilx_engine.h
@@ -48,6 +48,8 @@
                                    int round, int32_t *state_io, void *records_out);
 
 APRIL_EXPORT int aprilx_plan_gemm(int M, int N, int kz, int zcount, int tile_ok, int force, int32_t *out);
+
+APRIL_EXPORT int aprilx_ramp_window(int L, int T, int R, int32_t *out, int cap);
 
 APRIL_EXPORT int aprilx_stream_form(int kind, int M, int N, int K, int kz, int groups);
 
@@ -119,6 +121,7 @@
     uint64_t confidence_records;
 } AprilxStats;
 APRIL_EXPORT void aprilx_model_stats(AprilASRModel model, int device_index, AprilxStats *out);
+APRIL_EXPORT int aprilx_model_ramp_stats(AprilASRModel model, int device_index, uint64_t *ramp_hosted, uint64_t *ramp_eligible);
 APRIL_EXPORT int aprilx_model_feed_latency(AprilASRModel model, int device_index, double *out_ms, int cap, int reset);
 APRIL_EXPORT void aprilx_model_profile(AprilASRModel model, int enable);
 
```

New measurement: 20040 (median of 6 runs). 1.5% higher.
